# ygjwd12345/UCD

Measured on NVIDIA B200. Metric: ucd_loss_fwd_bwd_pixel_pairs_per_s, higher is better.
Workload: dtype bf16 operands / f32 accumulate (contrastive); f32 (CE, KD, upsample)

## Files before the change

include/ucd_b200.h:

```cpp
#ifndef UCD_B200_H
#define UCD_B200_H

#include <stddef.h>
#include <stdint.h>

#ifdef __cplusplus
extern "C" {
#endif

#define UCD_OK 0
#define UCD_EINVAL (-1)
#define UCD_ECUDA (-2)
#define UCD_ENOSUP (-3)

#define UCD_REDUCTION_NONE 0
#define UCD_REDUCTION_MEAN 1
#define UCD_REDUCTION_SUM 2

#define UCD_FEAT_DIM 256
#define UCD_TILE 128

int ucd_version(void);
const char* ucd_last_error(void);
int ucd_device_ok(void);

int ucd_unce_fwd(const float* x, int64_t* y, float* loss_px, float* lse_all, float* lse_old,
                 float* stats , float* scratch ,
                 int B, int C, int old_cl, int64_t HW, int ignore_index, void* stream);
int ucd_unce_bwd(const float* x, const int64_t* y, const float* lse_all,
                 const float* bkg_gap ,
                 const float* g_px, const float* g_scalar, float g_mul, const float* stats,
                 int mean_over_valid, float* dx, int accumulate, int B, int C, int old_cl, int64_t HW,
                 int ignore_index, void* stream);

int ucd_unkd_fwd(const float* x, const float* t, const float* mask, float alpha, float* out_px,
                 float* stats, float* lse3, float* scratch, int B, int C, int C_old, int64_t HW,
                 void* stream);
int ucd_unkd_bwd(const float* x, const float* t, const float* mask, float alpha, const float* lse3,
                 const float* g_px, const float* g_scalar, float g_mul, float* dx, int accumulate, int B, int C,
                 int C_old, int64_t HW, void* stream);
size_t ucd_reduce_scratch_floats(void);

int ucd_kd_fwd(const float* x, const float* t, const float* mask, float alpha, float* out_px, float* stats,
               float* lse3, float* scratch, int B, int C, int C_old, int64_t HW, int variant, float stats_scale,
               void* stream);
int ucd_kd_bwd(const float* x, const float* t, const float* mask, float alpha, const float* lse3,
               const float* g_px, const float* g_scalar, float g_mul, float* dx, int accumulate, int B, int C,
               int C_old, int64_t HW, int variant, void* stream);
int ucd_unce_unkd_bwd(const float* x, const int64_t* y, const float* lse_all, const float* bkg_gap ,
                      const float* ce_g_px, const float* ce_g_scalar, float ce_g_mul, const float* ce_stats,
                      int mean_over_valid, int old_cl, int ignore_index, const float* t, const float* mask,
                      float alpha, const float* lse3, const float* kd_g_px, const float* kd_g_scalar, float kd_g_mul,
                      int kd_variant, float* dx, int accumulate, int B, int C, int C_old, int64_t HW, void* stream);
int ucd_bkg_mask(const float* t_old, const int64_t* labels, float* mask, int B, int C_old, int64_t HW,
                 int old_cl, void* stream);

int ucd_upsample_bilinear_fwd(const float* in, float* out, int64_t planes, int h, int w, int H, int W,
                              void* stream);
int ucd_upsample_bilinear_bwd(const float* gout, float* gin, int64_t planes, int h, int w, int H, int W,
                              void* stream);
int ucd_unce_unkd_bwd_lowres(const float* x, const int64_t* y, const float* lse_all, const float* bkg_gap,
                             const float* ce_g_px, const float* ce_g_scalar, float ce_g_mul, const float* ce_stats,
                             int mean_over_valid, int old_cl, int ignore_index, const float* t, const float* mask,
                             float alpha, const float* lse3, const float* kd_g_px, const float* kd_g_scalar,
                             float kd_g_mul, int kd_variant, float* d_lr, int B, int C, int C_old, int h, int w, int H,
                             int W, void* stream);

size_t ucd_seg_fused_workspace_floats(int B, int C, int C_old, int h, int w, int H, int W);
int ucd_seg_fused_fwd(const float* lr, const float* lr_old, int64_t* labels, float* g_ce, float* g_kd,
                      float* sums, float* workspace, size_t workspace_floats, int B, int C, int C_old, int h,
                      int w, int H, int W, int old_cl, int ignore_index, float alpha, int need_grad,
                      void* stream);

int64_t ucd_con_max_tiles(int64_t n_px);
int ucd_con_prob_kpad(int C_old);
int ucd_con_num_bins(int max_label, int C_old);
int64_t ucd_con_px_meta_ints(int64_t n_px);
int64_t ucd_con_blk_meta_ints(int64_t n_px, int nb);
int ucd_con_prep_labels(const int64_t* labels, const float* l_po, int B, int C_old, int h, int w,
                        int H, int W, int max_label, int32_t* px_meta, int32_t* blk_meta, int32_t* counts,
                        int32_t* counts_host ,
                        void* stream);
int ucd_con_prep_pack(const float* f_n, const float* f_o, const float* l_po, const int32_t* px_meta,
                      int32_t* blk_meta, const int32_t* counts, int B, int C_old, int h, int w, int max_label,
                      float* anchor_f32, float* contrast_f32, void* la, void* lc,
                      int label_bytes ,
                      void* feat_tiles, void* prob_tiles, int32_t* lab_tiles, int32_t* tile_range,
                      int32_t* row_range , int32_t* row_ref, float* inv_norm,
                      int64_t max_tiles, void* stream);
int ucd_con_prep_bwd(const float* g_anchor, const float* anchor_f32, const float* inv_norm,
                     const int32_t* px_meta, const int32_t* blk_meta, float* df_n, int B, int h, int w,
                     void* stream);
int ucd_con_prep_pack_bf16(const void* f_n, const void* f_o, const float* l_po, const int32_t* px_meta,
                           int32_t* blk_meta, const int32_t* counts, int B, int C_old, int h, int w, int max_label,
                           float* anchor_f32, float* contrast_f32, void* la, void* lc, int label_bytes,
                           void* feat_tiles, void* prob_tiles, int32_t* lab_tiles, int32_t* tile_range,
                           int32_t* row_range, int32_t* row_ref, float* inv_norm, int64_t max_tiles, void* stream);
int ucd_con_prep_bwd_bf16(const float* g_anchor, const float* anchor_f32, const float* inv_norm,
                          const int32_t* px_meta, const int32_t* blk_meta, void* df_n, int B, int h, int w,
                          void* stream);
int ucd_con_tile_ranges(const int32_t* lab_tiles, int64_t n_tiles, const int32_t* n_limit, int32_t* tile_range,
                        void* stream);
int ucd_con_pack_rows(const float* rows, const int32_t* labels, int64_t n, void* feat_tiles,
                      int32_t* lab_tiles, int64_t max_tiles, void* stream);

int ucd_rows_normalize_fwd(const float* f, float* rows, float* inv_norm, int B, int h, int w, void* stream);
int ucd_rows_normalize_bwd(const float* g_rows, const float* rows, const float* inv_norm, float* df, int B, int h,
                           int w, void* stream);

size_t ucd_con_workspace_bytes(int64_t max_row_tiles, int64_t max_col_tiles, int64_t plan_row_tiles,
                               int64_t local_col_tiles );
int ucd_con_fwd(const void* feat_tiles, const void* prob_tiles, const int32_t* lab_tiles,
                const int32_t* chunk_counts, int n_chunks, int64_t chunk_tiles, int64_t chunk_stride_bytes,
                int local_chunk, int part, const void* row_feat_tiles,
                const void* row_prob_tiles, const int32_t* row_lab_tiles, const int32_t* n_rows,
                const int32_t* tile_range, const int32_t* row_range, int64_t self_tile0, const int32_t* min_new, int p_mode, int kpad, const float* dense_p,
                int64_t ldp, float inv_temperature, int need_grad, float* out, float* grad_unit,
                void* workspace, size_t workspace_bytes, int64_t max_row_tiles, int64_t plan_row_tiles,
                void* stream);
size_t ucd_selfcon_workspace_bytes(int64_t tiles );
int ucd_selfcon_fwd(const void* feat_tiles, const int32_t* lab_tiles, const int32_t* tile_range, const int32_t* counts,
                    const int32_t* n_rows, int64_t n, int64_t n_anchor, int mode, float inv_temperature, float kappa,
                    int need_grad, float* out, float* grad_unit, void* workspace, size_t workspace_bytes, void* stream);
int ucd_con_bwd(const float* grad_unit, const float* out, const float* g_scalar, float g_mul,
                const int32_t* n_rows, const int32_t* row_ref, float* d_anchor, int64_t max_rows, void* stream);

#ifdef __cplusplus
}
#endif
#endif
```

ucd_b200/_lib.py:

```python
import ctypes
import os
from ctypes import c_float, c_int, c_int64, c_size_t, c_void_p

_HERE = os.path.dirname(os.path.abspath(__file__))
LIB_PATH = os.path.join(_HERE, "libucd_b200.so")

_lib = None

UCD_ENOSUP = -3

P = c_void_p
_PROTOS = {
    "ucd_version": (c_int, []),
    "ucd_last_error": (ctypes.c_char_p, []),
    "ucd_device_ok": (c_int, []),
    "ucd_reduce_scratch_floats": (c_size_t, []),
    "ucd_unce_fwd": (c_int, [P, P, P, P, P, P, P, c_int, c_int, c_int, c_int64, c_int, P]),
    "ucd_unce_bwd": (c_int, [P, P, P, P, P, P, c_float, P, c_int, P, c_int, c_int, c_int, c_int, c_int64, c_int, P]),
    "ucd_unkd_fwd": (c_int, [P, P, P, c_float, P, P, P, P, c_int, c_int, c_int, c_int64, P]),
    "ucd_unkd_bwd": (c_int, [P, P, P, c_float, P, P, P, c_float, P, c_int, c_int, c_int, c_int, c_int64, P]),
    "ucd_kd_fwd": (c_int, [P, P, P, c_float, P, P, P, P, c_int, c_int, c_int, c_int64, c_int, c_float, P]),
    "ucd_kd_bwd": (c_int, [P, P, P, c_float, P, P, P, c_float, P, c_int, c_int, c_int, c_int, c_int64, c_int, P]),
    "ucd_unce_unkd_bwd": (c_int, [P, P, P, P, P, P, c_float, P, c_int, c_int, c_int, P, P, c_float, P, P, P, c_float, c_int,
                                  P, c_int, c_int, c_int, c_int, c_int64, P]),
    "ucd_unce_unkd_bwd_lowres": (c_int, [P, P, P, P, P, P, c_float, P, c_int, c_int, c_int, P, P, c_float, P, P, P,
                                         c_float, c_int, P, c_int, c_int, c_int, c_int, c_int, c_int, c_int, P]),
    "ucd_bkg_mask": (c_int, [P, P, P, c_int, c_int, c_int64, c_int, P]),
    "ucd_upsample_bilinear_fwd": (c_int, [P, P, c_int64, c_int, c_int, c_int, c_int, P]),
    "ucd_upsample_bilinear_bwd": (c_int, [P, P, c_int64, c_int, c_int, c_int, c_int, P]),
    "ucd_seg_fused_workspace_floats": (c_size_t, [c_int, c_int, c_int, c_int, c_int, c_int, c_int]),
    "ucd_seg_fused_fwd": (c_int, [P, P, P, P, P, P, P, c_size_t, c_int, c_int, c_int, c_int, c_int, c_int, c_int,
                                  c_int, c_int, c_float, c_int, P]),
    "ucd_con_max_tiles": (c_int64, [c_int64]),
    "ucd_con_prob_kpad": (c_int, [c_int]),
    "ucd_con_num_bins": (c_int, [c_int, c_int]),
    "ucd_con_px_meta_ints": (c_int64, [c_int64]),
    "ucd_con_blk_meta_ints": (c_int64, [c_int64, c_int]),
    "ucd_con_prep_labels": (c_int, [P, P, c_int, c_int, c_int, c_int, c_int, c_int, c_int, P, P, P, P, P]),
    "ucd_con_prep_pack": (c_int, [P, P, P, P, P, P, c_int, c_int, c_int, c_int, c_int, P, P, P, P, c_int, P, P, P, P,
                                  P, P, P, c_int64, P]),
    "ucd_con_prep_bwd": (c_int, [P, P, P, P, P, P, c_int, c_int, c_int, P]),
    "ucd_con_prep_pack_bf16": (c_int, [P, P, P, P, P, P, c_int, c_int, c_int, c_int, c_int, P, P, P, P, c_int, P, P, P,
                                       P, P, P, P, c_int64, P]),
    "ucd_con_prep_bwd_bf16": (c_int, [P, P, P, P, P, P, c_int, c_int, c_int, P]),
    "ucd_rows_normalize_fwd": (c_int, [P, P, P, c_int, c_int, c_int, P]),
    "ucd_rows_normalize_bwd": (c_int, [P, P, P, P, c_int, c_int, c_int, P]),
    "ucd_con_tile_ranges": (c_int, [P, c_int64, P, P, P]),
    "ucd_con_pack_rows": (c_int, [P, P, c_int64, P, P, c_int64, P]),
    "ucd_con_workspace_bytes": (c_size_t, [c_int64, c_int64, c_int64, c_int64]),
    "ucd_con_fwd": (c_int, [P, P, P, P, c_int, c_int64, c_int64, c_int, c_int, P, P, P, P, P, P, c_int64, P, c_int, c_int,
                            P, c_int64, c_float, c_int, P, P, P, c_size_t, c_int64, c_int64, P]),
    "ucd_con_bwd": (c_int, [P, P, P, c_float, P, P, P, c_int64, P]),
    "ucd_selfcon_workspace_bytes": (c_size_t, [c_int64]),
    "ucd_selfcon_fwd": (c_int, [P, P, P, P, P, c_int64, c_int64, c_int, c_float, c_float, c_int, P, P, P, c_size_t, P]),
}
EXPORTED = tuple(_PROTOS)
_DEBUG_PROTOS = {
    "ucd_con_debug_trace": (c_int, [P]),
    "ucd_con_debug_splits": (c_int, [c_int64, c_int64]),
    "ucd_selftest_umma": (c_int, [c_int, ctypes.POINTER(c_float)]),
    "ucd_selftest_mma_rate": (c_int, [c_int, c_int, ctypes.POINTER(c_float)]),
    "ucd_selftest_mma_mix": (c_int, [c_int] * 8 + [ctypes.POINTER(c_float)]),
    "ucd_selftest_pipe_rate": (c_int, [c_int, c_int, c_int, ctypes.POINTER(c_float)]),
    "ucd_selftest_read_probe": (c_int, [P, ctypes.c_longlong, c_int, c_int, c_int, c_int, ctypes.POINTER(c_float)]),
}
DEBUG_EXPORTED = tuple(_DEBUG_PROTOS)
DEBUG_LIB_PATH = os.path.join(_HERE, "libucd_b200_debug.so")
_debug = None


def lib():
    global _lib
    if _lib is None:
        if not os.path.exists(LIB_PATH):
            raise RuntimeError(
                "ucd_b200: %s is missing - build it with `python -m ucd_b200.build` "
                "(there is no CPU or PyTorch fallback for this path)" % LIB_PATH)
        h = ctypes.CDLL(LIB_PATH)
        for name, (res, args) in _PROTOS.items():
            fn = getattr(h, name)
            fn.restype = res
            fn.argtypes = args
        _lib = h
    return _lib


def debug_lib(as_product=False):
    global _debug, _lib
    if _debug is None:
        if not os.path.exists(DEBUG_LIB_PATH):
            raise RuntimeError("ucd_b200: %s is missing - build it with `python -m ucd_b200.build --debug`" % DEBUG_LIB_PATH)
        h = ctypes.CDLL(DEBUG_LIB_PATH)
        for name, (res, args) in list(_PROTOS.items()) + list(_DEBUG_PROTOS.items()):
            fn = getattr(h, name)
            fn.restype = res
            fn.argtypes = args
        _debug = h
    if as_product:
        _lib = _debug
    return _debug


class _NvtxProxy:

    def __init__(self, handle):
        self._h = handle

    def __getattr__(self, name):
        fn = getattr(self._h, name)
        if not name.startswith("ucd_") or name in ("ucd_last_error", "ucd_version", "ucd_device_ok"):
            return fn
        import torch

        def wrapped(*args):
            torch.cuda.nvtx.range_push(name)
            try:
                return fn(*args)
            finally:
                torch.cuda.nvtx.range_pop()
        return wrapped


def enable_nvtx(on=True):
    global _lib
    h = lib()
    if on and not isinstance(h, _NvtxProxy):
        _lib = _NvtxProxy(h)
    elif not on and isinstance(h, _NvtxProxy):
        _lib = h._h


def check(rc, what=""):
    if rc != 0:
        msg = lib().ucd_last_error().decode("utf-8", "replace")
        raise RuntimeError("ucd_b200 %s failed (code %d): %s" % (what, rc, msg))


def ptr(t):
    if t is None:
        return None
    return c_void_p(t) if isinstance(t, int) else c_void_p(t.data_ptr())


_raw_stream = None


def cur_stream():
    global _raw_stream
    import torch
    if _raw_stream is None:
        get_raw = getattr(torch._C, "_cuda_getCurrentRawStream", None)
        get_dev = getattr(torch._C, "_cuda_getDevice", None)
        if get_raw is not None and get_dev is not None:
            _raw_stream = lambda: get_raw(get_dev())
        else:
            _raw_stream = lambda: torch.cuda.current_stream().cuda_stream
    return c_void_p(_raw_stream())
```

ucd_b200/csrc/ce_kd.cu:

```cuda
#include "common.cuh"
#include "sweep_adjoint.cuh"

#include <stdlib.h>

namespace ucd {

constexpr int kStreamThreads = 256;
constexpr int kStreamMaxBlocks = kNumSMs * 8;
constexpr int kScratchFloats = 4 * kStreamMaxBlocks + 64;

template <int VEC>
struct Vec;
template <>
struct Vec<4> {
  static __device__ __forceinline__ void load(const float* p, float (&v)[4]) {
    float4 t = ldg_stream4(p);
    v[0] = t.x, v[1] = t.y, v[2] = t.z, v[3] = t.w;
  }
  static __device__ __forceinline__ void load_cached(const float* p, float (&v)[4]) {
    float4 t = *reinterpret_cast<const float4*>(p);
    v[0] = t.x, v[1] = t.y, v[2] = t.z, v[3] = t.w;
  }
  static __device__ __forceinline__ void store(float* p, const float (&v)[4]) {
    *reinterpret_cast<float4*>(p) = make_float4(v[0], v[1], v[2], v[3]);
  }
  static __device__ __forceinline__ void store_stream(float* p, const float (&v)[4]) {
    stg_stream4(p, make_float4(v[0], v[1], v[2], v[3]));
  }
};
template <>
struct Vec<1> {
  static __device__ __forceinline__ void load(const float* p, float (&v)[1]) { v[0] = ldg_stream1(p); }
  static __device__ __forceinline__ void load_cached(const float* p, float (&v)[1]) { v[0] = *p; }
  static __device__ __forceinline__ void store(float* p, const float (&v)[1]) { *p = v[0]; }
  static __device__ __forceinline__ void store_stream(float* p, const float (&v)[1]) { stg_stream1(p, v[0]); }
};

template <int VEC, bool ACC>
__device__ __forceinline__ void store_dx(float* p, float (&o)[VEC]) {
  if (ACC) {
    float old[VEC];
    Vec<VEC>::load(p, old);
#pragma unroll
    for (int i = 0; i < VEC; ++i) o[i] += old[i];
  }
  Vec<VEC>::store_stream(p, o);
}

__global__ void reduce_partials_kernel(const float* __restrict__ part, int nblk, int nk, float* __restrict__ out,
                                       float scale) {
  __shared__ float red[32];
  for (int k = 0; k < nk; ++k) {
    float acc = 0.f;
    for (int i = threadIdx.x; i < nblk; i += blockDim.x) acc += part[(size_t)k * nblk + i];
    float r = block_sum(acc, red);
    if (threadIdx.x == 0) out[k] = r * scale;
  }
}

constexpr float kNegBig = -3.0e38f;
constexpr int kLseChunk = 8;

template <int VEC, bool PICK>
__device__ __forceinline__ void lse_chunks(const float* __restrict__ xp, long long HW, int c0, int c1,
                                           const long long (&lab)[VEC], float (&m)[VEC], float (&s)[VEC],
                                           float (&picked)[VEC]) {
  for (int c = c0; c < c1; c += kLseChunk) {
    float v[kLseChunk][VEC];
#pragma unroll
    for (int k = 0; k < kLseChunk; ++k) {
      if (c + k < c1) {
        Vec<VEC>::load(xp + (long long)(c + k) * HW, v[k]);
      } else {
#pragma unroll
        for (int i = 0; i < VEC; ++i) v[k][i] = kNegBig;
      }
    }
#pragma unroll
    for (int i = 0; i < VEC; ++i) {
      float cm = v[0][i];
#pragma unroll
      for (int k = 1; k < kLseChunk; ++k) cm = fmaxf(cm, v[k][i]);
      const float nm = fmaxf(m[i], cm * kLog2e);
      float acc = s[i] * ex2f(m[i] - nm);
#pragma unroll
      for (int k = 0; k < kLseChunk; ++k) {
        acc += ex2f(fmaf(v[k][i], kLog2e, -nm));
        if (PICK) picked[i] = (lab[i] == c + k) ? v[k][i] : picked[i];
      }
      m[i] = nm;
      s[i] = acc;
    }
  }
}

template <int VEC>
__device__ __forceinline__ void lse_chunk4(const float (&v)[4][VEC], float (&m)[VEC], float (&s)[VEC]) {
#pragma unroll
  for (int i = 0; i < VEC; ++i) {
    const float cm = fmaxf(fmaxf(v[0][i], v[1][i]), fmaxf(v[2][i], v[3][i]));
    const float nm = fmaxf(m[i], cm * kLog2e);
    float acc = s[i] * ex2f(m[i] - nm);
#pragma unroll
    for (int k = 0; k < 4; ++k) acc += ex2f(fmaf(v[k][i], kLog2e, -nm));
    m[i] = nm;
    s[i] = acc;
  }
}

template <int VEC>
__device__ __forceinline__ void lse_planes(const float*& xc, long long HW, int n, float (&m)[VEC], float (&s)[VEC]) {
  int c = 0;
  for (; c + 4 <= n; c += 4) {
    float v[4][VEC];
    Vec<VEC>::load(xc, v[0]);
    Vec<VEC>::load(xc + HW, v[1]);
    Vec<VEC>::load(xc + 2 * HW, v[2]);
    Vec<VEC>::load(xc + 3 * HW, v[3]);
    xc += 4 * HW;
    lse_chunk4<VEC>(v, m, s);
  }
  if (c < n) {
    float v[4][VEC];
#pragma unroll
    for (int k = 0; k < 4; ++k) {
      if (c + k < n) {
        Vec<VEC>::load(xc + k * HW, v[k]);
      } else {
#pragma unroll
        for (int i = 0; i < VEC; ++i) v[k][i] = kNegBig;
      }
    }
    xc += (long long)(n - c) * HW;
    lse_chunk4<VEC>(v, m, s);
  }
}

__device__ __forceinline__ void group_to_bp(long long g, long long gpi, bool small, int vec, long long& b, long long& p) {
  if (small) {
    const unsigned bb = (unsigned)g / (unsigned)gpi;
    b = bb;
    p = (long long)((unsigned)g - bb * (unsigned)gpi) * vec;
  } else {
    b = g / gpi;
    p = (g - b * gpi) * vec;
  }
}

template <int VEC>
__global__ void __launch_bounds__(kStreamThreads, VEC == 4 ? 4 : 2)
unce_fwd_kernel(const float* __restrict__ x, long long* __restrict__ y, float* __restrict__ loss_px,
                float* __restrict__ lse_all_out, float* __restrict__ lse_old_out, float* __restrict__ part,
                int B, int C, int old_cl, long long HW, int ignore_index) {
  const long long gpi = HW / VEC;
  const long long n_groups = gpi * B;
  const bool small = n_groups < (1ll << 31) && gpi < (1ll << 31);
  const int oc = old_cl < C ? (old_cl > 0 ? old_cl : 0) : C;
  float loss_acc = 0.f, valid_acc = 0.f;
  for (long long g = (long long)blockIdx.x * blockDim.x + threadIdx.x; g < n_groups;
       g += (long long)gridDim.x * blockDim.x) {
    long long b, p;
    group_to_bp(g, gpi, small, VEC, b, p);
    const float* xp = x + (b * C) * HW + p;
    long long* yp = y + b * HW + p;
    long long yl[VEC];
    if (VEC == 4) {
      const longlong2 t0 = *reinterpret_cast<const longlong2*>(yp), t1 = *reinterpret_cast<const longlong2*>(yp + 2);
      yl[0] = t0.x, yl[1] = t0.y, yl[2 % VEC] = t1.x, yl[3 % VEC] = t1.y;
    } else {
#pragma unroll
      for (int i = 0; i < VEC; ++i) yl[i] = yp[i];
    }
    int lab[VEC];
    float picked[VEC];
#pragma unroll
    for (int i = 0; i < VEC; ++i) {
      long long t = yl[i];
      if (t < old_cl) {
        if (t != 0) yp[i] = 0;
        t = 0;
      }
      lab[i] = (t < 0 || t > 0x7fffffffLL) ? -1 : (int)t;
      picked[i] = (lab[i] >= 0 && lab[i] < C) ? __ldg(xp + (long long)lab[i] * HW + i) : 0.f;
    }
    float m[VEC], s[VEC], lse_old2[VEC];
#pragma unroll
    for (int i = 0; i < VEC; ++i) m[i] = kNegBig, s[i] = 0.f;
    const float* xc = xp;
    lse_planes<VEC>(xc, HW, oc, m, s);
#pragma unroll
    for (int i = 0; i < VEC; ++i) lse_old2[i] = m[i] + lg2f(s[i]);
    lse_planes<VEC>(xc, HW, C - oc, m, s);
    float out[VEC], la[VEC], lo[VEC];
#pragma unroll
    for (int i = 0; i < VEC; ++i) {
      const float lse2 = m[i] + lg2f(s[i]);
      la[i] = lse2 * kLn2;
      lo[i] = lse_old2[i] * kLn2;
      const bool ign = lab[i] == ignore_index;
      float l = (lab[i] == 0 && old_cl > 0) ? (la[i] - lo[i]) : (la[i] - picked[i]);
      if (ign || lab[i] < 0 || lab[i] >= C) l = 0.f;
      out[i] = l;
      loss_acc += l;
      valid_acc += ign ? 0.f : 1.f;
    }
    Vec<VEC>::store(loss_px + b * HW + p, out);
    Vec<VEC>::store(lse_all_out + b * HW + p, la);
    if (lse_old_out != nullptr) Vec<VEC>::store(lse_old_out + b * HW + p, lo);
  }
  if (part != nullptr) {
    __shared__ float red[32];
    float r0 = block_sum(loss_acc, red);
    float r1 = block_sum(valid_acc, red);
    if (threadIdx.x == 0) {
      part[blockIdx.x] = r0;
      part[gridDim.x + blockIdx.x] = r1;
    }
  }
}

template <int VEC, bool ACC>
__global__ void __launch_bounds__(kStreamThreads)
unce_bwd_kernel(const float* __restrict__ x, const long long* __restrict__ y, const float* __restrict__ lse_all,
                const float* __restrict__ bkg_gap, const float* __restrict__ g_px,
                const float* __restrict__ g_scalar, float g_mul, const float* __restrict__ stats,
                int mean_over_valid, float* __restrict__ dx, int B, int C, int old_cl, long long HW,
                int ignore_index) {
  const long long gpi = HW / VEC;
  const long long n_groups = gpi * B;
  float gs = 0.f;
  if (g_px == nullptr) {
    gs = g_scalar[0] * g_mul;
    if (mean_over_valid) gs = gs / stats[1];
  }
  for (long long g = (long long)blockIdx.x * blockDim.x + threadIdx.x; g < n_groups;
       g += (long long)gridDim.x * blockDim.x) {
    const long long b = g / gpi, p = (g - b * gpi) * VEC;
    const float* xp = x + (b * C) * HW + p;
    float* dp = dx + (b * C) * HW + p;
    const long long* yp = y + b * HW + p;
    float la2[VEC], up[VEC], fold[VEC];
    int lab[VEC];
    {
      float la[VEC], lo[VEC], gp[VEC];
      Vec<VEC>::load_cached(lse_all + b * HW + p, la);
      Vec<VEC>::load_cached(bkg_gap + b * HW + p, lo);
      if (g_px != nullptr) Vec<VEC>::load_cached(g_px + b * HW + p, gp);
#pragma unroll
      for (int i = 0; i < VEC; ++i) {
        long long t = yp[i];
        if (t < old_cl) t = 0;
        const bool dead = (t == ignore_index) || t < 0 || t >= C;
        lab[i] = dead ? -1 : (int)t;
        up[i] = dead ? 0.f : (g_px != nullptr ? gp[i] : gs);
        la2[i] = la[i] * kLog2e;
        fold[i] = ex2f(lo[i] * kLog2e);
      }
    }
#pragma unroll 4
    for (int c = 0; c < C; ++c) {
      float v[VEC], o[VEC];
      Vec<VEC>::load(xp + (long long)c * HW, v);
#pragma unroll
      for (int i = 0; i < VEC; ++i) {
        const float pr = ex2f(fmaf(v[i], kLog2e, -la2[i]));
        float sub;
        if (lab[i] == 0 && old_cl > 0)
          sub = (c < old_cl) ? pr * fold[i] : 0.f;
        else
          sub = (c == lab[i]) ? 1.f : 0.f;
        o[i] = up[i] * (pr - sub);
      }
      store_dx<VEC, ACC>(dp + (long long)c * HW, o);
    }
  }
}

template <int VEC, bool TAIL>
__device__ __forceinline__ void unkd_old_chunk(const float (&v)[4][VEC], const float (&u)[4][VEC], int nv, bool skip0,
                                               float a2, float (&m)[VEC], float (&s)[VEC], float (&mt)[VEC],
                                               float (&st)[VEC], float (&wx)[VEC]) {
#pragma unroll
  for (int i = 0; i < VEC; ++i) {
    float cm = v[0][i], ct = u[0][i] * a2;
#pragma unroll
    for (int k = 1; k < 4; ++k) {
      const bool live = !TAIL || k < nv;
      cm = live ? fmaxf(cm, v[k][i]) : cm;
      ct = live ? fmaxf(ct, u[k][i] * a2) : ct;
    }
    const float nm = fmaxf(m[i], cm * kLog2e), nt = fmaxf(mt[i], ct);
    float acc = s[i] * ex2f(m[i] - nm);
    const float rs = ex2f(mt[i] - nt);
    float tacc = st[i] * rs, wacc = wx[i] * rs;
#pragma unroll
    for (int k = 0; k < 4; ++k) {
      const bool live = !TAIL || k < nv;
      const float ex = ex2f(fmaf(v[k][i], kLog2e, -nm));
      const float et = ex2f(fmaf(u[k][i], a2, -nt));
      acc += live ? ex : 0.f;
      tacc += live ? et : 0.f;
      const float w = (live && !(k == 0 && skip0)) ? et : 0.f;
      wacc = fmaf(w, v[k][i], wacc);
    }
    m[i] = nm, s[i] = acc, mt[i] = nt, st[i] = tacc, wx[i] = wacc;
  }
}

template <int VEC>
__global__ void __launch_bounds__(kStreamThreads, VEC == 4 ? 3 : 2)
unkd_fwd_kernel(const float* __restrict__ x, const float* __restrict__ t, const float* __restrict__ mask,
                float alpha, float* __restrict__ out_px, float* __restrict__ lse3, float* __restrict__ part,
                int B, int C, int Cs, int C_old, int mask_zero, long long HW) {
  const long long gpi = HW / VEC;
  const long long n_groups = gpi * B;
  const bool small = n_groups < (1ll << 31) && gpi < (1ll << 31);
  const long long plane = (long long)B * HW;
  const float a2 = alpha * kLog2e;
  const float inv_cold = 1.f / (float)C_old;
  float acc = 0.f;
  for (long long g = (long long)blockIdx.x * blockDim.x + threadIdx.x; g < n_groups;
       g += (long long)gridDim.x * blockDim.x) {
    long long b, p;
    group_to_bp(g, gpi, small, VEC, b, p);
    const float* xp = x + (b * Cs) * HW + p;
    const float* xc = xp;
    const float* tc = t + (b * C_old) * HW + p;
    float m[VEC], s[VEC], mt[VEC], st[VEC], wx[VEC], x0[VEC], t0[VEC];
#pragma unroll
    for (int i = 0; i < VEC; ++i) m[i] = mt[i] = kNegBig, s[i] = st[i] = wx[i] = 0.f;
    int c = 0;
    for (; c + 4 <= C_old; c += 4) {
      float v[4][VEC], u[4][VEC];
#pragma unroll
      for (int k = 0; k < 4; ++k) {
        Vec<VEC>::load(xc + k * HW, v[k]);
        Vec<VEC>::load(tc + k * HW, u[k]);
      }
      xc += 4 * HW, tc += 4 * HW;
      if (c == 0) {
#pragma unroll
        for (int i = 0; i < VEC; ++i) x0[i] = v[0][i], t0[i] = u[0][i] * a2;
      }
      unkd_old_chunk<VEC, false>(v, u, 4, c == 0, a2, m, s, mt, st, wx);
    }
    if (c < C_old) {
      const int nv = C_old - c;
      float v[4][VEC], u[4][VEC];
#pragma unroll
      for (int k = 0; k < 4; ++k) {
        if (k < nv) {
          Vec<VEC>::load(xc + k * HW, v[k]);
          Vec<VEC>::load(tc + k * HW, u[k]);
        } else {
#pragma unroll
          for (int i = 0; i < VEC; ++i) v[k][i] = 0.f, u[k][i] = 0.f;
        }
      }
      if (c == 0) {
#pragma unroll
        for (int i = 0; i < VEC; ++i) x0[i] = v[0][i], t0[i] = u[0][i] * a2;
      }
      unkd_old_chunk<VEC, true>(v, u, nv, c == 0, a2, m, s, mt, st, wx);
    }
    float mn[VEC], sn[VEC];
#pragma unroll
    for (int i = 0; i < VEC; ++i) mn[i] = kNegBig, sn[i] = 0.f;
    xc = xp + (long long)C_old * HW;
    lse_planes<VEC>(xc, HW, C - C_old, mn, sn);
    float o[VEC], l_all[VEC], l_bkg[VEC], l_t[VEC];
    float mk[VEC];
    if (mask != nullptr) Vec<VEC>::load_cached(mask + b * HW + p, mk);
#pragma unroll
    for (int i = 0; i < VEC; ++i) {
      const float ma = fmaxf(m[i], mn[i]);
      const float lse2 = ma + lg2f(fmaf(s[i], ex2f(m[i] - ma), sn[i] * ex2f(mn[i] - ma)));
      const float x02 = x0[i] * kLog2e;
      const float mb = fmaxf(x02, mn[i]);
      const float lseb2 = mb + lg2f(fmaf(sn[i], ex2f(mn[i] - mb), ex2f(x02 - mb)));
      const float lset2 = mt[i] + lg2f(st[i]);
      l_all[i] = lse2 * kLn2;
      l_bkg[i] = lseb2 * kLn2;
      l_t[i] = lset2 * kLn2;
      const float q0 = ex2f(t0[i] - lset2);
      const float dot = wx[i] / st[i];
      float l = (q0 * (l_bkg[i] - l_all[i]) + dot - (1.f - q0) * l_all[i]) * inv_cold;
      if (mask != nullptr) l *= mask_zero ? (mk[i] == 0.f ? 1.f : 0.f) : mk[i];
      o[i] = -l;
      acc += l;
    }
    if (out_px != nullptr) Vec<VEC>::store(out_px + b * HW + p, o);
    Vec<VEC>::store(lse3 + b * HW + p, l_all);
    Vec<VEC>::store(lse3 + plane + b * HW + p, l_bkg);
    Vec<VEC>::store(lse3 + 2 * plane + b * HW + p, l_t);
  }
  __shared__ float red[32];
  float r = block_sum(acc, red);
  if (threadIdx.x == 0) part[blockIdx.x] = r;
}

template <int VEC, bool ACC>
__global__ void __launch_bounds__(kStreamThreads)
unkd_bwd_kernel(const float* __restrict__ x, const float* __restrict__ t, const float* __restrict__ mask,
                float alpha, const float* __restrict__ lse3, const float* __restrict__ g_px,
                const float* __restrict__ g_scalar, float g_mul, float* __restrict__ dx, int B, int C, int Cs,
                int C_old, int mask_zero, long long HW) {
  const long long gpi = HW / VEC;
  const long long n_groups = gpi * B;
  const long long plane = (long long)B * HW;
  const float a2 = alpha * kLog2e;
  const float inv_cold = 1.f / (float)C_old;
  const float gs = (g_px == nullptr) ? g_scalar[0] * g_mul : 0.f;
  for (long long g = (long long)blockIdx.x * blockDim.x + threadIdx.x; g < n_groups;
       g += (long long)gridDim.x * blockDim.x) {
    const long long b = g / gpi, p = (g - b * gpi) * VEC;
    const float* xp = x + (b * Cs) * HW + p;
    const float* tp = t + (b * C_old) * HW + p;
    float* dp = dx + (b * Cs) * HW + p;
    float la2[VEC], lt2[VEC], up[VEC], fb[VEC];
    {
      float la[VEC], lb[VEC], lt[VEC], gp[VEC], mk[VEC], u0[VEC];
      Vec<VEC>::load_cached(lse3 + b * HW + p, la);
      Vec<VEC>::load_cached(lse3 + plane + b * HW + p, lb);
      Vec<VEC>::load_cached(lse3 + 2 * plane + b * HW + p, lt);
      Vec<VEC>::load_cached(tp, u0);
      if (g_px != nullptr) Vec<VEC>::load_cached(g_px + b * HW + p, gp);
      if (mask != nullptr) Vec<VEC>::load_cached(mask + b * HW + p, mk);
#pragma unroll
      for (int i = 0; i < VEC; ++i) {
        la2[i] = la[i] * kLog2e;
        lt2[i] = lt[i] * kLog2e;
        float u = (g_px != nullptr ? gp[i] : gs) * inv_cold;
        if (mask != nullptr) u *= mask_zero ? (mk[i] == 0.f ? 1.f : 0.f) : mk[i];
        up[i] = u;
        const float q0 = ex2f(fmaf(u0[i], a2, -lt2[i]));
        fb[i] = q0 * ex2f((la[i] - lb[i]) * kLog2e);
      }
    }
    {
      float v[VEC], o[VEC];
      Vec<VEC>::load(xp, v);
#pragma unroll
      for (int i = 0; i < VEC; ++i) {
        const float pr = ex2f(fmaf(v[i], kLog2e, -la2[i]));
        o[i] = up[i] * (pr - pr * fb[i]);
      }
      store_dx<VEC, ACC>(dp, o);
    }
#pragma unroll 4
    for (int c = 1; c < C_old; ++c) {
      float v[VEC], u[VEC], o[VEC];
      Vec<VEC>::load(xp + (long long)c * HW, v);
      Vec<VEC>::load(tp + (long long)c * HW, u);
#pragma unroll
      for (int i = 0; i < VEC; ++i) {
        const float pr = ex2f(fmaf(v[i], kLog2e, -la2[i]));
        const float q = ex2f(fmaf(u[i], a2, -lt2[i]));
        o[i] = up[i] * (pr - q);
      }
      store_dx<VEC, ACC>(dp + (long long)c * HW, o);
    }
#pragma unroll 4
    for (int c = C_old; c < C; ++c) {
      float v[VEC], o[VEC];
      Vec<VEC>::load(xp + (long long)c * HW, v);
#pragma unroll
      for (int i = 0; i < VEC; ++i) {
        const float pr = ex2f(fmaf(v[i], kLog2e, -la2[i]));
        o[i] = up[i] * (pr - pr * fb[i]);
      }
      store_dx<VEC, ACC>(dp + (long long)c * HW, o);
    }
    if (!ACC)
      for (int c = C; c < Cs; ++c) {
        float o[VEC];
#pragma unroll
        for (int i = 0; i < VEC; ++i) o[i] = 0.f;
        Vec<VEC>::store_stream(dp + (long long)c * HW, o);
      }
  }
}

struct PairArgs {
  const long long* y;
  const float *lse_all, *bkg_gap, *ce_g_px, *t, *mask, *lse3, *kd_g_px;
  long long plane;
  float gs_ce, gs_kd, a2, inv_cold;
  int old_cl, ignore_index, C, C_old, mask_zero;
};

__device__ __forceinline__ PairArgs pair_args(const long long* y, const float* lse_all, const float* bkg_gap,
                                              const float* ce_g_px, const float* ce_g_scalar, float ce_g_mul,
                                              const float* ce_stats, int mean_over_valid, int old_cl, int ignore_index,
                                              const float* t, const float* mask, float alpha, const float* lse3,
                                              const float* kd_g_px, const float* kd_g_scalar, float kd_g_mul,
                                              int mask_zero, int B, int C, int C_old, long long HW) {
  PairArgs a;
  a.y = y, a.lse_all = lse_all, a.bkg_gap = bkg_gap, a.ce_g_px = ce_g_px, a.t = t, a.mask = mask, a.lse3 = lse3;
  a.kd_g_px = kd_g_px;
  a.plane = (long long)B * HW;
  a.a2 = alpha * kLog2e;
  a.inv_cold = 1.f / (float)C_old;
  a.gs_ce = 0.f;
  if (ce_g_px == nullptr) {
    a.gs_ce = ce_g_scalar[0] * ce_g_mul;
    if (mean_over_valid) a.gs_ce = a.gs_ce / ce_stats[1];
  }
  a.gs_kd = (kd_g_px == nullptr) ? kd_g_scalar[0] * kd_g_mul : 0.f;
  a.old_cl = old_cl, a.ignore_index = ignore_index, a.C = C, a.C_old = C_old, a.mask_zero = mask_zero;
  return a;
}

template <int VEC>
struct PairCoef {
  float la2[VEC], lt2[VEC], uce[VEC], ukd[VEC], fold[VEC], fb[VEC];
  int lab[VEC];
};

template <int VEC>
__device__ __forceinline__ void pair_coef(const PairArgs& a, long long px, const float* tp, PairCoef<VEC>& q) {
  float la[VEC], lo[VEC], lb[VEC], lt[VEC], gp[VEC], gk[VEC], mk[VEC], u0[VEC];
  Vec<VEC>::load_cached(a.lse_all + px, la);
  Vec<VEC>::load_cached(a.bkg_gap + px, lo);
  Vec<VEC>::load_cached(a.lse3 + a.plane + px, lb);
  Vec<VEC>::load_cached(a.lse3 + 2 * a.plane + px, lt);
  Vec<VEC>::load_cached(tp, u0);
  if (a.ce_g_px != nullptr) Vec<VEC>::load_cached(a.ce_g_px + px, gp);
  if (a.kd_g_px != nullptr) Vec<VEC>::load_cached(a.kd_g_px + px, gk);
  if (a.mask != nullptr) Vec<VEC>::load_cached(a.mask + px, mk);
  const long long* yp = a.y + px;
#pragma unroll
  for (int i = 0; i < VEC; ++i) {
    long long tt = yp[i];
    if (tt < a.old_cl) tt = 0;
    const bool dead = (tt == a.ignore_index) || tt < 0 || tt >= a.C;
    q.lab[i] = dead ? -1 : (int)tt;
    q.uce[i] = dead ? 0.f : (a.ce_g_px != nullptr ? gp[i] : a.gs_ce);
    q.la2[i] = la[i] * kLog2e;
    q.lt2[i] = lt[i] * kLog2e;
    q.fold[i] = ex2f(lo[i] * kLog2e);
    float u = (a.kd_g_px != nullptr ? gk[i] : a.gs_kd) * a.inv_cold;
    if (a.mask != nullptr) u *= a.mask_zero ? (mk[i] == 0.f ? 1.f : 0.f) : mk[i];
    q.ukd[i] = u;
    const float q0 = ex2f(fmaf(u0[i], a.a2, -q.lt2[i]));
    q.fb[i] = q0 * ex2f((la[i] - lb[i]) * kLog2e);
  }
}

template <int VEC>
__device__ __forceinline__ float pair_dx(const PairArgs& a, const PairCoef<VEC>& q, int i, int c, bool old_fg, float v,
                                         float u) {
  const float pr = ex2f(fmaf(v, kLog2e, -q.la2[i]));
  float sub_ce;
  if (q.lab[i] == 0 && a.old_cl > 0)
    sub_ce = (c < a.old_cl) ? pr * q.fold[i] : 0.f;
  else
    sub_ce = (c == q.lab[i]) ? 1.f : 0.f;
  const float sub_kd = old_fg ? ex2f(fmaf(u, a.a2, -q.lt2[i])) : pr * q.fb[i];
  return fmaf(q.uce[i], pr - sub_ce, q.ukd[i] * (pr - sub_kd));
}

template <int VEC, bool ACC>
__global__ void __launch_bounds__(kStreamThreads)
unce_unkd_bwd_kernel(const float* __restrict__ x, const long long* __restrict__ y, const float* __restrict__ lse_all,
                     const float* __restrict__ bkg_gap, const float* __restrict__ ce_g_px,
                     const float* __restrict__ ce_g_scalar, float ce_g_mul, const float* __restrict__ ce_stats,
                     int mean_over_valid, int old_cl, int ignore_index, const float* __restrict__ t,
                     const float* __restrict__ mask, float alpha, const float* __restrict__ lse3,
                     const float* __restrict__ kd_g_px, const float* __restrict__ kd_g_scalar, float kd_g_mul,
                     int mask_zero, float* __restrict__ dx, int B, int C, int C_old, long long HW) {
  const long long gpi = HW / VEC;
  const long long n_groups = gpi * B;
  const PairArgs a = pair_args(y, lse_all, bkg_gap, ce_g_px, ce_g_scalar, ce_g_mul, ce_stats, mean_over_valid, old_cl,
                               ignore_index, t, mask, alpha, lse3, kd_g_px, kd_g_scalar, kd_g_mul, mask_zero, B, C,
                               C_old, HW);
  for (long long g = (long long)blockIdx.x * blockDim.x + threadIdx.x; g < n_groups;
       g += (long long)gridDim.x * blockDim.x) {
    const long long b = g / gpi, p = (g - b * gpi) * VEC;
    const float* xp = x + (b * C) * HW + p;
    const float* tp = t + (b * C_old) * HW + p;
    float* dp = dx + (b * C) * HW + p;
    PairCoef<VEC> q;
    pair_coef<VEC>(a, b * HW + p, tp, q);
#pragma unroll 4
    for (int c = 0; c < C; ++c) {
      float v[VEC], u[VEC], o[VEC];
      Vec<VEC>::load(xp + (long long)c * HW, v);
      const bool old_fg = c >= 1 && c < C_old;
      if (old_fg) Vec<VEC>::load(tp + (long long)c * HW, u);
#pragma unroll
      for (int i = 0; i < VEC; ++i) o[i] = pair_dx<VEC>(a, q, i, c, old_fg, v[i], u[i]);
      store_dx<VEC, ACC>(dp + (long long)c * HW, o);
    }
  }
}

template <int KMAX, int NREG>
__global__ void __maxnreg__(NREG)
unce_unkd_bwd_lowres_kernel(const float* __restrict__ x, const long long* __restrict__ y,
                            const float* __restrict__ lse_all, const float* __restrict__ bkg_gap,
                            const float* __restrict__ ce_g_px, const float* __restrict__ ce_g_scalar, float ce_g_mul,
                            const float* __restrict__ ce_stats, int mean_over_valid, int old_cl, int ignore_index,
                            const float* __restrict__ t, const float* __restrict__ mask, float alpha,
                            const float* __restrict__ lse3, const float* __restrict__ kd_g_px,
                            const float* __restrict__ kd_g_scalar, float kd_g_mul, int mask_zero,
                            float* __restrict__ d_lr, int B, int C, int C_old, int h, int w, int H, int W,
                            float scale_h, float scale_w, int n_ranges, int range_rows, int n_cgroups, int ny_cap) {
  extern __shared__ __align__(16) uint8_t lr_dyn[];
  const int wv = blockDim.x;
  const int tid = threadIdx.x;
  float2* s_p = reinterpret_cast<float2*>(lr_dyn);
  short4* s_j = reinterpret_cast<short4*>(s_p + 2 * KMAX * wv);
  float2* s_h = reinterpret_cast<float2*>(s_j + w);
  int* s_k = reinterpret_cast<int*>(s_h + ny_cap);
  int* s_x0 = s_k + ny_cap;
  int* s_x1 = s_x0 + wv;
  __shared__ int s_lim[2];
  const long long HW = (long long)H * W;
  const PairArgs a = pair_args(y, lse_all, bkg_gap, ce_g_px, ce_g_scalar, ce_g_mul, ce_stats, mean_over_valid, old_cl,
                               ignore_index, t, mask, alpha, lse3, kd_g_px, kd_g_scalar, kd_g_mul, mask_zero, B, C,
                               C_old, HW);
  const int cg = blockIdx.x % n_cgroups;
  const int rest = blockIdx.x / n_cgroups;
  const int rg = rest % n_ranges;
  const long long b = rest / n_ranges;
  const int c0 = (int)((long long)cg * C / n_cgroups), kc = (int)((long long)(cg + 1) * C / n_cgroups) - c0;
  const int y0 = rg * range_rows, ylast = min(h, y0 + range_rows) - 1;
  float wx0[4], wx1[4];
  sweep_x_taps(tid, wv, w, W, scale_w, wx0, wx1, s_x0, s_x1, s_j);
  int i_lo, i_hi;
  const int Ylo = sweep_y_taps(tid, wv, y0, ylast, h, H, scale_h, ny_cap, s_k, s_h, s_lim, i_lo, i_hi);
  const int X = tid * 4;
  const float* xb = x + (b * C + c0) * HW + X;
  const float* tb = t + b * C_old * HW + X;
  float* out = d_lr + (b * C + c0) * (long long)h * w;
  float2 a0[KMAX], a1[KMAX];
#pragma unroll
  for (int j = 0; j < KMAX; ++j) a0[j] = a1[j] = make_float2(0.f, 0.f);
  int cur = -1, flip = 0;
  auto emit = [&](int row, bool shared) {
    float2* sp = s_p + flip * KMAX * wv;
#pragma unroll
    for (int j = 0; j < KMAX; ++j)
      if (j < kc) sp[j * wv + tid] = a0[j];
    __syncthreads();
    for (int o = tid; o < kc * w; o += wv) {
      const int j = o / w, xo = o - j * w;
      const short4 jr = s_j[xo];
      const float2* pj = sp + j * wv;
      float acc = 0.f;
      for (int i = jr.x; i < jr.y; ++i) acc += pj[i].x;
      for (int i = jr.z; i < jr.w; ++i) acc += pj[i].y;
      float* dst = out + ((long long)j * h + row) * w + xo;
      if (shared)
        atomicAdd(dst, acc);
      else
        *dst = acc;
    }
    flip ^= 1;
  };
#pragma unroll 1
  for (int i = i_lo; i < i_hi; ++i) {
    const int k = s_k[i];
    if (k != cur) {
      if (cur >= 0) {
        emit(cur, cur == y0 && y0 > 0);
#pragma unroll
        for (int j = 0; j < KMAX; ++j) a0[j] = a1[j], a1[j] = make_float2(0.f, 0.f);
      }
      cur = k;
    }
    const long long row = (long long)(Ylo + i) * W;
    PairCoef<4> q;
    pair_coef<4>(a, b * HW + row + X, tb + row, q);
    const float2 hw = s_h[i];
#pragma unroll
    for (int j0 = 0; j0 < KMAX; j0 += 4) {
      float v[4][4], u[4][4];
#pragma unroll
      for (int jj = 0; jj < 4; ++jj) {
        const int c = c0 + j0 + jj;
        if (j0 + jj < kc) Vec<4>::load(xb + (long long)(j0 + jj) * HW + row, v[jj]);
        if (j0 + jj < kc && c >= 1 && c < C_old) Vec<4>::load(tb + (long long)c * HW + row, u[jj]);
      }
#pragma unroll
      for (int jj = 0; jj < 4; ++jj) {
        const int j = j0 + jj, c = c0 + j;
        if (j < kc) {
          const bool old_fg = c >= 1 && c < C_old;
          float o[4];
#pragma unroll
          for (int e = 0; e < 4; ++e) o[e] = pair_dx<4>(a, q, e, c, old_fg, v[jj][e], u[jj][e]);
          const float p0 = fmaf(o[3], wx0[3], fmaf(o[2], wx0[2], fmaf(o[1], wx0[1], o[0] * wx0[0])));
          const float p1 = fmaf(o[3], wx1[3], fmaf(o[2], wx1[2], fmaf(o[1], wx1[1], o[0] * wx1[0])));
          a0[j].x = fmaf(hw.x, p0, a0[j].x), a0[j].y = fmaf(hw.x, p1, a0[j].y);
          a1[j].x = fmaf(hw.y, p0, a1[j].x), a1[j].y = fmaf(hw.y, p1, a1[j].y);
        }
      }
    }
  }
  if (cur >= 0) {
    emit(cur, cur == y0 && y0 > 0);
    if (ylast < h - 1) {
#pragma unroll
      for (int j = 0; j < KMAX; ++j) a0[j] = a1[j];
      emit(ylast + 1, true);
    }
  }
}

__global__ void __launch_bounds__(kStreamThreads)
bkg_mask_kernel(const float* __restrict__ t, const long long* __restrict__ y, float* __restrict__ mask, int B,
                int C_old, long long HW, int old_cl) {
  const long long n = (long long)B * HW;
  for (long long g = (long long)blockIdx.x * blockDim.x + threadIdx.x; g < n; g += (long long)gridDim.x * blockDim.x) {
    const long long b = g / HW, p = g - b * HW;
    const float* tp = t + (b * C_old) * HW + p;
    const float t0 = ldg_stream1(tp);
    const bool t0_nan = t0 != t0;
    bool bkg = true;
    for (int c = 1; c < C_old; ++c) {
      const float v = ldg_stream1(tp + (long long)c * HW);
      if (!t0_nan && (v > t0 || v != v)) bkg = false;
    }
    mask[g] = (bkg || y[g] > old_cl) ? 1.f : 0.f;
  }
}

static int stream_grid(long long n_groups) {
  long long blocks = (n_groups + kStreamThreads - 1) / kStreamThreads;
  if (blocks > kStreamMaxBlocks) blocks = kStreamMaxBlocks;
  if (blocks < 1) blocks = 1;
  return (int)blocks;
}

static bool can_vec4(long long HW, std::initializer_list<const void*> ptrs) {
  if (HW % 4 != 0) return false;
  for (const void* p : ptrs)
    if (p != nullptr && !aligned16(p)) return false;
  return true;
}

}

using namespace ucd;

extern "C" size_t ucd_reduce_scratch_floats(void) { return (size_t)kScratchFloats; }

extern "C" int ucd_unce_fwd(const float* x, int64_t* y, float* loss_px, float* lse_all, float* lse_old,
                            float* stats, float* scratch, int B, int C, int old_cl, int64_t HW,
                            int ignore_index, void* stream) {
  UCD_CHECK_ARG(x && y && loss_px && lse_all, "ucd_unce_fwd: null pointer");
  UCD_CHECK_ARG(B > 0 && C > 0 && HW > 0, "ucd_unce_fwd: bad shape B=%d C=%d HW=%lld", B, C, (long long)HW);
  UCD_CHECK_ARG(old_cl >= 0 && old_cl <= C, "ucd_unce_fwd: old_cl=%d outside [0,%d]", old_cl, C);
  UCD_CHECK_ARG(stats == nullptr || scratch != nullptr, "ucd_unce_fwd: stats requested without scratch");
  cudaStream_t st = (cudaStream_t)stream;
  float* part = stats ? scratch : nullptr;
  const bool v4 = can_vec4(HW, {x, loss_px, lse_all, lse_old}) && aligned16(y);
  const int grid = stream_grid((long long)B * HW / (v4 ? 4 : 1));
  if (v4)
    unce_fwd_kernel<4><<<grid, kStreamThreads, 0, st>>>(x, (long long*)y, loss_px, lse_all, lse_old, part, B, C,
                                                        old_cl, HW, ignore_index);
  else
    unce_fwd_kernel<1><<<grid, kStreamThreads, 0, st>>>(x, (long long*)y, loss_px, lse_all, lse_old, part, B, C,
                                                        old_cl, HW, ignore_index);
  UCD_CHECK_LAUNCH("unce_fwd_kernel");
  if (stats) {
    reduce_partials_kernel<<<1, 256, 0, st>>>(part, grid, 2, stats, 1.f);
    UCD_CHECK_LAUNCH("reduce_partials_kernel");
  }
  return UCD_OK;
}

extern "C" int ucd_unce_bwd(const float* x, const int64_t* y, const float* lse_all, const float* bkg_gap,
                            const float* g_px, const float* g_scalar, float g_mul, const float* stats,
                            int mean_over_valid, float* dx, int accumulate, int B, int C, int old_cl, int64_t HW,
                            int ignore_index, void* stream) {
  UCD_CHECK_ARG(x && y && lse_all && bkg_gap && dx, "ucd_unce_bwd: null pointer");
  UCD_CHECK_ARG(g_px || g_scalar, "ucd_unce_bwd: need g_px or g_scalar");
  UCD_CHECK_ARG(!mean_over_valid || stats, "ucd_unce_bwd: mean_over_valid needs stats");
  UCD_CHECK_ARG(B > 0 && C > 0 && HW > 0, "ucd_unce_bwd: bad shape");
  cudaStream_t st = (cudaStream_t)stream;
  const bool v4 = can_vec4(HW, {x, lse_all, bkg_gap, g_px, dx}) && aligned16(y);
  const int grid = stream_grid((long long)B * HW / (v4 ? 4 : 1));
  auto kern = v4 ? (accumulate ? unce_bwd_kernel<4, true> : unce_bwd_kernel<4, false>)
                 : (accumulate ? unce_bwd_kernel<1, true> : unce_bwd_kernel<1, false>);
  kern<<<grid, kStreamThreads, 0, st>>>(x, (const long long*)y, lse_all, bkg_gap, g_px, g_scalar, g_mul, stats,
                                        mean_over_valid, dx, B, C, old_cl, HW, ignore_index);
  UCD_CHECK_LAUNCH("unce_bwd_kernel");
  return UCD_OK;
}

static int kd_fwd_impl(const float* x, const float* t, const float* mask, float alpha, float* out_px, float* stats,
                       float* lse3, float* scratch, int B, int C, int C_old, int64_t HW, int variant, float stats_scale,
                       void* stream) {
  UCD_CHECK_ARG(x && t && stats && lse3 && scratch, "ucd_kd_fwd: null pointer");
  UCD_CHECK_ARG(B > 0 && HW > 0 && C_old >= 1 && C >= C_old, "ucd_kd_fwd: bad shape C=%d C_old=%d", C, C_old);
  UCD_CHECK_ARG(variant >= 0 && variant <= 2, "ucd_kd_fwd: bad variant %d", variant);
  cudaStream_t st = (cudaStream_t)stream;
  const int Cu = variant == 1 ? C_old : C, mz = variant == 2 ? 1 : 0;
  const bool v4 = can_vec4(HW, {x, t, mask, out_px, lse3}) && ((long long)B * HW) % 4 == 0;
  const int grid = stream_grid((long long)B * HW / (v4 ? 4 : 1));
  if (v4)
    unkd_fwd_kernel<4><<<grid, kStreamThreads, 0, st>>>(x, t, mask, alpha, out_px, lse3, scratch, B, Cu, C, C_old, mz, HW);
  else
    unkd_fwd_kernel<1><<<grid, kStreamThreads, 0, st>>>(x, t, mask, alpha, out_px, lse3, scratch, B, Cu, C, C_old, mz, HW);
  UCD_CHECK_LAUNCH("unkd_fwd_kernel");
  reduce_partials_kernel<<<1, 256, 0, st>>>(scratch, grid, 1, stats, stats_scale);
  UCD_CHECK_LAUNCH("reduce_partials_kernel");
  return UCD_OK;
}

static int kd_bwd_impl(const float* x, const float* t, const float* mask, float alpha, const float* lse3,
                       const float* g_px, const float* g_scalar, float g_mul, float* dx, int accumulate, int B, int C,
                       int C_old, int64_t HW, int variant, void* stream) {
  UCD_CHECK_ARG(x && t && lse3 && dx, "ucd_kd_bwd: null pointer");
  UCD_CHECK_ARG(g_px || g_scalar, "ucd_kd_bwd: need g_px or g_scalar");
  UCD_CHECK_ARG(B > 0 && HW > 0 && C_old >= 1 && C >= C_old, "ucd_kd_bwd: bad shape");
  UCD_CHECK_ARG(variant >= 0 && variant <= 2, "ucd_kd_bwd: bad variant %d", variant);
  cudaStream_t st = (cudaStream_t)stream;
  const int Cu = variant == 1 ? C_old : C, mz = variant == 2 ? 1 : 0;
  const bool v4 = can_vec4(HW, {x, t, mask, g_px, lse3, dx}) && ((long long)B * HW) % 4 == 0;
  const int grid = stream_grid((long long)B * HW / (v4 ? 4 : 1));
  auto kern = v4 ? (accumulate ? unkd_bwd_kernel<4, true> : unkd_bwd_kernel<4, false>)
                 : (accumulate ? unkd_bwd_kernel<1, true> : unkd_bwd_kernel<1, false>);
  kern<<<grid, kStreamThreads, 0, st>>>(x, t, mask, alpha, lse3, g_px, g_scalar, g_mul, dx, B, Cu, C, C_old, mz, HW);
  UCD_CHECK_LAUNCH("unkd_bwd_kernel");
  return UCD_OK;
}

extern "C" int ucd_unkd_fwd(const float* x, const float* t, const float* mask, float alpha, float* out_px,
                            float* stats, float* lse3, float* scratch, int B, int C, int C_old, int64_t HW,
                            void* stream) {
  return kd_fwd_impl(x, t, mask, alpha, out_px, stats, lse3, scratch, B, C, C_old, HW, 0, 1.f, stream);
}

extern "C" int ucd_unkd_bwd(const float* x, const float* t, const float* mask, float alpha, const float* lse3,
                            const float* g_px, const float* g_scalar, float g_mul, float* dx, int accumulate, int B,
                            int C, int C_old, int64_t HW, void* stream) {
  return kd_bwd_impl(x, t, mask, alpha, lse3, g_px, g_scalar, g_mul, dx, accumulate, B, C, C_old, HW, 0, stream);
}

extern "C" int ucd_kd_fwd(const float* x, const float* t, const float* mask, float alpha, float* out_px,
                          float* stats, float* lse3, float* scratch, int B, int C, int C_old, int64_t HW,
                          int variant, float stats_scale, void* stream) {
  return kd_fwd_impl(x, t, mask, alpha, out_px, stats, lse3, scratch, B, C, C_old, HW, variant, stats_scale, stream);
}

extern "C" int ucd_kd_bwd(const float* x, const float* t, const float* mask, float alpha, const float* lse3,
                          const float* g_px, const float* g_scalar, float g_mul, float* dx, int accumulate, int B,
                          int C, int C_old, int64_t HW, int variant, void* stream) {
  return kd_bwd_impl(x, t, mask, alpha, lse3, g_px, g_scalar, g_mul, dx, accumulate, B, C, C_old, HW, variant, stream);
}

extern "C" int ucd_bkg_mask(const float* t_old, const int64_t* labels, float* mask, int B, int C_old, int64_t HW,
                            int old_cl, void* stream) {
  UCD_CHECK_ARG(t_old && labels && mask, "ucd_bkg_mask: null pointer");
  UCD_CHECK_ARG(B > 0 && C_old >= 1 && HW > 0, "ucd_bkg_mask: bad shape");
  bkg_mask_kernel<<<stream_grid((long long)B * HW), kStreamThreads, 0, (cudaStream_t)stream>>>(
      t_old, (const long long*)labels, mask, B, C_old, HW, old_cl);
  UCD_CHECK_LAUNCH("bkg_mask_kernel");
  return UCD_OK;
}

extern "C" int ucd_unce_unkd_bwd(const float* x, const int64_t* y, const float* lse_all, const float* bkg_gap,
                                 const float* ce_g_px, const float* ce_g_scalar, float ce_g_mul, const float* ce_stats,
                                 int mean_over_valid, int old_cl, int ignore_index, const float* t, const float* mask,
                                 float alpha, const float* lse3, const float* kd_g_px, const float* kd_g_scalar,
                                 float kd_g_mul, int kd_variant, float* dx, int accumulate, int B, int C, int C_old,
                                 int64_t HW, void* stream) {
  UCD_CHECK_ARG(x && y && lse_all && bkg_gap && t && lse3 && dx, "ucd_unce_unkd_bwd: null pointer");
  UCD_CHECK_ARG((ce_g_px || ce_g_scalar) && (kd_g_px || kd_g_scalar), "ucd_unce_unkd_bwd: need g_px or g_scalar for both terms");
  UCD_CHECK_ARG(!mean_over_valid || ce_stats, "ucd_unce_unkd_bwd: mean_over_valid needs stats");
  UCD_CHECK_ARG(B > 0 && HW > 0 && C_old >= 1 && C >= C_old, "ucd_unce_unkd_bwd: bad shape");
  UCD_CHECK_ARG(kd_variant == 0 || kd_variant == 2, "ucd_unce_unkd_bwd: KD variant must be 0 (unbiased) or 2 (masked)");
  cudaStream_t st = (cudaStream_t)stream;
  const bool v4 = can_vec4(HW, {x, lse_all, bkg_gap, ce_g_px, t, mask, lse3, kd_g_px, dx}) && aligned16(y) &&
                  ((long long)B * HW) % 4 == 0;
  const int grid = stream_grid((long long)B * HW / (v4 ? 4 : 1));
  auto kern = v4 ? (accumulate ? unce_unkd_bwd_kernel<4, true> : unce_unkd_bwd_kernel<4, false>)
                 : (accumulate ? unce_unkd_bwd_kernel<1, true> : unce_unkd_bwd_kernel<1, false>);
  kern<<<grid, kStreamThreads, 0, st>>>(x, (const long long*)y, lse_all, bkg_gap, ce_g_px, ce_g_scalar, ce_g_mul,
                                        ce_stats, mean_over_valid, old_cl, ignore_index, t, mask, alpha, lse3, kd_g_px,
                                        kd_g_scalar, kd_g_mul, kd_variant == 2 ? 1 : 0, dx, B, C, C_old, HW);
  UCD_CHECK_LAUNCH("unce_unkd_bwd_kernel");
  return UCD_OK;
}

extern "C" int ucd_unce_unkd_bwd_lowres(const float* x, const int64_t* y, const float* lse_all, const float* bkg_gap,
                                        const float* ce_g_px, const float* ce_g_scalar, float ce_g_mul,
                                        const float* ce_stats, int mean_over_valid, int old_cl, int ignore_index,
                                        const float* t, const float* mask, float alpha, const float* lse3,
                                        const float* kd_g_px, const float* kd_g_scalar, float kd_g_mul, int kd_variant,
                                        float* d_lr, int B, int C, int C_old, int h, int w, int H, int W,
                                        void* stream) {
  UCD_CHECK_ARG(x && y && lse_all && bkg_gap && t && lse3 && d_lr, "ucd_unce_unkd_bwd_lowres: null pointer");
  UCD_CHECK_ARG((ce_g_px || ce_g_scalar) && (kd_g_px || kd_g_scalar),
                "ucd_unce_unkd_bwd_lowres: need g_px or g_scalar for both terms");
  UCD_CHECK_ARG(!mean_over_valid || ce_stats, "ucd_unce_unkd_bwd_lowres: mean_over_valid needs stats");
  UCD_CHECK_ARG(B > 0 && C_old >= 1 && C >= C_old && h > 0 && w > 0 && H > 0 && W > 0,
                "ucd_unce_unkd_bwd_lowres: bad shape");
  UCD_CHECK_ARG(kd_variant == 0 || kd_variant == 2,
                "ucd_unce_unkd_bwd_lowres: KD variant must be 0 (unbiased) or 2 (masked)");
  const int up = H / h;
  const bool ok = H % h == 0 && W % w == 0 && (W / w) % 8 == 0 && W / 4 <= 256 && (W / 4) % 32 == 0 && w <= W / 4 &&
                  can_vec4((long long)H * W, {x, lse_all, bkg_gap, ce_g_px, t, mask, lse3, kd_g_px}) && aligned16(y) &&
                  up <= 64;
  if (!ok) {
    set_error("ucd_unce_unkd_bwd_lowres: %dx%d -> %dx%d is not a sweep-form shape", h, w, H, W);
    return UCD_ENOSUP;
  }
  cudaStream_t st = (cudaStream_t)stream;
  const int wv = W / 4;
  struct Variant {
    int k, nreg;
    void (*fn)(const float*, const long long*, const float*, const float*, const float*, const float*, float,
               const float*, int, int, int, const float*, const float*, float, const float*, const float*,
               const float*, float, int, float*, int, int, int, int, int, int, int, float, float, int, int, int, int);
  };
  static const Variant variants[] = {{8, 128, unce_unkd_bwd_lowres_kernel<8, 128>},
                                     {4, 128, unce_unkd_bwd_lowres_kernel<4, 128>},
#ifdef UCD_DEBUG_KNOBS
                                     {4, 96, unce_unkd_bwd_lowres_kernel<4, 96>},
                                     {8, 112, unce_unkd_bwd_lowres_kernel<8, 112>},
#endif
  };
  int vi = 0;
#ifdef UCD_DEBUG_KNOBS
  if (const char* e = getenv("UCD_LRB_VARIANT")) vi = (atoi(e) >= 0 && atoi(e) < 4) ? atoi(e) : 0;
#endif
  const Variant& var = variants[vi];
  const int min_groups = (C + var.k - 1) / var.k;
  int groups = min_groups, rows = h;
  const long long want = 2ll * kNumSMs * (65536 / var.nreg / 32 * 32);
  auto threads = [&](int r, int g) { return (long long)B * ((h + r - 1) / r) * g * wv; };
  while (rows > 1 && threads(rows, groups) < want) rows = (rows + 1) / 2;
  while (groups < C && threads(rows, groups) < want) ++groups;
  auto dyn_bytes = [&](int r) {
    return (size_t)2 * var.k * wv * 8 + (size_t)w * 8 + (size_t)((r + 2) * up + 8) * 12 + (size_t)2 * wv * 4;
  };
#ifdef UCD_DEBUG_KNOBS
  if (const char* e = getenv("UCD_LRB_ROWS")) rows = atoi(e) > 0 ? min(atoi(e), h) : rows;
  if (const char* e = getenv("UCD_LRB_GROUPS")) groups = atoi(e) >= min_groups ? min(atoi(e), C) : groups;
#endif
  while (rows > 1 && dyn_bytes(rows) > 200 * 1024) rows = (rows + 1) / 2;
  const int n_ranges = (h + rows - 1) / rows;
  const long long nb = (long long)B * n_ranges * groups;
  if (nb >= (1ll << 31) || dyn_bytes(rows) > 200 * 1024) {
    set_error("ucd_unce_unkd_bwd_lowres: B=%d h=%d H=%d needs more blocks or shared memory than one launch has", B, h, H);
    return UCD_ENOSUP;
  }
  const int ny_cap = (rows + 2) * up + 8;
  const size_t dyn = dyn_bytes(rows);
  auto kern = var.fn;
  cudaError_t e;
  if (dyn > 48 * 1024) {
    e = cudaFuncSetAttribute(kern, cudaFuncAttributeMaxDynamicSharedMemorySize, (int)dyn);
    if (e != cudaSuccess) return cuda_fail(e, "cudaFuncSetAttribute(unce_unkd_bwd_lowres)");
  }
  e = cudaMemsetAsync(d_lr, 0, (size_t)B * C * h * w * sizeof(float), st);
  if (e != cudaSuccess) return cuda_fail(e, "cudaMemsetAsync(unce_unkd_bwd_lowres)");
  kern<<<(unsigned)nb, wv, dyn, st>>>(x, (const long long*)y, lse_all, bkg_gap, ce_g_px, ce_g_scalar, ce_g_mul,
                                      ce_stats, mean_over_valid, old_cl, ignore_index, t, mask, alpha, lse3, kd_g_px,
                                      kd_g_scalar, kd_g_mul, kd_variant == 2 ? 1 : 0, d_lr, B, C, C_old, h, w, H, W,
                                      (float)h / (float)H, (float)w / (float)W, n_ranges, rows, groups, ny_cap);
  UCD_CHECK_LAUNCH("unce_unkd_bwd_lowres_kernel");
  return UCD_OK;
}
```

ucd_b200/csrc/common.cuh:

```cuda
#pragma once
#include <cuda_runtime.h>
#include <cuda_bf16.h>
#include <stdint.h>
#include <stdio.h>
#include <stdarg.h>

#include "../../include/ucd_b200.h"

namespace ucd {

void set_error(const char* fmt, ...);
int cuda_fail(cudaError_t e, const char* what);

#define UCD_CHECK_ARG(cond, ...)            \
  do {                                      \
    if (!(cond)) {                          \
      ::ucd::set_error(__VA_ARGS__);        \
      return UCD_EINVAL;                    \
    }                                       \
  } while (0)

#define UCD_CHECK_LAUNCH(what)                                   \
  do {                                                           \
    cudaError_t e__ = cudaGetLastError();                        \
    if (e__ != cudaSuccess) return ::ucd::cuda_fail(e__, what);  \
  } while (0)

inline bool aligned16(const void* p) { return (reinterpret_cast<uintptr_t>(p) & 15u) == 0; }

constexpr int kNumSMs = 148;
constexpr float kLog2e = 1.4426950408889634f;
constexpr float kLn2 = 0.6931471805599453f;

__device__ __forceinline__ float ex2f(float x) {
  float y;
  asm("ex2.approx.ftz.f32 %0, %1;" : "=f"(y) : "f"(x));
  return y;
}
__device__ __forceinline__ float lg2f(float x) {
  float y;
  asm("lg2.approx.ftz.f32 %0, %1;" : "=f"(y) : "f"(x));
  return y;
}
__device__ __forceinline__ float rcpf(float x) {
  float y;
  asm("rcp.approx.ftz.f32 %0, %1;" : "=f"(y) : "f"(x));
  return y;
}

__device__ __forceinline__ void lse_push(float& m, float& s, float v) {
  float d = v - m;
  float e = ex2f(-fabsf(d));
  s = (d > 0.f) ? fmaf(s, e, 1.f) : (s + e);
  m = fmaxf(m, v);
}

__device__ __forceinline__ float warp_sum(float v) {
#pragma unroll
  for (int o = 16; o > 0; o >>= 1) v += __shfl_xor_sync(0xffffffffu, v, o);
  return v;
}
__device__ __forceinline__ float warp_max(float v) {
#pragma unroll
  for (int o = 16; o > 0; o >>= 1) v = fmaxf(v, __shfl_xor_sync(0xffffffffu, v, o));
  return v;
}

__device__ __forceinline__ float block_sum(float v, float* smem32) {
  const int lane = threadIdx.x & 31, wid = threadIdx.x >> 5;
  v = warp_sum(v);
  __syncthreads();
  if (lane == 0) smem32[wid] = v;
  __syncthreads();
  const int nw = (blockDim.x + 31) >> 5;
  float r = 0.f;
  if (wid == 0) {
    r = (lane < nw) ? smem32[lane] : 0.f;
    r = warp_sum(r);
  }
  return r;
}

__device__ __forceinline__ float4 ldg_stream4(const float* p) {
  float4 v;
  asm volatile("ld.global.nc.L1::no_allocate.v4.f32 {%0,%1,%2,%3}, [%4];"
               : "=f"(v.x), "=f"(v.y), "=f"(v.z), "=f"(v.w)
               : "l"(p));
  return v;
}
__device__ __forceinline__ float ldg_stream1(const float* p) {
  float v;
  asm volatile("ld.global.nc.L1::no_allocate.f32 %0, [%1];" : "=f"(v) : "l"(p));
  return v;
}
__device__ __forceinline__ void stg_stream4(float* p, float4 v) {
  asm volatile("st.global.cs.v4.f32 [%0], {%1,%2,%3,%4};" ::"l"(p), "f"(v.x), "f"(v.y), "f"(v.z), "f"(v.w)
               : "memory");
}
__device__ __forceinline__ void stg_stream1(float* p, float v) {
  asm volatile("st.global.cs.f32 [%0], %1;" ::"l"(p), "f"(v) : "memory");
}

__device__ __forceinline__ void cp_async16(void* smem_dst, const void* gsrc) {
  const uint32_t d = (uint32_t)__cvta_generic_to_shared(smem_dst);
  asm volatile("cp.async.cg.shared.global [%0], [%1], 16;" ::"r"(d), "l"(gsrc) : "memory");
}
__device__ __forceinline__ void cp_async_commit() { asm volatile("cp.async.commit_group;" ::: "memory"); }
template <int N>
__device__ __forceinline__ void cp_async_wait() {
  asm volatile("cp.async.wait_group %0;" ::"n"(N) : "memory");
}

struct Tap {
  int i0, i1;
  float w0, w1;
};
__device__ __forceinline__ Tap bilinear_tap(int dst, float scale, int in_size, int out_size) {
  Tap t;
  if (in_size == out_size) {
    t.i0 = t.i1 = dst;
    t.w0 = 1.f;
    t.w1 = 0.f;
    return t;
  }
  float src = __fmaf_rn(scale, __fadd_rn((float)dst, 0.5f), -0.5f);
  src = src < 0.f ? 0.f : src;
  int i0 = (int)floorf(src);
  i0 = i0 < in_size - 1 ? i0 : in_size - 1;
  t.i0 = i0;
  t.i1 = i0 + (i0 < in_size - 1 ? 1 : 0);
  float l1 = __fsub_rn(src, (float)i0);
  l1 = fminf(fmaxf(l1, 0.f), 1.f);
  t.w1 = l1;
  t.w0 = __fsub_rn(1.f, l1);
  return t;
}

__device__ __forceinline__ float bilinear_blend(bool small_out, float v00, float v01, float v10, float v11,
                                                float h0, float h1, float w0, float w1) {
  if (small_out) {
    float acc = __fmul_rn(__fmul_rn(h0, w1), v01);
    acc = __fmaf_rn(__fmul_rn(h0, w0), v00, acc);
    acc = __fmaf_rn(__fmul_rn(h1, w0), v10, acc);
    return __fmaf_rn(__fmul_rn(h1, w1), v11, acc);
  }
  const float t0 = __fmaf_rn(v00, w0, __fmul_rn(v01, w1));
  const float t1 = __fmaf_rn(v10, w0, __fmul_rn(v11, w1));
  return __fmaf_rn(t0, h0, __fmul_rn(t1, h1));
}

}
```

ucd_b200/csrc/upsample.cu:

```cuda
#include "common.cuh"
#include "sweep_adjoint.cuh"

#include <stdlib.h>

namespace ucd {

constexpr int kUpThreads = 256;

template <int VEC>
__global__ void __launch_bounds__(kUpThreads)
upsample_fwd_kernel(const float* __restrict__ in, float* __restrict__ out, long long planes, int h, int w, int H,
                    int W, float scale_h, float scale_w, int planes_per_block) {
  const int wv = (W + VEC - 1) / VEC;
  const long long idx = (long long)blockIdx.x * blockDim.x + threadIdx.x;
  if (idx >= (long long)H * wv) return;
  const int Y = (int)(idx / wv);
  const int X = (int)(idx - (long long)Y * wv) * VEC;
  const Tap ty = bilinear_tap(Y, scale_h, h, H);
  int x0[VEC], x1[VEC];
  float wx0[VEC], wx1[VEC];
  const bool small_out = H + W <= 128;
  bool uniform = true;
#pragma unroll
  for (int i = 0; i < VEC; ++i) {
    const Tap tx = bilinear_tap(X + i, scale_w, w, W);
    x0[i] = tx.i0, x1[i] = tx.i1, wx0[i] = tx.w0, wx1[i] = tx.w1;
    uniform = uniform && tx.i0 == x0[0] && tx.i1 == x1[0];
  }
  const long long p0 = (long long)blockIdx.y * planes_per_block;
  const long long p1 = (p0 + planes_per_block < planes) ? p0 + planes_per_block : planes;
  const size_t in_plane = (size_t)h * w, out_plane = (size_t)H * W;
  float* dst = out + p0 * out_plane + (size_t)Y * W + X;
  if (uniform) {
    const float* s00 = in + p0 * in_plane + ty.i0 * w + x0[0];
    const int d01 = x1[0] - x0[0], d10 = (ty.i1 - ty.i0) * w;
    constexpr int UP = 4;
    long long p = p0;
    for (; p + UP <= p1; p += UP) {
      float v[UP][4];
#pragma unroll
      for (int u = 0; u < UP; ++u) {
        const float* s = s00 + u * in_plane;
        v[u][0] = __ldg(s), v[u][1] = __ldg(s + d01), v[u][2] = __ldg(s + d10), v[u][3] = __ldg(s + d10 + d01);
      }
#pragma unroll
      for (int u = 0; u < UP; ++u) {
        float r[VEC];
#pragma unroll
        for (int i = 0; i < VEC; ++i)
          r[i] = bilinear_blend(small_out, v[u][0], v[u][1], v[u][2], v[u][3], ty.w0, ty.w1, wx0[i], wx1[i]);
        if (VEC == 4)
          stg_stream4(dst + u * out_plane, make_float4(r[0], r[1], r[2], r[3]));
        else
          stg_stream1(dst + u * out_plane, r[0]);
      }
      s00 += UP * in_plane;
      dst += UP * out_plane;
    }
    for (; p < p1; ++p) {
      const float a = __ldg(s00), b = __ldg(s00 + d01), c = __ldg(s00 + d10), d = __ldg(s00 + d10 + d01);
      float r[VEC];
#pragma unroll
      for (int i = 0; i < VEC; ++i) r[i] = bilinear_blend(small_out, a, b, c, d, ty.w0, ty.w1, wx0[i], wx1[i]);
      if (VEC == 4)
        stg_stream4(dst, make_float4(r[0], r[1], r[2], r[3]));
      else
        stg_stream1(dst, r[0]);
      s00 += in_plane;
      dst += out_plane;
    }
    return;
  }
  for (long long p = p0; p < p1; ++p) {
    const float* src = in + p * in_plane;
    float r[VEC];
#pragma unroll
    for (int i = 0; i < VEC; ++i)
      r[i] = bilinear_blend(small_out, __ldg(src + ty.i0 * w + x0[i]), __ldg(src + ty.i0 * w + x1[i]),
                            __ldg(src + ty.i1 * w + x0[i]), __ldg(src + ty.i1 * w + x1[i]), ty.w0, ty.w1, wx0[i],
                            wx1[i]);
    if (VEC == 4)
      stg_stream4(dst, make_float4(r[0], r[1], r[2], r[3]));
    else
      stg_stream1(dst, r[0]);
    dst += out_plane;
  }
}

constexpr int kUpMaxIvRows = 96;
template <int VEC>
__global__ void __launch_bounds__(kUpThreads)
upsample_fwd_interval_kernel(const float* __restrict__ in, float* __restrict__ out, int h, int w, int H, int W,
                             float scale_h, float scale_w, int tw, int n_col_tiles) {
  __shared__ float s_h0[kUpMaxIvRows], s_h1[kUpMaxIvRows];
  __shared__ int s_lo[3], s_hi[3];
  const int wv = (W + VEC - 1) / VEC;
  const int rp = kUpThreads / tw;
  const int per_plane = h * n_col_tiles;
  const long long plane = blockIdx.x / per_plane;
  const int rem = (int)(blockIdx.x - plane * per_plane);
  const int k = rem / n_col_tiles, col_tile = rem - k * n_col_tiles;
  const float inv = (float)H / (float)h;
  int lo = (int)floorf(((float)k - 0.5f) * inv) - 2, hi = (int)ceilf(((float)k + 1.5f) * inv) + 2;
  lo = max(lo, 0), hi = min(hi, H - 1);
  if (threadIdx.x < kUpMaxIvRows) {
    const int Y = lo + (int)threadIdx.x;
    bool match = false;
    if (Y <= hi) {
      const Tap ty = bilinear_tap(Y, scale_h, h, H);
      match = ty.i0 == k;
      s_h0[threadIdx.x] = ty.w0, s_h1[threadIdx.x] = ty.w1;
    }
    const unsigned bal = __ballot_sync(0xffffffffu, match);
    if ((threadIdx.x & 31) == 0) {
      const int wq = threadIdx.x >> 5;
      s_lo[wq] = bal ? wq * 32 + __ffs(bal) - 1 : 1 << 30;
      s_hi[wq] = bal ? wq * 32 + 31 - __clz(bal) : -1;
    }
  }
  __syncthreads();
  const int ia = min(s_lo[0], min(s_lo[1], s_lo[2])), ib = max(s_hi[0], max(s_hi[1], s_hi[2]));
  const int nrow = ib - ia + 1;
  if (nrow <= 0) return;
  const int Ya = lo + ia;
  const int xg = col_tile * tw + (int)threadIdx.x % tw, rphase = (int)threadIdx.x / tw;
  if (xg >= wv || rphase >= rp) return;
  const int X = xg * VEC;
  const int k1 = min(k + 1, h - 1);
  const float* r0 = in + (size_t)plane * h * w + (size_t)k * w;
  const float* r1 = in + (size_t)plane * h * w + (size_t)k1 * w;
  float t0[VEC], t1[VEC];
#pragma unroll
  for (int i = 0; i < VEC; ++i) {
    const Tap tx = bilinear_tap(min(X + i, W - 1), scale_w, w, W);
    t0[i] = __fmaf_rn(__ldg(r0 + tx.i0), tx.w0, __fmul_rn(__ldg(r0 + tx.i1), tx.w1));
    t1[i] = __fmaf_rn(__ldg(r1 + tx.i0), tx.w0, __fmul_rn(__ldg(r1 + tx.i1), tx.w1));
  }
  float* dst = out + (size_t)plane * H * W + (size_t)(Ya + rphase) * W + X;
  const size_t step = (size_t)rp * W;
#pragma unroll 4
  for (int r = rphase; r < nrow; r += rp) {
    const float h0 = s_h0[ia + r], h1 = s_h1[ia + r];
    float o[VEC];
#pragma unroll
    for (int i = 0; i < VEC; ++i) o[i] = __fmaf_rn(t0[i], h0, __fmul_rn(t1[i], h1));
    if (VEC == 4)
      stg_stream4(dst, make_float4(o[0], o[1], o[2], o[3]));
    else
      stg_stream1(dst, o[0]);
    dst += step;
  }
}

template <int RY, int VEC>
__global__ void __launch_bounds__(kUpThreads)
upsample_bwd_kernel(const float* __restrict__ gout, float* __restrict__ gin, int h, int w, int H, int W,
                    float scale_h, float scale_w, float inv_scale_h, float inv_scale_w, int ny_cap) {
  extern __shared__ __align__(16) float up_smem[];
  float* colsum = up_smem;
  float* wrow = up_smem + (size_t)RY * W;
  const long long plane = blockIdx.y;
  const int ybase = blockIdx.x * RY;
  const int ylast = min(ybase + RY, h) - 1;
  const float* g = gout + (size_t)plane * H * W;
  int Ylo = (int)floorf(((float)ybase - 0.5f) * inv_scale_h - 0.5f) - 2;
  int Yhi = (int)ceilf(((float)ylast + 1.5f) * inv_scale_h - 0.5f) + 2;
  Ylo = max(Ylo, 0);
  Yhi = min(Yhi, H - 1);
  if (h == H) {
    Ylo = ybase;
    Yhi = ylast;
  }
  Yhi = min(Yhi, Ylo + ny_cap - 1);
  const int ny = Yhi - Ylo + 1;
  for (int i = threadIdx.x; i < ny; i += kUpThreads) {
    const Tap ty = bilinear_tap(Ylo + i, scale_h, h, H);
#pragma unroll
    for (int r = 0; r < RY; ++r) {
      float wgt = 0.f;
      if (ty.i0 - ybase == r) wgt += ty.w0;
      if (ty.i1 - ybase == r) wgt += ty.w1;
      wrow[i * RY + r] = wgt;
    }
  }
  for (int i = threadIdx.x; i < RY * W; i += kUpThreads) colsum[i] = 0.f;
  __syncthreads();
  const int ngroups = (W + VEC - 1) / VEC;
  const int nsplit = max(1, min(kUpThreads / ngroups, 8));
  const int team = threadIdx.x / ngroups;
  const bool working = team < nsplit || ngroups >= kUpThreads;
  for (int g0 = 0; g0 < ngroups; g0 += kUpThreads) {
    const int xg = g0 + (ngroups >= kUpThreads ? threadIdx.x : threadIdx.x - team * ngroups);
    float acc[RY][VEC];
#pragma unroll
    for (int r = 0; r < RY; ++r)
#pragma unroll
      for (int k = 0; k < VEC; ++k) acc[r][k] = 0.f;
    if (working && xg < ngroups) {
      const int ystep = ngroups >= kUpThreads ? 1 : nsplit;
      const float* gp = g + (size_t)Ylo * W + (size_t)xg * VEC;
#pragma unroll 4
      for (int i = (ngroups >= kUpThreads ? 0 : team); i < ny; i += ystep) {
        float v[VEC];
        if (VEC == 4) {
          const float4 t = ldg_stream4(gp + (size_t)i * W);
          v[0] = t.x, v[1] = t.y, v[2] = t.z, v[3] = t.w;
        } else {
          v[0] = ldg_stream1(gp + (size_t)i * W);
        }
        float wr[RY];
        if (RY == 4) {
          const float4 t = *reinterpret_cast<const float4*>(wrow + i * RY);
          wr[0] = t.x, wr[1] = t.y, wr[2] = t.z, wr[3] = t.w;
        } else {
#pragma unroll
          for (int r = 0; r < RY; ++r) wr[r] = wrow[i * RY + r];
        }
#pragma unroll
        for (int r = 0; r < RY; ++r)
#pragma unroll
          for (int k = 0; k < VEC; ++k) acc[r][k] = fmaf(wr[r], v[k], acc[r][k]);
      }
    }
    for (int s = 0; s < (ngroups >= kUpThreads ? 1 : nsplit); ++s) {
      if (working && xg < ngroups && (ngroups >= kUpThreads || team == s)) {
#pragma unroll
        for (int r = 0; r < RY; ++r)
#pragma unroll
          for (int k = 0; k < VEC; ++k) colsum[r * W + xg * VEC + k] += acc[r][k];
      }
      __syncthreads();
    }
  }
  const int n_out = RY * w;
  for (int o = threadIdx.x; o < n_out; o += kUpThreads) {
    const int r = o / w, x = o - r * w;
    if (ybase + r >= h) continue;
    int Xlo = (int)floorf(((float)x - 0.5f) * inv_scale_w - 0.5f) - 2;
    int Xhi = (int)ceilf(((float)x + 1.5f) * inv_scale_w - 0.5f) + 2;
    Xlo = max(Xlo, 0);
    Xhi = min(Xhi, W - 1);
    if (w == W) Xlo = Xhi = x;
    float acc = 0.f;
    for (int X = Xlo; X <= Xhi; ++X) {
      const Tap tx = bilinear_tap(X, scale_w, w, W);
      float wgt = 0.f;
      if (tx.i0 == x) wgt += tx.w0;
      if (tx.i1 == x) wgt += tx.w1;
      acc = fmaf(wgt, colsum[r * W + X], acc);
    }
    gin[((size_t)plane * h + ybase + r) * w + x] = acc;
  }
}

template <int UN>
__global__ void __launch_bounds__(256, 4)
upsample_bwd_sweep_kernel(const float* __restrict__ gout, float* __restrict__ gin, int h, int w, int H, int W,
                          float scale_h, float scale_w, long long total_rows, int cap_rows, int ny_cap) {
  extern __shared__ __align__(16) uint8_t up_dyn[];
  const int wv = blockDim.x;
  const int tid = threadIdx.x;
  float4* ring = reinterpret_cast<float4*>(up_dyn);
  float2* s_p = reinterpret_cast<float2*>(ring + (size_t)UN * wv);
  short4* s_j = reinterpret_cast<short4*>(s_p + 2 * wv);
  float2* s_h = reinterpret_cast<float2*>(s_j + w);
  int* s_k = reinterpret_cast<int*>(s_h + ny_cap);
  int* s_x0 = s_k + ny_cap;
  int* s_x1 = s_x0 + wv;
  __shared__ int s_lim[2];
  const int X = tid * 4;
  float wx0[4], wx1[4];
  sweep_x_taps(tid, wv, w, W, scale_w, wx0, wx1, s_x0, s_x1, s_j);
  const uint32_t ring_s = (uint32_t)__cvta_generic_to_shared(ring + tid);
  const uint32_t slot_b = (uint32_t)wv * 16u;
  int flip = 0;
  const long long r_begin = total_rows * (long long)blockIdx.x / (long long)gridDim.x;
  const long long r_end = total_rows * ((long long)blockIdx.x + 1) / (long long)gridDim.x;
  for (long long r = r_begin; r < r_end;) {
    const long long plane = r / h;
    const int y0 = (int)(r - plane * h);
    const int ylast = (int)min((long long)min(h, y0 + cap_rows), y0 + (r_end - r)) - 1;
    r += ylast - y0 + 1;
    int i_lo, i_hi;
    const int Ylo = sweep_y_taps(tid, wv, y0, ylast, h, H, scale_h, ny_cap, s_k, s_h, s_lim, i_lo, i_hi);
    const float* gp = gout + (size_t)plane * H * W + (size_t)(Ylo + i_lo) * W + X;
    float* out = gin + (size_t)plane * h * w;
    float a0p0 = 0.f, a0p1 = 0.f, a1p0 = 0.f, a1p1 = 0.f, c0 = 0.f, c1 = 0.f;
    int cur = -1;
    auto emit = [&](int row, float v0, float v1, bool shared) {
      s_p[flip * wv + tid] = make_float2(v0, v1);
      __syncthreads();
      if (tid < w) {
        const short4 jr = s_j[tid];
        const float2* sp = s_p + flip * wv;
        float acc = 0.f;
        for (int j = jr.x; j < jr.y; ++j) acc += sp[j].x;
        for (int j = jr.z; j < jr.w; ++j) acc += sp[j].y;
        if (shared)
          atomicAdd(out + (size_t)row * w + tid, acc);
        else
          out[(size_t)row * w + tid] = acc;
      }
      flip ^= 1;
    };
    auto flush = [&]() {
      emit(cur, a0p0 + c0, a0p1 + c1, cur == y0 && y0 > 0);
      c0 = a1p0, c1 = a1p1;
      a0p0 = a0p1 = a1p0 = a1p1 = 0.f;
    };
    int nfetch = i_hi - i_lo;
    uint32_t fslot = 0, cslot = 0;
    auto fetch = [&]() {
      if (nfetch > 0) {
        asm volatile("cp.async.cg.shared.global [%0], [%1], 16;" ::"r"(ring_s + fslot), "l"(gp) : "memory");
        gp += W;
        --nfetch;
      }
      cp_async_commit();
      fslot = (fslot + slot_b == slot_b * UN) ? 0u : fslot + slot_b;
    };
#pragma unroll
    for (int j = 0; j < UN - 1; ++j) fetch();
#pragma unroll 1
    for (int i = i_lo; i < i_hi; ++i) {
      fetch();
      cp_async_wait<UN - 1>();
      const int k = s_k[i];
      if (k != cur) {
        if (cur >= 0) flush();
        cur = k;
      }
      float4 x;
      asm volatile("ld.shared.v4.f32 {%0,%1,%2,%3}, [%4];" : "=f"(x.x), "=f"(x.y), "=f"(x.z), "=f"(x.w) : "r"(ring_s + cslot));
      cslot = (cslot + slot_b == slot_b * UN) ? 0u : cslot + slot_b;
      const float2 hw = s_h[i];
      const float p0 = fmaf(x.w, wx0[3], fmaf(x.z, wx0[2], fmaf(x.y, wx0[1], x.x * wx0[0])));
      const float p1 = fmaf(x.w, wx1[3], fmaf(x.z, wx1[2], fmaf(x.y, wx1[1], x.x * wx1[0])));
      a0p0 = fmaf(hw.x, p0, a0p0), a0p1 = fmaf(hw.x, p1, a0p1);
      a1p0 = fmaf(hw.y, p0, a1p0), a1p1 = fmaf(hw.y, p1, a1p1);
    }
    cp_async_wait<0>();
    if (cur >= 0) {
      flush();
      if (ylast < h - 1) emit(ylast + 1, c0, c1, true);
    }
  }
}

}

using namespace ucd;

extern "C" int ucd_upsample_bilinear_fwd(const float* in, float* out, int64_t planes, int h, int w, int H, int W,
                                         void* stream) {
  UCD_CHECK_ARG(in && out, "ucd_upsample_bilinear_fwd: null pointer");
  UCD_CHECK_ARG(planes > 0 && h > 0 && w > 0 && H > 0 && W > 0, "ucd_upsample_bilinear_fwd: bad shape");
  UCD_CHECK_ARG((long long)h * w < (1ll << 30), "ucd_upsample_bilinear_fwd: source plane too large");
  cudaStream_t st = (cudaStream_t)stream;
  const float sh = (float)h / (float)H, sw = (float)w / (float)W;
  const bool v4 = (W % 4 == 0) && aligned16(out);
  const int wv = v4 ? W / 4 : W;
  if (H + W > 128 && H >= h && W >= w && (double)H / h <= 40.0  && planes * (long long)h < (1ll << 30) / 64) {
    const int tw = wv < kUpThreads ? wv : kUpThreads;
    const int nct = (wv + tw - 1) / tw;
    const unsigned nblk = (unsigned)(planes * h * nct);
    if (v4)
      upsample_fwd_interval_kernel<4><<<nblk, kUpThreads, 0, st>>>(in, out, h, w, H, W, sh, sw, tw, nct);
    else
      upsample_fwd_interval_kernel<1><<<nblk, kUpThreads, 0, st>>>(in, out, h, w, H, W, sh, sw, tw, nct);
    UCD_CHECK_LAUNCH("upsample_fwd_interval_kernel");
    return UCD_OK;
  }
  const long long work = (long long)H * wv;
  const int gx = (int)((work + kUpThreads - 1) / kUpThreads);
  long long want_y = (32ll * kNumSMs + gx - 1) / gx;
  if (want_y < 1) want_y = 1;
  if (want_y > (planes + 15) / 16) want_y = (planes + 15) / 16;
#ifdef UCD_DEBUG_KNOBS
  if (const char* e = getenv("UCD_UP_GY")) want_y = atoi(e) > 0 ? atoi(e) : want_y;
#endif
  if (want_y > planes) want_y = planes;
  const int ppb = (int)((planes + want_y - 1) / want_y);
  const int gy = (int)((planes + ppb - 1) / ppb);
  UCD_CHECK_ARG(gy <= 65535, "ucd_upsample_bilinear_fwd: too many planes");
  dim3 grid(gx, gy);
  if (v4)
    upsample_fwd_kernel<4><<<grid, kUpThreads, 0, st>>>(in, out, planes, h, w, H, W, sh, sw, ppb);
  else
    upsample_fwd_kernel<1><<<grid, kUpThreads, 0, st>>>(in, out, planes, h, w, H, W, sh, sw, ppb);
  UCD_CHECK_LAUNCH("upsample_fwd_kernel");
  return UCD_OK;
}

extern "C" int ucd_upsample_bilinear_bwd(const float* gout, float* gin, int64_t planes, int h, int w, int H, int W,
                                         void* stream) {
  UCD_CHECK_ARG(gout && gin, "ucd_upsample_bilinear_bwd: null pointer");
  UCD_CHECK_ARG(planes > 0 && h > 0 && w > 0 && H > 0 && W > 0, "ucd_upsample_bilinear_bwd: bad shape");
  cudaStream_t st = (cudaStream_t)stream;
  constexpr int RY = 4;
  const int ny_cap = (h == H) ? RY : (int)((double)(RY + 2) * H / h) + 8;
  const size_t smem = ((size_t)RY * W + (size_t)ny_cap * RY) * sizeof(float);
  UCD_CHECK_ARG(smem <= 200 * 1024, "ucd_upsample_bilinear_bwd: W=%d / scale too large for one block", W);
  const float sh = (float)h / (float)H, sw = (float)w / (float)W;
  const bool v4 = (W % 4 == 0) && aligned16(gout);
  const int up = H / (h > 0 ? h : 1);
  constexpr int kUpSweepTaps = 640;
  const int cap_rows = up > 0 ? (kUpSweepTaps - 8) / up - 2 : 0;
  if (v4 && H % h == 0 && W % w == 0 && (W / w) % 8 == 0 && W / 4 <= 256 && (W / 4) % 32 == 0 && w <= W / 4 &&
      cap_rows >= 1) {
    int un = 8, bps = (W / 4 <= 128 ? 4 : 2);
#ifdef UCD_DEBUG_KNOBS
    if (const char* e = getenv("UCD_UPB_UN")) un = atoi(e);
    if (const char* e = getenv("UCD_UPB_BPS")) bps = atoi(e);
#endif
    const long long total_rows = planes * h;
    long long nb = (long long)kNumSMs * bps;
    while (nb > kNumSMs && total_rows / nb < 4) nb -= kNumSMs;
    if (nb > total_rows) nb = total_rows;
    long long seg = (total_rows + nb - 1) / nb + 1;
    if (seg > cap_rows) seg = cap_rows;
    const int ny_cap = (int)(seg + 2) * up + 8;
    const int wv4 = W / 4;
    const size_t dyn = (size_t)un * wv4 * 16 + (size_t)2 * wv4 * 8 + (size_t)ny_cap * 12 + (size_t)2 * wv4 * 4 + (size_t)w * 8;
    cudaError_t e = cudaMemsetAsync(gin, 0, (size_t)planes * h * w * sizeof(float), st);
    if (e != cudaSuccess) return cuda_fail(e, "cudaMemsetAsync(upsample_bwd)");
    auto kern = upsample_bwd_sweep_kernel<8>;
#ifdef UCD_DEBUG_KNOBS
    if (un == 4) kern = upsample_bwd_sweep_kernel<4>;
    if (un == 12) kern = upsample_bwd_sweep_kernel<12>;
    if (un == 16) kern = upsample_bwd_sweep_kernel<16>;
#endif
    if (dyn > 48 * 1024) {
      e = cudaFuncSetAttribute(kern, cudaFuncAttributeMaxDynamicSharedMemorySize, (int)dyn);
      if (e != cudaSuccess) return cuda_fail(e, "cudaFuncSetAttribute(upsample_bwd_sweep)");
    }
    kern<<<(unsigned)nb, wv4, dyn, st>>>(gout, gin, h, w, H, W, sh, sw, total_rows, cap_rows, ny_cap);
    UCD_CHECK_LAUNCH("upsample_bwd_sweep_kernel");
    return UCD_OK;
  }
  auto kern = v4 ? upsample_bwd_kernel<RY, 4> : upsample_bwd_kernel<RY, 1>;
  if (smem > 48 * 1024) {
    cudaError_t e = cudaFuncSetAttribute(kern, cudaFuncAttributeMaxDynamicSharedMemorySize, (int)smem);
    if (e != cudaSuccess) return cuda_fail(e, "cudaFuncSetAttribute(upsample_bwd)");
  }
  const int gyb = (h + RY - 1) / RY;
  for (int64_t p0 = 0; p0 < planes; p0 += 65535) {
    const int np = (int)((planes - p0 < 65535) ? planes - p0 : 65535);
    dim3 grid(gyb, np);
    kern<<<grid, kUpThreads, smem, st>>>(gout + (size_t)p0 * H * W, gin + (size_t)p0 * h * w, h, w, H, W, sh, sw,
                                         (float)H / (float)h, (float)W / (float)w, ny_cap);
    UCD_CHECK_LAUNCH("upsample_bwd_kernel");
  }
  return UCD_OK;
}
```

ucd_b200/losses.py:

```python
from __future__ import annotations

import weakref

import torch
import torch.nn as nn

from . import _lib
from ._lib import check, cur_stream, ptr

FEAT_DIM = 256
TILE = 128


def _need_cuda(*tensors):
    cur = None
    for t in tensors:
        if t is None:
            continue
        if not t.is_cuda:
            raise RuntimeError("ucd_b200: expected CUDA tensors (there is no CPU fallback for this path)")
        if cur is None:
            cur = torch.cuda.current_device()
        if t.device.index != cur:
            raise RuntimeError("ucd_b200: tensor on cuda:%d but the current device is cuda:%d - wrap the call in "
                               "`with torch.cuda.device(tensor.device):`" % (t.device.index, cur))


def _f32c(t):
    if t.dtype != torch.float32:
        t = t.float()
    return t.contiguous()


def _scalar_grad(g):
    if g.dim() == 0:
        return g.reshape(1)
    if all(s == 0 for s in g.stride()):
        return g.as_strided((1,), (1,))
    return None


class _UpsampleFn(torch.autograd.Function):
    @staticmethod
    def forward(ctx, x, out_h, out_w):
        _need_cuda(x)
        ctx.set_materialize_grads(False)
        x = _f32c(x)
        lead, (h, w) = x.shape[:-2], x.shape[-2:]
        planes = 1
        for d in lead:
            planes *= d
        out = torch.empty(*lead, out_h, out_w, device=x.device, dtype=torch.float32)
        if planes > 0:
            check(_lib.lib().ucd_upsample_bilinear_fwd(ptr(x), ptr(out), planes, h, w, out_h, out_w, cur_stream()),
                  "upsample_bilinear_fwd")
        ctx.shape = (lead, h, w, out_h, out_w, planes)
        return out

    @staticmethod
    def backward(ctx, g):
        if g is None:
            return None, None, None
        lead, h, w, out_h, out_w, planes = ctx.shape
        g = _f32c(g)
        gin = torch.empty(*lead, h, w, device=g.device, dtype=torch.float32)
        if planes > 0:
            check(_lib.lib().ucd_upsample_bilinear_bwd(ptr(g), ptr(gin), planes, h, w, out_h, out_w, cur_stream()),
                  "upsample_bilinear_bwd")
        return gin, None, None


def interpolate_bilinear(x, size):
    out = _UpsampleFn.apply(x, int(size[0]), int(size[1]))
    if out.requires_grad:
        out._ucd_upsample = (x, x._version, out._version)
    return out


class _Route:

    __slots__ = ("lr_shape", "out_ref", "out_hw", "probe_node")
    _probes = {}

    def __init__(self, src, out, probe_node):
        self.lr_shape, self.out_hw, self.probe_node = tuple(src.shape), tuple(out.shape[2:]), probe_node
        self.out_ref = weakref.ref(out)

    @staticmethod
    def of(outputs):
        rec = getattr(outputs, "_ucd_upsample", None)
        if rec is None:
            return None
        src, src_version, out_version = rec
        if (src._version != src_version or outputs._version != out_version or not src.requires_grad
                or src.dim() != 4 or outputs.dim() != 4):
            return None
        probe = _Route._probes.get(outputs.device)
        if probe is None:
            probe = _Route._probes[outputs.device] = torch.empty((), device=outputs.device, requires_grad=True)
        return _Route(src, outputs, torch.autograd.graph.get_gradient_edge(probe).node), src, probe

    def route_now(self):
        out = self.out_ref()
        if out is None or out.retains_grad or out._backward_hooks:
            return False
        try:
            return bool(torch._C._will_engine_execute_node(self.probe_node))
        except Exception:
            return False


class _GradChain:

    __slots__ = ("token", "calls", "pending", "closed")
    MAX_MEMBERS = 4

    def __init__(self):
        self.token, self.calls, self.pending, self.closed = None, 0, [], False

    @staticmethod
    def of(t):
        if not (torch.is_grad_enabled() and t.requires_grad and t.dtype == torch.float32 and t.is_contiguous()):
            return None
        chain = getattr(t, "_ucd_grad_chain", None)
        if chain is None or chain.closed or chain.calls >= _GradChain.MAX_MEMBERS:
            chain = t._ucd_grad_chain = _GradChain()
        return chain

    def submit(self, term, seq, is_head, route=None):
        self.closed = True
        if seq == self.calls:
            self.pending = []
        if not is_head:
            if term is not None:
                self.pending.append(term)
            return None, None, None
        terms, self.pending = self.pending + ([term] if term is not None else []), []
        self.token = None
        if not terms:
            return None, None, None
        d_lr = _launch_lowres(terms, route) if route is not None else None
        if d_lr is not None:
            return None, None, d_lr
        return _launch_terms(terms), None, None


def _pair(terms):
    ce = [t for t in terms if t["kind"] == "ce"]
    kd = [t for t in terms if t["kind"] == "kd" and t["variant"] in (0, 2)]
    if ce and kd and ce[0]["C"] == kd[0]["C"] and ce[0]["HW"] == kd[0]["HW"]:
        return ce[0], kd[0]
    return None


def _launch_lowres(terms, route):
    pair = _pair(terms)
    if pair is None or len(terms) != 2 or not route.route_now():
        return None
    c, k = pair
    B, C, h, w = route.lr_shape
    H, W = route.out_hw
    d_lr = torch.empty(B, C, h, w, device=c["x"].device, dtype=torch.float32)
    rc = _lib.lib().ucd_unce_unkd_bwd_lowres(
        ptr(c["x"]), ptr(c["targets"]), ptr(c["lse"][0]), ptr(c["lse"][1]), ptr(c["g_px"]), ptr(c["g_sc"]), 1.0,
        ptr(c["stats"]), c["mean_over_valid"], c["old_cl"], c["ignore_index"], ptr(k["t"]), ptr(k["m"]), k["alpha"],
        ptr(k["lse3"]), ptr(k["g_px"]), ptr(k["g_sc"]), k["g_mul"], k["variant"], ptr(d_lr), B, C, k["C_old"], h, w,
        H, W, cur_stream())
    if rc == _lib.UCD_ENOSUP:
        return None
    check(rc, "unce_unkd_bwd_lowres")
    return d_lr


def _launch_terms(terms):
    dx = torch.empty_like(terms[0]["x"])
    pair = _pair(terms)
    acc = False
    if pair is not None:
        c, k = pair
        check(_lib.lib().ucd_unce_unkd_bwd(
            ptr(c["x"]), ptr(c["targets"]), ptr(c["lse"][0]), ptr(c["lse"][1]), ptr(c["g_px"]), ptr(c["g_sc"]), 1.0,
            ptr(c["stats"]), c["mean_over_valid"], c["old_cl"], c["ignore_index"], ptr(k["t"]), ptr(k["m"]), k["alpha"],
            ptr(k["lse3"]), ptr(k["g_px"]), ptr(k["g_sc"]), k["g_mul"], k["variant"], ptr(dx), 0, c["B"], c["C"],
            k["C_old"], c["HW"], cur_stream()), "unce_unkd_bwd")
        terms = [t for t in terms if t is not c and t is not k]
        acc = True
    for t in terms:
        _launch_term(t, dx, acc)
        acc = True
    return dx


def _launch_term(t, dx, acc):
    if t["kind"] == "ce":
        check(_lib.lib().ucd_unce_bwd(ptr(t["x"]), ptr(t["targets"]), ptr(t["lse"][0]), ptr(t["lse"][1]), ptr(t["g_px"]),
                                      ptr(t["g_sc"]), 1.0, ptr(t["stats"]), t["mean_over_valid"], ptr(dx),
                                      1 if acc else 0, t["B"], t["C"], t["old_cl"], t["HW"], t["ignore_index"],
                                      cur_stream()), "unce_bwd")
    else:
        check(_lib.lib().ucd_kd_bwd(ptr(t["x"]), ptr(t["t"]), ptr(t["m"]), t["alpha"], ptr(t["lse3"]), ptr(t["g_px"]),
                                    ptr(t["g_sc"]), t["g_mul"], ptr(dx), 1 if acc else 0, t["B"], t["C"], t["C_old"],
                                    t["HW"], t["variant"], cur_stream()), "kd_bwd")


class _UnceFn(torch.autograd.Function):
    @staticmethod
    def forward(ctx, inputs, targets, old_cl, ignore_index, reduction, chain=None, link=None, route=None, src=None,
                probe=None):
        ctx.chain, ctx.is_head, ctx.seq = chain, link is None, (chain.calls if chain is not None else 0)
        ctx.route = route
        ctx.set_materialize_grads(False)
        B, C = inputs.shape[0], inputs.shape[1]
        HW = inputs.numel() // max(B * C, 1)
        x = _f32c(inputs)
        dev = x.device
        loss_px = torch.empty(targets.shape, device=dev, dtype=torch.float32)
        lse = torch.empty(targets.shape, device=dev, dtype=torch.float32)
        want_stats = reduction != "none"
        stats = torch.empty(2, device=dev, dtype=torch.float32) if want_stats else None
        scratch = (torch.empty(_lib.lib().ucd_reduce_scratch_floats(), device=dev, dtype=torch.float32)
                   if want_stats else None)
        check(_lib.lib().ucd_unce_fwd(ptr(x), ptr(targets), ptr(loss_px), ptr(lse), None, ptr(stats),
                                      ptr(scratch), B, C, old_cl, HW, ignore_index, cur_stream()), "unce_fwd")
        ctx.save_for_backward(x, targets, lse, stats, loss_px)
        ctx.cfg = (B, C, HW, old_cl, ignore_index, reduction)
        out = loss_px if reduction == "none" else (stats[0].clone() if reduction == "sum" else stats[0] / stats[1])
        if chain is None:
            return out
        return out, torch.empty((), device=dev, dtype=torch.float32)

    @staticmethod
    def backward(ctx, g, g_token=None):
        x, targets, lse, stats, loss_px = ctx.saved_tensors
        B, C, HW, old_cl, ignore_index, reduction = ctx.cfg
        if g is None:
            if ctx.chain is None:
                return (None,) * 10
            d_in, d_link, d_src = ctx.chain.submit(None, ctx.seq, ctx.is_head, ctx.route)
            return d_in, None, None, None, None, None, d_link, None, d_src, None
        g_px, g_sc = None, None
        if reduction == "none":
            g_sc = _scalar_grad(g)
            if g_sc is None:
                g_px = _f32c(g)
        else:
            g_sc = g.reshape(1)
        if g_sc is not None:
            g_sc = _f32c(g_sc)
        term = dict(kind="ce", x=x, targets=targets, lse=(lse, loss_px), stats=stats, g_px=g_px, g_sc=g_sc,
                    mean_over_valid=1 if reduction == "mean" else 0, B=B, C=C, HW=HW, old_cl=old_cl,
                    ignore_index=ignore_index)
        if ctx.chain is None:
            dx = torch.empty_like(x)
            _launch_term(term, dx, False)
            return (dx,) + (None,) * 9
        d_in, d_link, d_src = ctx.chain.submit(term, ctx.seq, ctx.is_head, ctx.route)
        return d_in, None, None, None, None, None, d_link, None, d_src, None


def _chained(fn, inputs, args):
    chain = _GradChain.of(inputs)
    if chain is None:
        return fn.apply(inputs, *args)
    route = None
    if chain.token is None:
        route = _Route.of(inputs)
    chain.calls += 1
    if route is None:
        out, token = fn.apply(inputs, *args, chain, chain.token)
    else:
        out, token = fn.apply(inputs, *args, chain, chain.token, *route)
    chain.token = token
    return out


class UnbiasedCrossEntropy(nn.Module):

    def __init__(self, old_cl=None, reduction='mean', ignore_index=255):
        super().__init__()
        self.reduction = reduction
        self.ignore_index = ignore_index
        self.old_cl = old_cl

    def forward(self, inputs, targets):
        _need_cuda(inputs, targets)
        if self.reduction not in ("none", "mean", "sum"):
            raise ValueError("reduction must be 'none', 'mean' or 'sum'")
        if targets.dtype != torch.int64:
            raise TypeError("UnbiasedCrossEntropy: targets must be int64 (train.py:98 casts labels to long)")
        if inputs.dim() < 2 or targets.shape != inputs.shape[:1] + inputs.shape[2:]:
            raise ValueError("UnbiasedCrossEntropy: inputs [B,C,...] and targets [B,...] shapes disagree")
        old_cl = inputs.shape[1] if self.old_cl is None else int(self.old_cl)
        tgt = targets if targets.is_contiguous() else targets.contiguous()
        out = _chained(_UnceFn, inputs, (tgt, old_cl, int(self.ignore_index), self.reduction))
        if tgt is not targets:
            targets.copy_(tgt)
        return out


class _UnkdFn(torch.autograd.Function):
    @staticmethod
    def forward(ctx, inputs, targets, mask, alpha, reduction, variant=0, chain=None, link=None, route=None, src=None,
                probe=None):
        ctx.chain, ctx.is_head, ctx.seq = chain, link is None, (chain.calls if chain is not None else 0)
        ctx.route = route
        ctx.set_materialize_grads(False)
        B, C, C_old = inputs.shape[0], inputs.shape[1], targets.shape[1]
        HW = inputs.numel() // max(B * C, 1)
        x, t = _f32c(inputs), _f32c(targets)
        m = None if mask is None else _f32c(mask)
        dev = x.device
        px_shape = (B,) + tuple(inputs.shape[2:])
        out_px = torch.empty(px_shape, device=dev, dtype=torch.float32) if reduction == "none" else None
        stats = torch.empty(1, device=dev, dtype=torch.float32)
        lse3 = torch.empty((3,) + px_shape, device=dev, dtype=torch.float32)
        scratch = torch.empty(_lib.lib().ucd_reduce_scratch_floats(), device=dev, dtype=torch.float32)
        scale = -1.0 / float(B * HW) if reduction == "mean" else -1.0
        check(_lib.lib().ucd_kd_fwd(ptr(x), ptr(t), ptr(m), float(alpha), ptr(out_px), ptr(stats), ptr(lse3),
                                    ptr(scratch), B, C, C_old, HW, variant, scale, cur_stream()), "kd_fwd")
        ctx.save_for_backward(x, t, m, lse3)
        ctx.cfg = (B, C, C_old, HW, float(alpha), reduction, variant)
        out = out_px if reduction == "none" else stats[0]
        if chain is None:
            return out
        return out, torch.empty((), device=dev, dtype=torch.float32)

    @staticmethod
    def backward(ctx, g, g_token=None):
        x, t, m, lse3 = ctx.saved_tensors
        B, C, C_old, HW, alpha, reduction, variant = ctx.cfg
        if g is None:
            if ctx.chain is None:
                return (None,) * 11
            d_in, d_link, d_src = ctx.chain.submit(None, ctx.seq, ctx.is_head, ctx.route)
            return d_in, None, None, None, None, None, None, d_link, None, d_src, None
        g_px, g_sc, g_mul = None, None, 1.0
        if reduction == "none":
            g_sc = _scalar_grad(g)
            if g_sc is None:
                g_px = _f32c(g)
        else:
            g_sc = g.reshape(1)
            if reduction == "mean":
                g_mul = 1.0 / float(B * HW)
        if g_sc is not None:
            g_sc = _f32c(g_sc)
        term = dict(kind="kd", x=x, t=t, m=m, lse3=lse3, g_px=g_px, g_sc=g_sc, g_mul=g_mul, alpha=alpha, B=B, C=C,
                    C_old=C_old, HW=HW, variant=variant)
        if ctx.chain is None:
            dx = torch.empty_like(x)
            _launch_term(term, dx, False)
            return (dx,) + (None,) * 10
        d_in, d_link, d_src = ctx.chain.submit(term, ctx.seq, ctx.is_head, ctx.route)
        return d_in, None, None, None, None, None, None, d_link, None, d_src, None


class UnbiasedKnowledgeDistillationLoss(nn.Module):

    def __init__(self, reduction='mean', alpha=1.):
        super().__init__()
        self.reduction = reduction
        self.alpha = alpha

    def forward(self, inputs, targets, mask=None):
        _need_cuda(inputs, targets, mask)
        if inputs.shape[1] < targets.shape[1] or inputs.shape[2:] != targets.shape[2:]:
            raise ValueError("UnbiasedKnowledgeDistillationLoss: inputs [B,C,...] / targets [B,C_old,...] disagree")
        if mask is not None and tuple(mask.shape) != (inputs.shape[0],) + tuple(inputs.shape[2:]):
            raise ValueError("UnbiasedKnowledgeDistillationLoss: mask must be [B,...]")
        red = self.reduction if self.reduction in ("mean", "sum") else "none"
        return _chained(_UnkdFn, inputs, (targets.detach(), mask, self.alpha, red, 0))


def _kd_forward(name, variant, self, inputs, targets, mask):
    _need_cuda(inputs, targets, mask)
    if inputs.shape[1] < targets.shape[1] or inputs.shape[2:] != targets.shape[2:]:
        raise ValueError("%s: inputs [B,C,...] / targets [B,C_old,...] disagree" % name)
    if mask is not None and tuple(mask.shape) != (inputs.shape[0],) + tuple(inputs.shape[2:]):
        raise ValueError("%s: mask must be [B,...]" % name)
    red = self.reduction if self.reduction in ("mean", "sum") else "none"
    return _chained(_UnkdFn, inputs, (targets.detach(), mask, self.alpha, red, variant))


class KnowledgeDistillationLoss(nn.Module):

    def __init__(self, reduction='mean', alpha=1.):
        super().__init__()
        self.reduction = reduction
        self.alpha = alpha

    def forward(self, inputs, targets, mask=None):
        return _kd_forward("KnowledgeDistillationLoss", 1, self, inputs, targets, mask)


class MaskKnowledgeDistillationLoss(nn.Module):

    def __init__(self, reduction='mean', alpha=1.):
        super().__init__()
        self.reduction = reduction
        self.alpha = alpha

    def forward(self, inputs, targets, mask=None):
        return _kd_forward("MaskKnowledgeDistillationLoss", 2, self, inputs, targets, mask)


class MaskCrossEntropy(nn.Module):

    def __init__(self, old_cl=None, reduction='mean', ignore_index=255):
        super().__init__()
        self.reduction = reduction
        self.ignore_index = ignore_index
        self.old_cl = old_cl

    def forward(self, inputs, targets, outputs_old=None):
        _need_cuda(inputs, targets, outputs_old)
        if targets.dtype != torch.int64:
            raise TypeError("MaskCrossEntropy: targets must be int64")
        if inputs.dim() < 2 or targets.shape != inputs.shape[:1] + inputs.shape[2:]:
            raise ValueError("MaskCrossEntropy: inputs [B,C,...] and targets [B,...] shapes disagree")
        if outputs_old is not None and self.old_cl is None:
            raise TypeError("MaskCrossEntropy: old_cl=None cannot be compared with the labels (loss.py:210)")
        old_cl = 0 if self.old_cl is None else int(self.old_cl)
        ign = int(self.ignore_index)
        if old_cl > 1:
            tgt = torch.where((targets >= 1) & (targets < old_cl), torch.full_like(targets, ign), targets).contiguous()
        else:
            tgt = targets.clone()
        loss = _UnceFn.apply(inputs, tgt, old_cl, ign, "none")
        if outputs_old is not None:
            t = _f32c(outputs_old.detach())
            B, C_old = t.shape[0], t.shape[1]
            mask = torch.empty(targets.shape, device=t.device, dtype=torch.float32)
            lab = targets if targets.is_contiguous() else targets.contiguous()
            check(_lib.lib().ucd_bkg_mask(ptr(t), ptr(lab), ptr(mask), B, C_old, t[0, 0].numel(), old_cl,
                                          cur_stream()), "bkg_mask")
            loss = loss * mask
        if self.reduction == 'mean':
            return -torch.mean(loss)
        if self.reduction == 'sum':
            return -torch.sum(loss)
        return loss


def payload_layout(max_tiles, kpad):
    al = lambda n: (n + 255) & ~255
    off = {"counts": 0}
    o = 256
    for name, nbytes in (("range", max_tiles * 8), ("lab", max_tiles * TILE * 4), ("prob", max_tiles * kpad * TILE * 2),
                         ("feat", max_tiles * FEAT_DIM * TILE * 2)):
        off[name] = o
        o += al(nbytes)
    off["nbytes"] = o
    return off


def payload_views(buf, max_tiles, kpad):
    lay = payload_layout(max_tiles, kpad)
    assert buf.dtype == torch.uint8 and buf.shape[-1] == lay["nbytes"]

    def sec(name, nbytes, dtype, shape):
        v = buf[..., lay[name]:lay[name] + nbytes].view(dtype)
        return v.unflatten(-1, shape)
    T = max_tiles
    return dict(counts=sec("counts", 16, torch.int32, (4,)), range=sec("range", T * 8, torch.int32, (T, 2)),
                lab=sec("lab", T * TILE * 4, torch.int32, (T, TILE)),
                prob=sec("prob", T * kpad * TILE * 2, torch.bfloat16, (T, kpad // 8, TILE, 8)),
                feat=sec("feat", T * FEAT_DIM * TILE * 2, torch.bfloat16, (T, FEAT_DIM // 8, TILE, 8)))


class ContrastPack:

    def __init__(self):
        self.n_px = 0
        self.shape = None
        self.c_old = 0
        self.kpad = 0
        self.max_tiles = 0
        self.payload = None
        self.addr = None
        self._views = None
        self.n_a = self.n_o = self.min_new = None
        self.px_meta = self.blk_meta = None
        self.label_n = self.mix = self.flags = None
        self.anchor_f32 = self.contrast_f32 = None
        self.la = self.lc = None
        self.row_range = None
        self.row_ref = self.inv_norm = None
        self.max_label = 20
        self.l_po = None
        self.bf16_feats = False

    @property
    def n_c(self):
        return self.n_a + self.n_o

    def _view(self, name):
        if self._views is None:
            self._views = payload_views(self.payload, self.max_tiles, self.kpad)
        return self._views[name]

    counts = property(lambda self: self._view("counts"))
    tile_range = property(lambda self: self._view("range"))
    lab_tiles = property(lambda self: self._view("lab"))
    prob_tiles = property(lambda self: self._view("prob"))
    feat_tiles = property(lambda self: self._view("feat"))


_PINNED = {}


def _pinned_counts(dev):
    key = (dev.type, dev.index)
    buf = _PINNED.get(key)
    if buf is None:
        buf = _PINNED[key] = torch.empty(4, dtype=torch.int32).pin_memory()
    return buf


def _multi_rank():
    import torch.distributed as dist
    return dist.is_available() and dist.is_initialized() and dist.get_world_size() > 1


def _build_pack(f_n, f_o, l_po, labels, max_label, sync=True, require_new_class=True):
    _need_cuda(f_n, f_o, l_po, labels)
    if f_n.dim() != 4 or f_n.shape[1] != FEAT_DIM or f_o.shape != f_n.shape:
        raise ValueError("pre_contrastive_pixel: f_n / f_o must be [B,%d,h,w]" % FEAT_DIM)
    B, _, h, w = f_n.shape
    if l_po.dim() != 4 or l_po.shape[0] != B or tuple(l_po.shape[2:]) != (h, w):
        raise ValueError("pre_contrastive_pixel: l_po must be [B,C_old,h,w]")
    if labels.dim() != 3 or labels.shape[0] != B:
        raise ValueError("pre_contrastive_pixel: l_n must be [B,H,W]")
    L = _lib.lib()
    dev = f_n.device
    labels = labels.to(torch.int64).contiguous()
    bf16_feats = f_n.dtype == torch.bfloat16 and f_o.dtype == torch.bfloat16
    if bf16_feats:
        f_n, f_o = f_n.contiguous(), f_o.contiguous()
    else:
        f_n, f_o = _f32c(f_n), _f32c(f_o)
    l_po = _f32c(l_po)
    H, W = labels.shape[-2:]
    pk = ContrastPack()
    pk.bf16_feats = bf16_feats
    pk.shape, pk.n_px, pk.c_old = (B, h, w), B * h * w, l_po.shape[1]
    pk.kpad = L.ucd_con_prob_kpad(pk.c_old)
    pk.max_tiles = L.ucd_con_max_tiles(pk.n_px)
    n_px = pk.n_px
    i32 = dict(device=dev, dtype=torch.int32)
    pk.max_label = int(max_label)
    nb = L.ucd_con_num_bins(pk.max_label, pk.c_old)
    pk.px_meta = torch.empty(7, n_px, **i32)
    pk.label_n, pk.mix, pk.flags = pk.px_meta[0], pk.px_meta[1], pk.px_meta[2]
    pk.blk_meta = torch.empty(L.ucd_con_blk_meta_ints(n_px, nb), **i32)
    lay = payload_layout(pk.max_tiles, pk.kpad)
    pk.payload = torch.empty(lay["nbytes"], device=dev, dtype=torch.uint8)
    base = pk.payload.data_ptr()
    ad = pk.addr = {k: base + lay[k] for k in ("counts", "range", "lab", "prob", "feat")}
    st = cur_stream()
    counts_host = _pinned_counts(dev)
    check(L.ucd_con_prep_labels(ptr(labels), ptr(l_po), B, pk.c_old, h, w, H, W, pk.max_label, ptr(pk.px_meta),
                                ptr(pk.blk_meta), ad["counts"], counts_host.data_ptr(), st), "con_prep_labels")
    copied = None
    if sync:
        copied = torch.cuda.Event()
        copied.record()
    pk.anchor_f32 = torch.empty(n_px, FEAT_DIM, device=dev, dtype=torch.float32)
    pk.contrast_f32 = torch.empty(2 * n_px, FEAT_DIM, device=dev, dtype=torch.float32)
    ldt = _label_dtype(max(pk.max_label, pk.c_old - 1))
    pk.la = torch.empty(n_px, device=dev, dtype=ldt)
    pk.lc = torch.empty(2 * n_px, device=dev, dtype=ldt)
    pk.row_range = torch.empty((n_px + TILE - 1) // TILE, 2, **i32)
    pk.row_ref = torch.empty(n_px, **i32)
    pk.inv_norm = torch.empty(n_px, device=dev, dtype=torch.float32)
    pack_fn = L.ucd_con_prep_pack_bf16 if bf16_feats else L.ucd_con_prep_pack
    check(pack_fn(ptr(f_n), ptr(f_o), ptr(l_po), ptr(pk.px_meta), ptr(pk.blk_meta), ad["counts"], B,
                  pk.c_old, h, w, pk.max_label, ptr(pk.anchor_f32), ptr(pk.contrast_f32), ptr(pk.la),
                  ptr(pk.lc), pk.la.element_size(), ad["feat"], ad["prob"], ad["lab"],
                  ad["range"], ptr(pk.row_range), ptr(pk.row_ref), ptr(pk.inv_norm),
                  pk.max_tiles, st),
          "con_prep_pack")
    pk.l_po = l_po
    if not sync:
        return pk
    copied.synchronize()
    pk.n_a, pk.n_o, pk.min_new, _ = (int(v) for v in counts_host.tolist())
    if require_new_class and pk.n_a > 0 and pk.min_new > max(int(max_label), 0):
        raise RuntimeError("pre_contrastive_pixel: no new-class pixel in the batch "
                           "(the reference raises here too, utils/loss.py:355)")
    return pk


class _AnchorFn(torch.autograd.Function):

    @staticmethod
    def forward(ctx, f_n, pack):
        ctx.pack = pack
        ctx.in_dtype = f_n.dtype
        return pack.anchor_f32[:pack.n_a]

    @staticmethod
    def backward(ctx, g):
        pk = ctx.pack
        B, h, w = pk.shape
        g = _f32c(g)
        if pk.n_a == 0:
            return torch.zeros(B, FEAT_DIM, h, w, device=g.device, dtype=ctx.in_dtype), None
        direct_bf16 = pk.bf16_feats and ctx.in_dtype == torch.bfloat16
        df = torch.empty(B, FEAT_DIM, h, w, device=g.device, dtype=torch.bfloat16 if direct_bf16 else torch.float32)
        bwd_fn = _lib.lib().ucd_con_prep_bwd_bf16 if direct_bf16 else _lib.lib().ucd_con_prep_bwd
        check(bwd_fn(ptr(g), ptr(pk.anchor_f32), ptr(pk.inv_norm), ptr(pk.px_meta),
                     ptr(pk.blk_meta), ptr(df), B, h, w, cur_stream()), "con_prep_bwd")
        return df.to(ctx.in_dtype), None


class JointProb:

    def __init__(self, pack):
        self.pack = pack

    @property
    def shape(self):
        return (self.pack.n_a, self.pack.n_c)

    def dense(self):
        pk = self.pack
        B, h, w = pk.shape
        p = torch.softmax(pk.l_po.permute(0, 2, 3, 1).reshape(pk.n_px, pk.c_old), dim=1)
        anchor = (pk.flags & 1).bool()
        pseudo = (pk.flags & 2).bool()
        pa = p[anchor]
        pc = torch.cat([pa, p[pseudo]])
        P = pa @ pc.T
        la, lc = pk.la[:pk.n_a].to(torch.int32), pk.lc[:pk.n_c].to(torch.int32)
        P[(la >= pk.min_new)[:, None] & (lc >= pk.min_new)[None, :]] = 1.0
        return P

    def detach(self):
        return self


def _label_dtype(max_label):
    return torch.int8 if max_label <= 127 else torch.int32


class _RowsFn(torch.autograd.Function):

    @staticmethod
    def forward(ctx, f):
        x = _f32c(f)
        B, D, h, w = x.shape
        rows = torch.empty(B * h * w, D, device=x.device, dtype=torch.float32)
        inv = torch.empty(B * h * w, device=x.device, dtype=torch.float32)
        check(_lib.lib().ucd_rows_normalize_fwd(ptr(x), ptr(rows), ptr(inv), B, h, w, cur_stream()), "rows_normalize_fwd")
        ctx.save_for_backward(rows, inv)
        ctx.shape, ctx.in_dtype = (B, D, h, w), f.dtype
        return rows

    @staticmethod
    def backward(ctx, g):
        rows, inv = ctx.saved_tensors
        B, D, h, w = ctx.shape
        df = torch.empty(B, D, h, w, device=g.device, dtype=torch.float32)
        check(_lib.lib().ucd_rows_normalize_bwd(ptr(_f32c(g)), ptr(rows), ptr(inv), ptr(df), B, h, w, cur_stream()),
              "rows_normalize_bwd")
        return df.to(ctx.in_dtype)


def _pixel_to_pixel(f_n, l_n, f_o, max_label):
    _need_cuda(f_n, l_n, f_o)
    if f_n.dim() != 4 or f_n.shape[1] != FEAT_DIM or (f_o is not None and f_o.shape != f_n.shape):
        raise ValueError("pre_contrastive_pixel: f_n / f_o must be [B,%d,h,w]" % FEAT_DIM)
    B, _, h, w = f_n.shape
    if l_n.dim() != 3 or l_n.shape[0] != B:
        raise ValueError("pre_contrastive_pixel: l_n must be [B,H,W]")
    L = _lib.lib()
    dev = f_n.device
    labels = l_n.to(torch.int64).contiguous()
    H, W = labels.shape[-2:]
    n_px = B * h * w
    i32 = dict(device=dev, dtype=torch.int32)
    px_meta = torch.empty(7, n_px, **i32)
    blk_meta = torch.empty(L.ucd_con_blk_meta_ints(n_px, L.ucd_con_num_bins(int(max_label), 1)), **i32)
    counts = torch.empty(4, **i32)
    dummy = torch.zeros(B, 1, h, w, device=dev, dtype=torch.float32)
    check(L.ucd_con_prep_labels(ptr(labels), ptr(dummy), B, 1, h, w, H, W, int(max_label), ptr(px_meta), ptr(blk_meta),
                                ptr(counts), None, cur_stream()), "con_prep_labels")
    lab = px_meta[0].to(_label_dtype(int(max_label)))
    out = _RowsFn.apply(f_n)
    if f_o is not None:
        out = torch.cat((out, _RowsFn.apply(f_o.detach())), dim=0)
        lab = torch.cat((lab, lab))
    return out.unsqueeze(1), lab


def pre_contrastive_pixel(f_n, l_n, l_po=None, f_o=None, max_label=20, require_new_class=None):
    if l_po is None:
        return _pixel_to_pixel(f_n, l_n, f_o, max_label)
    if f_o is None:
        raise UnboundLocalError("pre_contrastive_pixel: l_po without f_o is undefined in the reference too "
                                "(utils/loss.py:399 returns an unassigned `Output`)")
    if require_new_class is None:
        require_new_class = not _multi_rank()
    pack = _build_pack(f_n.detach(), f_o.detach(), l_po.detach(), l_n, max_label, require_new_class=require_new_class)
    anchor = _AnchorFn.apply(f_n, pack)
    anchor._ucd_pack = pack
    out = (anchor, pack.contrast_f32[:pack.n_c], pack.la[:pack.n_a], pack.lc[:pack.n_c], JointProb(pack))
    return out


pre_contractive_pixel = pre_contrastive_pixel


def _local_cols(pack):
    ad = pack.addr
    return dict(feat=ad["feat"], prob=ad["prob"], lab=ad["lab"], range=ad["range"],
                counts=ad["counts"], n_chunks=1, chunk_tiles=pack.max_tiles, kpad=pack.kpad, min_new=ad["counts"] + 8,
                payload=pack.payload)


def gather_contrast_columns(payload, max_tiles, kpad, group, async_op=False):
    import torch.distributed as dist
    world, rank = dist.get_world_size(group), dist.get_rank(group)
    payload = payload.contiguous()
    buf = torch.empty(world, payload.numel(), device=payload.device, dtype=torch.uint8)
    work = dist.all_gather_into_tensor(buf.view(-1), payload, group=group, async_op=async_op)
    out = payload_views(buf, max_tiles, kpad)
    out.update(buf=buf, n_chunks=world, chunk_tiles=max_tiles, chunk_stride=payload.numel(),
               self_tile0=rank * max_tiles, rank=rank, work=work if async_op else None)
    return out


class _ConFn(torch.autograd.Function):
    @staticmethod
    def forward(ctx, anchor, cols, rows, inv_tau, p_mode, dense_p, group, ddp_scale):
        L = _lib.lib()
        dev = anchor.device
        max_row_tiles = rows["max_tiles"]
        plan_tiles = rows.get("plan_tiles", 0)
        out = torch.empty(3, device=dev, dtype=torch.float32)
        need_grad = bool(ctx.needs_input_grad[0])
        grad_unit = (torch.empty(max_row_tiles * TILE, FEAT_DIM, device=dev, dtype=torch.float32)
                     if need_grad else None)

        def run(c, part, n_chunks, stride, local_chunk, self_tile0, ws, ws_bytes):
            check(L.ucd_con_fwd(ptr(c["feat"]), ptr(c["prob"]), ptr(c["lab"]), ptr(c["counts"]), n_chunks,
                                c["chunk_tiles"], stride, local_chunk, part, ptr(rows["feat"]), ptr(rows["prob"]),
                                ptr(rows["lab"]), ptr(rows["n_rows"]), ptr(c["range"]), ptr(rows["range"]),
                                self_tile0, ptr(c["min_new"]), p_mode, c["kpad"], ptr(dense_p),
                                0 if dense_p is None else dense_p.shape[1], inv_tau, 1 if need_grad else 0, ptr(out),
                                ptr(grad_unit), ptr(ws), ws_bytes, max_row_tiles, plan_tiles, cur_stream()),
                  "con_fwd")

        if group is None:
            ws_bytes = L.ucd_con_workspace_bytes(max_row_tiles, cols["n_chunks"] * cols["chunk_tiles"], plan_tiles, 0)
            ws = torch.empty(ws_bytes, device=dev, dtype=torch.uint8)
            run(cols, 0, cols["n_chunks"], 0, -1, rows["self_tile0"], ws, ws_bytes)
        else:
            g = gather_contrast_columns(cols["payload"], cols["chunk_tiles"], cols["kpad"], group, async_op=True)
            world, rank, T = g["n_chunks"], g["rank"], cols["chunk_tiles"]
            ws_bytes = L.ucd_con_workspace_bytes(max_row_tiles, world * T, plan_tiles, T)
            ws = torch.empty(ws_bytes, device=dev, dtype=torch.uint8)
            run(cols, 1, world, g["chunk_stride"], rank, g["self_tile0"], ws, ws_bytes)
            g["work"].wait()
            gc = dict(feat=g["feat"][0], prob=g["prob"][0], lab=g["lab"][0], range=g["range"][0],
                      counts=g["counts"][0], min_new=g["counts"][0, 2:3], chunk_tiles=T, kpad=cols["kpad"])
            run(gc, 2, world, g["chunk_stride"], rank, g["self_tile0"], ws, ws_bytes)
            ctx.gathered = g["buf"]
        world = 1
        if group is not None:
            import torch.distributed as dist
            dist.all_reduce(out[:2], group=group)
            world = dist.get_world_size(group)
        n_rows = rows["n_rows"]
        if isinstance(n_rows, int):
            ctx.n_rows_addr, ctx.keep = n_rows, rows.get("keep")
            ctx.save_for_backward(grad_unit, out, None, rows.get("row_ref"))
        else:
            ctx.n_rows_addr = None
            ctx.save_for_backward(grad_unit, out, n_rows, rows.get("row_ref"))
        ctx.static_pack = rows.get("static_pack")
        ctx.n_a = anchor.shape[0] if ctx.static_pack is None else ctx.static_pack.n_px
        ctx.in_dtype = anchor.dtype
        ctx.world = world if ddp_scale else 1
        if group is not None:
            return out[0] / out[1]
        return out[2]

    @staticmethod
    def backward(ctx, g):
        grad_unit, out, n_rows, row_ref = ctx.saved_tensors
        if ctx.n_rows_addr is not None:
            n_rows = ctx.n_rows_addr
        d_anchor = torch.empty(ctx.n_a, FEAT_DIM, device=g.device, dtype=torch.float32)
        if ctx.n_a == 0:
            return d_anchor.to(ctx.in_dtype), None, None, None, None, None, None, None
        check(_lib.lib().ucd_con_bwd(ptr(grad_unit), ptr(out), ptr(_f32c(g.reshape(1))), float(ctx.world),
                                     ptr(n_rows), ptr(row_ref), ptr(d_anchor), ctx.n_a, cur_stream()), "con_bwd")
        pk = ctx.static_pack
        if pk is not None:
            B, h, w = pk.shape
            direct_bf16 = pk.bf16_feats and ctx.in_dtype == torch.bfloat16
            df = torch.empty(B, FEAT_DIM, h, w, device=g.device,
                             dtype=torch.bfloat16 if direct_bf16 else torch.float32)
            bwd_fn = _lib.lib().ucd_con_prep_bwd_bf16 if direct_bf16 else _lib.lib().ucd_con_prep_bwd
            check(bwd_fn(ptr(d_anchor), ptr(pk.anchor_f32), ptr(pk.inv_norm), ptr(pk.px_meta),
                         ptr(pk.blk_meta), ptr(df), B, h, w, cur_stream()), "con_prep_bwd")
            d_anchor = df.to(ctx.in_dtype)
        return d_anchor, None, None, None, None, None, None, None


class PixelConLossV2(nn.Module):

    def __init__(self, sample_method='none', temperature=0.07, *, gather_negatives=False, process_group=None,
                 ddp_grad_scale=True):
        super(PixelConLossV2, self).__init__()
        self.temperature = temperature
        self.sample_method = sample_method
        self.gather_negatives = gather_negatives
        self.process_group = process_group
        self.ddp_grad_scale = ddp_grad_scale
        self.max_dense_bytes = 2 << 30
        print(temperature)

    def _group(self):
        if not self.gather_negatives:
            return None
        import torch.distributed as dist
        if not (dist.is_available() and dist.is_initialized()):
            return None
        g = self.process_group if self.process_group is not None else dist.group.WORLD
        return g if dist.get_world_size(g) > 1 else None

    def forward(self, anchor_features, contrast_feature, anchor_labels, contrast_labels, P=None):
        _need_cuda(anchor_features, contrast_feature)
        inv_tau = 1.0 / float(self.temperature)
        L = _lib.lib()
        dev = anchor_features.device
        pack = P.pack if isinstance(P, JointProb) else None
        own = pack is not None and (getattr(anchor_features, "_ucd_pack", None) is pack or (
            anchor_features.dtype == torch.float32 and tuple(anchor_features.shape) == (pack.n_a, FEAT_DIM)
            and (pack.n_a == 0 or anchor_features.data_ptr() == pack.anchor_f32.data_ptr())))
        if pack is not None and not own:
            import warnings
            n_bytes = 4.0 * pack.n_a * pack.n_c
            msg = ("PixelConLossV2: anchor_features is not the tensor pre_contrastive_pixel returned (cast / clone / "
                   "slice?): falling back to a dense %d x %d joint-probability matrix (%.2f GB).  Pass the tuple "
                   "through unchanged, or use PixelContrastiveDistillation." % (pack.n_a, pack.n_c, n_bytes / 1e9))
            if n_bytes > self.max_dense_bytes:
                raise RuntimeError(msg + "  Refusing: above max_dense_bytes=%d." % self.max_dense_bytes)
            warnings.warn(msg, RuntimeWarning, stacklevel=2)
            P, pack = P.dense(), None
        if pack is not None:
            group = self._group()
            ad = pack.addr
            rows = dict(feat=ad["feat"], prob=ad["prob"], lab=ad["lab"], n_rows=ad["counts"], keep=pack.payload,
                        range=pack.row_range, row_ref=pack.row_ref, max_tiles=max(1, (pack.n_a + TILE - 1) // TILE),
                        self_tile0=0)
            cols = _local_cols(pack)
            if pack.n_a == 0 and group is None:
                return anchor_features.sum() * 0.0
            return _ConFn.apply(anchor_features, cols, rows, inv_tau, 1, None, group, self.ddp_grad_scale)

        if anchor_features.dim() != 2 or anchor_features.shape[1] != FEAT_DIM or contrast_feature.shape[1] != FEAT_DIM:
            raise ValueError("PixelConLossV2: features must be [N,%d]" % FEAT_DIM)
        n_a, n_c = anchor_features.shape[0], contrast_feature.shape[0]
        if n_a == 0 or n_c == 0:
            return anchor_features.sum() * 0.0
        if contrast_feature.requires_grad and torch.is_grad_enabled():
            raise RuntimeError("PixelConLossV2: contrast_feature requires grad, but this implementation only "
                               "differentiates w.r.t. anchor_features (the UCD prep detaches the contrast side, "
                               "utils/loss.py:366); pass contrast_feature.detach() if that is what you mean")
        a32, c32 = _f32c(anchor_features.detach()), _f32c(contrast_feature.detach())
        la = anchor_labels.reshape(-1).to(device=dev, dtype=torch.int32).contiguous()
        lc = contrast_labels.reshape(-1).to(device=dev, dtype=torch.int32).contiguous()
        if la.numel() != n_a or lc.numel() != n_c:
            raise ValueError("PixelConLossV2: label / feature counts disagree")
        rt, ct = (n_a + TILE - 1) // TILE, (n_c + TILE - 1) // TILE
        bf = dict(device=dev, dtype=torch.bfloat16)
        rfeat = torch.empty(rt, FEAT_DIM // 8, TILE, 8, **bf)
        cfeat = torch.empty(ct, FEAT_DIM // 8, TILE, 8, **bf)
        rlab = torch.empty(rt, TILE, device=dev, dtype=torch.int32)
        clab = torch.empty(ct, TILE, device=dev, dtype=torch.int32)
        st = cur_stream()
        check(L.ucd_con_pack_rows(ptr(a32), ptr(la), n_a, ptr(rfeat), ptr(rlab), rt, st), "con_pack_rows")
        check(L.ucd_con_pack_rows(ptr(c32), ptr(lc), n_c, ptr(cfeat), ptr(clab), ct, st), "con_pack_rows")
        rrange = torch.empty(rt, 2, device=dev, dtype=torch.int32)
        crange = torch.empty(ct, 2, device=dev, dtype=torch.int32)
        check(L.ucd_con_tile_ranges(ptr(rlab), rt, None, ptr(rrange), st), "con_tile_ranges")
        check(L.ucd_con_tile_ranges(ptr(clab), ct, None, ptr(crange), st), "con_tile_ranges")
        counts = torch.tensor([[n_c, 0]], device=dev, dtype=torch.int32)
        n_rows = torch.tensor([n_a], device=dev, dtype=torch.int32)
        dense_p, p_mode = None, 0
        if P is not None:
            if tuple(P.shape) != (n_a, n_c):
                raise ValueError("PixelConLossV2: P must be [N_a, N_c]")
            dense_p, p_mode = _f32c(P.detach()), 2
        cols = dict(feat=cfeat, prob=None, lab=clab, range=crange, counts=counts, n_chunks=1, chunk_tiles=ct, kpad=16,
                    min_new=None)
        rows = dict(feat=rfeat, prob=None, lab=rlab, range=rrange, n_rows=n_rows, max_tiles=rt, self_tile0=0)
        return _ConFn.apply(anchor_features, cols, rows, inv_tau, p_mode, dense_p, None, False)


class _SelfConFn(torch.autograd.Function):
    @staticmethod
    def forward(ctx, rows, labels, mode, n_anchor, inv_tau, kappa):
        L = _lib.lib()
        dev = rows.device
        n, D = rows.shape
        x = _f32c(rows.detach())
        if D < FEAT_DIM:
            x = torch.nn.functional.pad(x, (0, FEAT_DIM - D))
        lab = labels.to(device=dev, dtype=torch.int32).contiguous()
        tiles = (n + TILE - 1) // TILE
        feat = torch.empty(tiles, FEAT_DIM // 8, TILE, 8, device=dev, dtype=torch.bfloat16)
        ltile = torch.empty(tiles, TILE, device=dev, dtype=torch.int32)
        rng = torch.empty(tiles, 2, device=dev, dtype=torch.int32)
        st = cur_stream()
        check(L.ucd_con_pack_rows(ptr(x), ptr(lab), n, ptr(feat), ptr(ltile), tiles, st), "con_pack_rows")
        check(L.ucd_con_tile_ranges(ptr(ltile), tiles, None, ptr(rng), st), "con_tile_ranges")
        meta = torch.tensor([n, 0, n], device=dev, dtype=torch.int32)
        need_grad = bool(ctx.needs_input_grad[0])
        out = torch.empty(3, device=dev, dtype=torch.float32)
        grad_unit = torch.empty(n, FEAT_DIM, device=dev, dtype=torch.float32) if need_grad else None
        ws_bytes = L.ucd_selfcon_workspace_bytes(tiles)
        ws = torch.empty(ws_bytes, device=dev, dtype=torch.uint8)
        check(L.ucd_selfcon_fwd(ptr(feat), ptr(ltile), ptr(rng), ptr(meta), meta.data_ptr() + 8, n, n_anchor, mode,
                                inv_tau, kappa, 1 if need_grad else 0, ptr(out), ptr(grad_unit), ptr(ws), ws_bytes, st),
              "selfcon_fwd")
        ctx.save_for_backward(grad_unit, out, meta)
        ctx.shape, ctx.in_dtype = (n, D), rows.dtype
        return out[2]

    @staticmethod
    def backward(ctx, g):
        grad_unit, out, meta = ctx.saved_tensors
        n, D = ctx.shape
        d = torch.empty(n, FEAT_DIM, device=g.device, dtype=torch.float32)
        check(_lib.lib().ucd_con_bwd(ptr(grad_unit), ptr(out), ptr(_f32c(g.reshape(1))), 1.0, meta.data_ptr() + 8, None,
                                     ptr(d), n, cur_stream()), "con_bwd")
        return d[:, :D].to(ctx.in_dtype), None, None, None, None, None


def _selfcon_rows(features, what):
    if features.dim() < 3:
        raise ValueError('`features` needs to be [bsz, n_views, ...],'
                         'at least 3 dimensions are required')
    _need_cuda(features)
    feats = features.reshape(features.shape[0], features.shape[1], -1)
    if feats.shape[2] > FEAT_DIM:
        raise NotImplementedError("%s: feature width %d > %d is not supported by the sweep kernels"
                                  % (what, feats.shape[2], FEAT_DIM))
    return feats, feats.transpose(0, 1).reshape(-1, feats.shape[2])


class PixelConLoss(nn.Module):

    def __init__(self, sample_method='none', temperature=1):
        super().__init__()
        self.temperature = temperature
        self.sample_method = sample_method

    def forward(self, features, labels=None):
        feats, rows = _selfcon_rows(features, "PixelConLoss")
        if labels is None:
            raise AttributeError("PixelConLoss: labels are required (the reference calls labels.view, loss_new.py:376)")
        lab = labels.reshape(-1)
        if lab.numel() != feats.shape[0] or feats.shape[1] != 1:
            raise ValueError("PixelConLoss: expected features [n, 1, D] and n labels")
        lab = lab.to(rows.device)
        lab = lab - lab.min()
        return _SelfConFn.apply(rows, lab, 0, rows.shape[0], 1.0 / float(self.temperature), 1.0)


class SupConLoss(nn.Module):

    def __init__(self, temperature=0.07, contrast_mode='all', base_temperature=0.07):
        super().__init__()
        self.temperature = temperature
        self.contrast_mode = contrast_mode
        self.base_temperature = base_temperature

    def forward(self, features, labels=None, mask=None):
        feats, rows = _selfcon_rows(features, "SupConLoss")
        bsz, n_views = feats.shape[0], feats.shape[1]
        if labels is not None and mask is not None:
            raise ValueError('Cannot define both `labels` and `mask`')
        if mask is not None:
            raise NotImplementedError("SupConLoss: an explicit `mask` is not supported; pass labels (or nothing: SimCLR)")
        if labels is None:
            lab = torch.arange(bsz, device=rows.device)
        else:
            lab = labels.contiguous().view(-1).to(rows.device)
            if lab.shape[0] != bsz:
                raise ValueError('Num of labels does not match num of features')
            lab = lab - lab.min()
        if self.contrast_mode == 'one':
            n_anchor = bsz
        elif self.contrast_mode == 'all':
            n_anchor = bsz * n_views
        else:
            raise ValueError('Unknown mode: {}'.format(self.contrast_mode))
        return _SelfConFn.apply(rows, lab.repeat(n_views), 1, n_anchor, 1.0 / float(self.temperature),
                                float(self.temperature) / float(self.base_temperature))


class PixelContrastiveDistillation(nn.Module):

    def __init__(self, temperature=0.07, max_label=20, *, gather_negatives=False, process_group=None,
                 ddp_grad_scale=True, expected_anchor_fraction=1.0):
        super().__init__()
        self.temperature = temperature
        self.max_label = int(max_label)
        self.gather_negatives = gather_negatives
        self.process_group = process_group
        self.ddp_grad_scale = ddp_grad_scale
        self.expected_anchor_fraction = float(expected_anchor_fraction)

    def _group(self):
        if not self.gather_negatives:
            return None
        import torch.distributed as dist
        if not (dist.is_available() and dist.is_initialized()):
            return None
        group = self.process_group if self.process_group is not None else dist.group.WORLD
        return group if dist.get_world_size(group) > 1 else None

    def forward(self, f_n, l_n, l_po, f_o):
        pack = _build_pack(f_n.detach(), f_o.detach(), l_po.detach(), l_n, self.max_label, sync=False)
        cap_tiles = (pack.n_px + TILE - 1) // TILE
        plan_tiles = max(1, min(cap_tiles, int(cap_tiles * self.expected_anchor_fraction + 0.999)))
        ad = pack.addr
        rows = dict(feat=ad["feat"], prob=ad["prob"], lab=ad["lab"], n_rows=ad["counts"], keep=pack.payload,
                    range=pack.row_range, row_ref=pack.row_ref, max_tiles=cap_tiles, self_tile0=0,
                    plan_tiles=plan_tiles, static_pack=pack)
        group = self._group()
        cols = _local_cols(pack)
        return _ConFn.apply(f_n, cols, rows, 1.0 / float(self.temperature), 1, None, group, self.ddp_grad_scale)


class _SegFusedFn(torch.autograd.Function):
    @staticmethod
    def forward(ctx, lr, lr_old, labels, old_cl, ignore_index, alpha):
        _need_cuda(lr, lr_old, labels)
        x, t = _f32c(lr), _f32c(lr_old)
        B, C, h, w = x.shape
        C_old = t.shape[1]
        H, W = labels.shape[-2:]
        dev = x.device
        need_grad = bool(ctx.needs_input_grad[0])
        sums = torch.empty(3, device=dev, dtype=torch.float32)
        g = torch.empty(2, B, C, h, w, device=dev, dtype=torch.float32) if need_grad else None
        n_ws = int(_lib.lib().ucd_seg_fused_workspace_floats(B, C, C_old, h, w, H, W))
        if n_ws == 0:
            raise ValueError("FusedUnbiasedLosses: shapes not supported (%s)" % ((B, C, C_old, h, w, H, W),))
        ws = torch.empty(n_ws, device=dev, dtype=torch.float32)
        check(_lib.lib().ucd_seg_fused_fwd(ptr(x), ptr(t), ptr(labels), ptr(g[0]) if need_grad else None,
                                           ptr(g[1]) if need_grad else None, ptr(sums), ptr(ws), n_ws, B, C, C_old,
                                           h, w, H, W, old_cl, ignore_index, float(alpha), 1 if need_grad else 0,
                                           cur_stream()), "seg_fused_fwd")
        ctx.save_for_backward(g)
        ctx.n_px = float(B * H * W)
        ctx.in_dtype = lr.dtype
        return sums[0] / ctx.n_px, sums[2] / ctx.n_px, sums[1]

    @staticmethod
    def backward(ctx, g_ce, g_kd, _g_cnt):
        (g,) = ctx.saved_tensors
        d = g[0] * (g_ce / ctx.n_px) + g[1] * (g_kd / ctx.n_px)
        return d.to(ctx.in_dtype), None, None, None, None, None


class FusedUnbiasedLosses(nn.Module):

    def __init__(self, old_cl, ignore_index=255, alpha=1., ce_reduction='mean'):
        super().__init__()
        self.old_cl, self.ignore_index, self.alpha, self.ce_reduction = int(old_cl), int(ignore_index), alpha, ce_reduction

    def forward(self, logits_lr, logits_old_lr, labels):
        if labels.dtype != torch.int64 or labels.dim() != 3:
            raise TypeError("FusedUnbiasedLosses: labels must be int64 [B,H,W]")
        if logits_lr.dim() != 4 or logits_old_lr.dim() != 4 or logits_lr.shape[0] != labels.shape[0] \
                or logits_lr.shape[2:] != logits_old_lr.shape[2:] or logits_old_lr.shape[1] > logits_lr.shape[1]:
            raise ValueError("FusedUnbiasedLosses: logits [B,C,h,w] / old logits [B,C_old,h,w] / labels [B,H,W] disagree")
        tgt = labels if labels.is_contiguous() else labels.contiguous()
        ce, kd, cnt = _SegFusedFn.apply(logits_lr, logits_old_lr.detach(), tgt, self.old_cl, self.ignore_index, self.alpha)
        if tgt is not labels:
            labels.copy_(tgt)
        if self.ce_reduction == 'valid':
            ce = ce * (float(labels.numel()) / cnt)
        return ce, kd
```

Before: 577,900.

## Compute CE and KD forward directly from low-res logits via fused bilinear upsample

Adds low-resolution forward kernels for the unbiased CE and KD losses. They rebuild upsampled logits on the fly from the pre-upsample source, using shared-memory row interpolation tiles, instead of reading the full-resolution upsampled tensors from HBM. Device walkers are refactored around a plane-source abstraction so the HBM and low-res paths share the same logsumexp code. The Python side detects tensors produced by the package's upsample, checks they are unmodified, and routes to the new path with a fallback. This cuts forward memory traffic but adds shared-memory syncs and recomputed interpolation.

```diff
diff --git a/include/ucd_b200.h b/include/ucd_b200.h
--- a/include/ucd_b200.h
+++ b/include/ucd_b200.h
@@ -27,6 +27,9 @@
 int ucd_unce_fwd(const float* x, int64_t* y, float* loss_px, float* lse_all, float* lse_old,
                  float* stats , float* scratch ,
                  int B, int C, int old_cl, int64_t HW, int ignore_index, void* stream);
+int ucd_unce_fwd_lowres(const float* lr, int64_t* y, float* loss_px, float* lse_all, float* lse_old,
+                        float* stats , float* scratch, int B, int C, int old_cl, int h, int w, int H, int W,
+                        int ignore_index, void* stream);
 int ucd_unce_bwd(const float* x, const int64_t* y, const float* lse_all,
                  const float* bkg_gap ,
                  const float* g_px, const float* g_scalar, float g_mul, const float* stats,
@@ -44,6 +47,9 @@
 int ucd_kd_fwd(const float* x, const float* t, const float* mask, float alpha, float* out_px, float* stats,
                float* lse3, float* scratch, int B, int C, int C_old, int64_t HW, int variant, float stats_scale,
                void* stream);
+int ucd_kd_fwd_lowres(const float* lr, const float* lo, const float* mask, float alpha, float* out_px, float* stats,
+                      float* lse3, float* scratch, int B, int C, int C_old, int h, int w, int H, int W, int variant,
+                      float stats_scale, void* stream);
 int ucd_kd_bwd(const float* x, const float* t, const float* mask, float alpha, const float* lse3,
                const float* g_px, const float* g_scalar, float g_mul, float* dx, int accumulate, int B, int C,
                int C_old, int64_t HW, int variant, void* stream);
diff --git a/ucd_b200/_lib.py b/ucd_b200/_lib.py
--- a/ucd_b200/_lib.py
+++ b/ucd_b200/_lib.py
@@ -16,10 +16,13 @@
     "ucd_device_ok": (c_int, []),
     "ucd_reduce_scratch_floats": (c_size_t, []),
     "ucd_unce_fwd": (c_int, [P, P, P, P, P, P, P, c_int, c_int, c_int, c_int64, c_int, P]),
+    "ucd_unce_fwd_lowres": (c_int, [P, P, P, P, P, P, P, c_int, c_int, c_int, c_int, c_int, c_int, c_int, c_int, P]),
     "ucd_unce_bwd": (c_int, [P, P, P, P, P, P, c_float, P, c_int, P, c_int, c_int, c_int, c_int, c_int64, c_int, P]),
     "ucd_unkd_fwd": (c_int, [P, P, P, c_float, P, P, P, P, c_int, c_int, c_int, c_int64, P]),
     "ucd_unkd_bwd": (c_int, [P, P, P, c_float, P, P, P, c_float, P, c_int, c_int, c_int, c_int, c_int64, P]),
     "ucd_kd_fwd": (c_int, [P, P, P, c_float, P, P, P, P, c_int, c_int, c_int, c_int64, c_int, c_float, P]),
+    "ucd_kd_fwd_lowres": (c_int, [P, P, P, c_float, P, P, P, P, c_int, c_int, c_int, c_int, c_int, c_int, c_int, c_int,
+                                  c_float, P]),
     "ucd_kd_bwd": (c_int, [P, P, P, c_float, P, P, P, c_float, P, c_int, c_int, c_int, c_int, c_int64, c_int, P]),
     "ucd_unce_unkd_bwd": (c_int, [P, P, P, P, P, P, c_float, P, c_int, c_int, c_int, P, P, c_float, P, P, P, c_float, c_int,
                                   P, c_int, c_int, c_int, c_int, c_int64, P]),
diff --git a/ucd_b200/csrc/ce_kd.cu b/ucd_b200/csrc/ce_kd.cu
--- a/ucd_b200/csrc/ce_kd.cu
+++ b/ucd_b200/csrc/ce_kd.cu
@@ -109,31 +109,72 @@
 }
 
 template <int VEC>
-__device__ __forceinline__ void lse_planes(const float*& xc, long long HW, int n, float (&m)[VEC], float (&s)[VEC]) {
+struct HbmPlanes {
+  const float* p;
+  long long HW;
+  __device__ __forceinline__ void next(float (&v)[4][VEC]) {
+    Vec<VEC>::load(p, v[0]);
+    Vec<VEC>::load(p + HW, v[1]);
+    Vec<VEC>::load(p + 2 * HW, v[2]);
+    Vec<VEC>::load(p + 3 * HW, v[3]);
+    p += 4 * HW;
+  }
+  __device__ __forceinline__ void tail(int n, float fill, float (&v)[4][VEC]) {
+#pragma unroll
+    for (int k = 0; k < 4; ++k) {
+      if (k < n) {
+        Vec<VEC>::load(p + k * HW, v[k]);
+      } else {
+#pragma unroll
+        for (int i = 0; i < VEC; ++i) v[k][i] = fill;
+      }
+    }
+    p += (long long)n * HW;
+  }
+};
+
+template <int VEC, class P>
+__device__ __forceinline__ void lse_planes(P& src, int n, float (&m)[VEC], float (&s)[VEC]) {
   int c = 0;
   for (; c + 4 <= n; c += 4) {
     float v[4][VEC];
-    Vec<VEC>::load(xc, v[0]);
-    Vec<VEC>::load(xc + HW, v[1]);
-    Vec<VEC>::load(xc + 2 * HW, v[2]);
-    Vec<VEC>::load(xc + 3 * HW, v[3]);
-    xc += 4 * HW;
+    src.next(v);
     lse_chunk4<VEC>(v, m, s);
   }
   if (c < n) {
     float v[4][VEC];
-#pragma unroll
-    for (int k = 0; k < 4; ++k) {
-      if (c + k < n) {
-        Vec<VEC>::load(xc + k * HW, v[k]);
-      } else {
-#pragma unroll
-        for (int i = 0; i < VEC; ++i) v[k][i] = kNegBig;
-      }
-    }
-    xc += (long long)(n - c) * HW;
+    src.tail(n - c, kNegBig, v);
     lse_chunk4<VEC>(v, m, s);
   }
+}
+
+template <int VEC, class P>
+__device__ __forceinline__ void unce_walk(P& src, int C, int oc, float (&m)[VEC], float (&s)[VEC],
+                                          float (&lse_old2)[VEC]) {
+#pragma unroll
+  for (int i = 0; i < VEC; ++i) m[i] = kNegBig, s[i] = 0.f;
+  lse_planes<VEC>(src, oc, m, s);
+#pragma unroll
+  for (int i = 0; i < VEC; ++i) lse_old2[i] = m[i] + lg2f(s[i]);
+  lse_planes<VEC>(src, C - oc, m, s);
+}
+
+__device__ __forceinline__ int unce_label(long long* yp, long long t, int old_cl, bool write) {
+  if (t < old_cl) {
+    if (t != 0 && write) *yp = 0;
+    t = 0;
+  }
+  return (t < 0 || t > 0x7fffffffLL) ? -1 : (int)t;
+}
+
+__device__ __forceinline__ float unce_px(float m, float s, float lse_old2, int lab, float picked, int C, int old_cl,
+                                         int ignore_index, float& la, float& lo) {
+  const float lse2 = m + lg2f(s);
+  la = lse2 * kLn2;
+  lo = lse_old2 * kLn2;
+  float l = (lab == 0 && old_cl > 0) ? (la - lo) : (la - picked);
+  if (lab == ignore_index || lab < 0 || lab >= C) l = 0.f;
+  return l;
 }
 
 __device__ __forceinline__ void group_to_bp(long long g, long long gpi, bool small, int vec, long long& b, long long& p) {
@@ -175,34 +216,18 @@
     float picked[VEC];
 #pragma unroll
     for (int i = 0; i < VEC; ++i) {
-      long long t = yl[i];
-      if (t < old_cl) {
-        if (t != 0) yp[i] = 0;
-        t = 0;
-      }
-      lab[i] = (t < 0 || t > 0x7fffffffLL) ? -1 : (int)t;
+      lab[i] = unce_label(yp + i, yl[i], old_cl, true);
       picked[i] = (lab[i] >= 0 && lab[i] < C) ? __ldg(xp + (long long)lab[i] * HW + i) : 0.f;
     }
     float m[VEC], s[VEC], lse_old2[VEC];
-#pragma unroll
-    for (int i = 0; i < VEC; ++i) m[i] = kNegBig, s[i] = 0.f;
-    const float* xc = xp;
-    lse_planes<VEC>(xc, HW, oc, m, s);
-#pragma unroll
-    for (int i = 0; i < VEC; ++i) lse_old2[i] = m[i] + lg2f(s[i]);
-    lse_planes<VEC>(xc, HW, C - oc, m, s);
+    HbmPlanes<VEC> src{xp, HW};
+    unce_walk<VEC>(src, C, oc, m, s, lse_old2);
     float out[VEC], la[VEC], lo[VEC];
 #pragma unroll
     for (int i = 0; i < VEC; ++i) {
-      const float lse2 = m[i] + lg2f(s[i]);
-      la[i] = lse2 * kLn2;
-      lo[i] = lse_old2[i] * kLn2;
-      const bool ign = lab[i] == ignore_index;
-      float l = (lab[i] == 0 && old_cl > 0) ? (la[i] - lo[i]) : (la[i] - picked[i]);
-      if (ign || lab[i] < 0 || lab[i] >= C) l = 0.f;
-      out[i] = l;
-      loss_acc += l;
-      valid_acc += ign ? 0.f : 1.f;
+      out[i] = unce_px(m[i], s[i], lse_old2[i], lab[i], picked[i], C, old_cl, ignore_index, la[i], lo[i]);
+      loss_acc += out[i];
+      valid_acc += lab[i] == ignore_index ? 0.f : 1.f;
     }
     Vec<VEC>::store(loss_px + b * HW + p, out);
     Vec<VEC>::store(lse_all_out + b * HW + p, la);
@@ -305,6 +330,59 @@
     }
     m[i] = nm, s[i] = acc, mt[i] = nt, st[i] = tacc, wx[i] = wacc;
   }
+}
+
+template <int VEC>
+struct UnkdStats {
+  float m[VEC], s[VEC], mt[VEC], st[VEC], wx[VEC], x0[VEC], t0[VEC], mn[VEC], sn[VEC];
+};
+
+template <int VEC, class P>
+__device__ __forceinline__ void unkd_walk(P& xs, P& ts, int C, int C_old, float a2, UnkdStats<VEC>& r) {
+#pragma unroll
+  for (int i = 0; i < VEC; ++i) r.m[i] = r.mt[i] = kNegBig, r.s[i] = r.st[i] = r.wx[i] = 0.f;
+  int c = 0;
+  for (; c + 4 <= C_old; c += 4) {
+    float v[4][VEC], u[4][VEC];
+    xs.next(v);
+    ts.next(u);
+    if (c == 0) {
+#pragma unroll
+      for (int i = 0; i < VEC; ++i) r.x0[i] = v[0][i], r.t0[i] = u[0][i] * a2;
+    }
+    unkd_old_chunk<VEC, false>(v, u, 4, c == 0, a2, r.m, r.s, r.mt, r.st, r.wx);
+  }
+  if (c < C_old) {
+    const int nv = C_old - c;
+    float v[4][VEC], u[4][VEC];
+    xs.tail(nv, 0.f, v);
+    ts.tail(nv, 0.f, u);
+    if (c == 0) {
+#pragma unroll
+      for (int i = 0; i < VEC; ++i) r.x0[i] = v[0][i], r.t0[i] = u[0][i] * a2;
+    }
+    unkd_old_chunk<VEC, true>(v, u, nv, c == 0, a2, r.m, r.s, r.mt, r.st, r.wx);
+  }
+#pragma unroll
+  for (int i = 0; i < VEC; ++i) r.mn[i] = kNegBig, r.sn[i] = 0.f;
+  lse_planes<VEC>(xs, C - C_old, r.mn, r.sn);
+}
+
+template <int VEC>
+__device__ __forceinline__ float unkd_px(const UnkdStats<VEC>& r, int i, float inv_cold, float& l_all, float& l_bkg,
+                                         float& l_t) {
+  const float ma = fmaxf(r.m[i], r.mn[i]);
+  const float lse2 = ma + lg2f(fmaf(r.s[i], ex2f(r.m[i] - ma), r.sn[i] * ex2f(r.mn[i] - ma)));
+  const float x02 = r.x0[i] * kLog2e;
+  const float mb = fmaxf(x02, r.mn[i]);
+  const float lseb2 = mb + lg2f(fmaf(r.sn[i], ex2f(r.mn[i] - mb), ex2f(x02 - mb)));
+  const float lset2 = r.mt[i] + lg2f(r.st[i]);
+  l_all = lse2 * kLn2;
+  l_bkg = lseb2 * kLn2;
+  l_t = lset2 * kLn2;
+  const float q0 = ex2f(r.t0[i] - lset2);
+  const float dot = r.wx[i] / r.st[i];
+  return (q0 * (l_bkg - l_all) + dot - (1.f - q0) * l_all) * inv_cold;
 }
 
 template <int VEC>
@@ -323,68 +401,15 @@
        g += (long long)gridDim.x * blockDim.x) {
     long long b, p;
     group_to_bp(g, gpi, small, VEC, b, p);
-    const float* xp = x + (b * Cs) * HW + p;
-    const float* xc = xp;
-    const float* tc = t + (b * C_old) * HW + p;
-    float m[VEC], s[VEC], mt[VEC], st[VEC], wx[VEC], x0[VEC], t0[VEC];
-#pragma unroll
-    for (int i = 0; i < VEC; ++i) m[i] = mt[i] = kNegBig, s[i] = st[i] = wx[i] = 0.f;
-    int c = 0;
-    for (; c + 4 <= C_old; c += 4) {
-      float v[4][VEC], u[4][VEC];
-#pragma unroll
-      for (int k = 0; k < 4; ++k) {
-        Vec<VEC>::load(xc + k * HW, v[k]);
-        Vec<VEC>::load(tc + k * HW, u[k]);
-      }
-      xc += 4 * HW, tc += 4 * HW;
-      if (c == 0) {
-#pragma unroll
-        for (int i = 0; i < VEC; ++i) x0[i] = v[0][i], t0[i] = u[0][i] * a2;
-      }
-      unkd_old_chunk<VEC, false>(v, u, 4, c == 0, a2, m, s, mt, st, wx);
-    }
-    if (c < C_old) {
-      const int nv = C_old - c;
-      float v[4][VEC], u[4][VEC];
-#pragma unroll
-      for (int k = 0; k < 4; ++k) {
-        if (k < nv) {
-          Vec<VEC>::load(xc + k * HW, v[k]);
-          Vec<VEC>::load(tc + k * HW, u[k]);
-        } else {
-#pragma unroll
-          for (int i = 0; i < VEC; ++i) v[k][i] = 0.f, u[k][i] = 0.f;
-        }
-      }
-      if (c == 0) {
-#pragma unroll
-        for (int i = 0; i < VEC; ++i) x0[i] = v[0][i], t0[i] = u[0][i] * a2;
-      }
-      unkd_old_chunk<VEC, true>(v, u, nv, c == 0, a2, m, s, mt, st, wx);
-    }
-    float mn[VEC], sn[VEC];
-#pragma unroll
-    for (int i = 0; i < VEC; ++i) mn[i] = kNegBig, sn[i] = 0.f;
-    xc = xp + (long long)C_old * HW;
-    lse_planes<VEC>(xc, HW, C - C_old, mn, sn);
+    HbmPlanes<VEC> xs{x + (b * Cs) * HW + p, HW}, ts{t + (b * C_old) * HW + p, HW};
+    UnkdStats<VEC> r;
+    unkd_walk<VEC>(xs, ts, C, C_old, a2, r);
     float o[VEC], l_all[VEC], l_bkg[VEC], l_t[VEC];
     float mk[VEC];
     if (mask != nullptr) Vec<VEC>::load_cached(mask + b * HW + p, mk);
 #pragma unroll
     for (int i = 0; i < VEC; ++i) {
-      const float ma = fmaxf(m[i], mn[i]);
-      const float lse2 = ma + lg2f(fmaf(s[i], ex2f(m[i] - ma), sn[i] * ex2f(mn[i] - ma)));
-      const float x02 = x0[i] * kLog2e;
-      const float mb = fmaxf(x02, mn[i]);
-      const float lseb2 = mb + lg2f(fmaf(sn[i], ex2f(mn[i] - mb), ex2f(x02 - mb)));
-      const float lset2 = mt[i] + lg2f(st[i]);
-      l_all[i] = lse2 * kLn2;
-      l_bkg[i] = lseb2 * kLn2;
-      l_t[i] = lset2 * kLn2;
-      const float q0 = ex2f(t0[i] - lset2);
-      const float dot = wx[i] / st[i];
-      float l = (q0 * (l_bkg[i] - l_all[i]) + dot - (1.f - q0) * l_all[i]) * inv_cold;
+      float l = unkd_px<VEC>(r, i, inv_cold, l_all[i], l_bkg[i], l_t[i]);
       if (mask != nullptr) l *= mask_zero ? (mk[i] == 0.f ? 1.f : 0.f) : mk[i];
       o[i] = -l;
       acc += l;
@@ -393,6 +418,251 @@
     Vec<VEC>::store(lse3 + b * HW + p, l_all);
     Vec<VEC>::store(lse3 + plane + b * HW + p, l_bkg);
     Vec<VEC>::store(lse3 + 2 * plane + b * HW + p, l_t);
+  }
+  __shared__ float red[32];
+  float r = block_sum(acc, red);
+  if (threadIdx.x == 0) part[blockIdx.x] = r;
+}
+
+constexpr int kLrWin = 32;
+constexpr int kLrMaxTW = 128;
+
+struct LrGeom {
+  const int *cx0, *cx1;
+  const float *cw0, *cw1;
+  int k, k1, w, hw, TW;
+};
+
+struct LrPlanes {
+  const float* src;
+  float* T;
+  const LrGeom* g;
+  int c, lo, hi, cend;
+  int tx4;
+  float h0, h1;
+  __device__ __forceinline__ void ensure(int n) {
+    if (c + n <= hi) return;
+    __syncthreads();
+    const int nc = min(kLrWin, cend - c), TW = g->TW, sh = __ffs(TW) - 1;
+    const int col = threadIdx.x & (TW - 1), js = blockDim.x >> sh;
+    const int a = g->cx0[col], b = g->cx1[col];
+    const float w0 = g->cw0[col], w1 = g->cw1[col];
+    const int d1 = (g->k1 - g->k) * g->w;
+    const float* p = src + (long long)c * g->hw + g->k * g->w;
+#pragma unroll 4
+    for (int j = threadIdx.x >> sh; j < nc; j += js) {
+      const float* r0 = p + (long long)j * g->hw;
+      const float v00 = __ldg(r0 + a), v01 = __ldg(r0 + b), v10 = __ldg(r0 + d1 + a), v11 = __ldg(r0 + d1 + b);
+      T[(2 * j) * TW + col] = __fmaf_rn(v00, w0, __fmul_rn(v01, w1));
+      T[(2 * j + 1) * TW + col] = __fmaf_rn(v10, w0, __fmul_rn(v11, w1));
+    }
+    __syncthreads();
+    lo = c, hi = c + nc;
+  }
+  __device__ __forceinline__ float get1(int ch, int i) const {
+    const float* p = T + (2 * (ch - lo)) * g->TW + tx4 + i;
+    return __fmaf_rn(p[0], h0, __fmul_rn(p[g->TW], h1));
+  }
+  __device__ __forceinline__ void get(int ch, float (&v)[4]) const {
+    const float* p = T + (2 * (ch - lo)) * g->TW + tx4;
+    const float4 t0 = *reinterpret_cast<const float4*>(p), t1 = *reinterpret_cast<const float4*>(p + g->TW);
+    v[0] = __fmaf_rn(t0.x, h0, __fmul_rn(t1.x, h1));
+    v[1] = __fmaf_rn(t0.y, h0, __fmul_rn(t1.y, h1));
+    v[2] = __fmaf_rn(t0.z, h0, __fmul_rn(t1.z, h1));
+    v[3] = __fmaf_rn(t0.w, h0, __fmul_rn(t1.w, h1));
+  }
+  __device__ __forceinline__ void next(float (&v)[4][4]) {
+    ensure(4);
+#pragma unroll
+    for (int k = 0; k < 4; ++k) get(c + k, v[k]);
+    c += 4;
+  }
+  __device__ __forceinline__ void tail(int n, float fill, float (&v)[4][4]) {
+    ensure(n);
+#pragma unroll
+    for (int k = 0; k < 4; ++k) {
+      if (k < n) {
+        get(c + k, v[k]);
+      } else {
+#pragma unroll
+        for (int i = 0; i < 4; ++i) v[k][i] = fill;
+      }
+    }
+    c += n;
+  }
+};
+
+struct LrBlock {
+  float s_h0[kIvMaxRows], s_h1[kIvMaxRows];
+  int s_lo[3], s_hi[3];
+  int cx0[kLrMaxTW], cx1[kLrMaxTW];
+  float cw0[kLrMaxTW], cw1[kLrMaxTW];
+};
+
+__device__ __forceinline__ int lr_item(LrBlock& sb, LrGeom& g, long long item, int n_tiles, int h, int w, int H, int W,
+                                       float scale_h, float scale_w, long long& b, int& Ya, int& ia, int& col0) {
+  const int tile = (int)(item % n_tiles);
+  const long long rest = item / n_tiles;
+  const int k = (int)(rest % h);
+  b = rest / h;
+  col0 = tile * g.TW;
+  __syncthreads();
+  for (int i = threadIdx.x; i < g.TW; i += blockDim.x) {
+    const Tap tx = bilinear_tap(min(col0 + i, W - 1), scale_w, w, W);
+    sb.cx0[i] = tx.i0, sb.cx1[i] = tx.i1, sb.cw0[i] = tx.w0, sb.cw1[i] = tx.w1;
+  }
+  g.k = k, g.k1 = min(k + 1, h - 1);
+  return interval_rows(k, h, H, scale_h, sb.s_h0, sb.s_h1, sb.s_lo, sb.s_hi, Ya, ia);
+}
+
+__device__ __forceinline__ float lr_point(const float* src, const LrGeom& g, int ch, float h0, float h1, const Tap& tx) {
+  const float* pl = src + (long long)ch * g.hw;
+  const float* r0 = pl + g.k * g.w;
+  const float* r1 = pl + g.k1 * g.w;
+  return bilinear_blend(false, __ldg(r0 + tx.i0), __ldg(r0 + tx.i1), __ldg(r1 + tx.i0), __ldg(r1 + tx.i1), h0, h1,
+                        tx.w0, tx.w1);
+}
+
+__global__ void __launch_bounds__(kStreamThreads, 3)
+unce_fwd_lowres_kernel(const float* __restrict__ lr, long long* __restrict__ y, float* __restrict__ loss_px,
+                       float* __restrict__ lse_all_out, float* __restrict__ lse_old_out, float* __restrict__ part,
+                       int B, int C, int old_cl, int ignore_index, int h, int w, int H, int W, float scale_h,
+                       float scale_w, int tw4, int n_tiles, int v4) {
+  extern __shared__ __align__(16) float lr_T[];
+  __shared__ LrBlock sb;
+  const int tx = threadIdx.x % tw4, rphase = threadIdx.x / tw4, rp = blockDim.x / tw4;
+  const long long HW = (long long)H * W;
+  const int oc = old_cl < C ? (old_cl > 0 ? old_cl : 0) : C;
+  LrGeom g{sb.cx0, sb.cx1, sb.cw0, sb.cw1, 0, 0, w, h * w, 4 * tw4};
+  float loss_acc = 0.f, valid_acc = 0.f;
+  const long long n_items = (long long)B * h * n_tiles;
+  for (long long item = blockIdx.x; item < n_items; item += gridDim.x) {
+    long long b;
+    int Ya, ia, col0;
+    const int nrow = lr_item(sb, g, item, n_tiles, h, w, H, W, scale_h, scale_w, b, Ya, ia, col0);
+    const float* src = lr + b * C * (long long)h * w;
+    const int X = col0 + 4 * tx;
+    for (int r0 = 0; r0 < nrow; r0 += rp) {
+      const int r = min(r0 + rphase, nrow - 1);
+      const bool live_row = r0 + rphase < nrow;
+      const float h0 = sb.s_h0[ia + r], h1 = sb.s_h1[ia + r];
+      const long long px = b * HW + (long long)(Ya + r) * W;
+      long long* yp = y + px;
+      long long yl[4];
+#pragma unroll
+      for (int i = 0; i < 4; ++i) yl[i] = yp[min(X + i, W - 1)];
+      LrPlanes xs{src, lr_T, &g, 0, 0, -1, C, 4 * tx, h0, h1};
+      xs.ensure(1);
+      int lab[4];
+      bool live[4];
+      float picked[4];
+#pragma unroll
+      for (int i = 0; i < 4; ++i) {
+        const int Xi = min(X + i, W - 1);
+        live[i] = live_row && X + i < W;
+        lab[i] = unce_label(yp + Xi, yl[i], old_cl, live[i]);
+        if (lab[i] >= 0 && lab[i] < xs.hi)
+          picked[i] = xs.get1(lab[i], i);
+        else
+          picked[i] = (lab[i] >= 0 && lab[i] < C) ? lr_point(src, g, lab[i], h0, h1, bilinear_tap(Xi, scale_w, w, W))
+                                                  : 0.f;
+      }
+      float m[4], s[4], lse_old2[4];
+      unce_walk<4>(xs, C, oc, m, s, lse_old2);
+      float out[4], la[4], lo[4];
+#pragma unroll
+      for (int i = 0; i < 4; ++i) {
+        out[i] = unce_px(m[i], s[i], lse_old2[i], lab[i], picked[i], C, old_cl, ignore_index, la[i], lo[i]);
+        if (live[i]) {
+          loss_acc += out[i];
+          valid_acc += lab[i] == ignore_index ? 0.f : 1.f;
+        }
+      }
+      if (v4 && live[3]) {
+        Vec<4>::store(loss_px + px + X, out);
+        Vec<4>::store(lse_all_out + px + X, la);
+        if (lse_old_out != nullptr) Vec<4>::store(lse_old_out + px + X, lo);
+      } else {
+#pragma unroll
+        for (int i = 0; i < 4; ++i)
+          if (live[i]) {
+            loss_px[px + X + i] = out[i];
+            lse_all_out[px + X + i] = la[i];
+            if (lse_old_out != nullptr) lse_old_out[px + X + i] = lo[i];
+          }
+      }
+    }
+  }
+  if (part != nullptr) {
+    __shared__ float red[32];
+    float r0 = block_sum(loss_acc, red);
+    float r1 = block_sum(valid_acc, red);
+    if (threadIdx.x == 0) {
+      part[blockIdx.x] = r0;
+      part[gridDim.x + blockIdx.x] = r1;
+    }
+  }
+}
+
+__global__ void __launch_bounds__(kStreamThreads, 3)
+unkd_fwd_lowres_kernel(const float* __restrict__ lr, const float* __restrict__ lo, const float* __restrict__ mask,
+                       float alpha, float* __restrict__ out_px, float* __restrict__ lse3, float* __restrict__ part,
+                       int B, int C, int Cs, int C_old, int mask_zero, int h, int w, int H, int W, float scale_h,
+                       float scale_w, int tw4, int n_tiles, int v4) {
+  extern __shared__ __align__(16) float lr_T[];
+  __shared__ LrBlock sb;
+  const int tx = threadIdx.x % tw4, rphase = threadIdx.x / tw4, rp = blockDim.x / tw4;
+  const long long HW = (long long)H * W, plane = (long long)B * HW;
+  const float a2 = alpha * kLog2e;
+  const float inv_cold = 1.f / (float)C_old;
+  LrGeom g{sb.cx0, sb.cx1, sb.cw0, sb.cw1, 0, 0, w, h * w, 4 * tw4};
+  float* T_t = lr_T + 2 * min(C, kLrWin) * g.TW;
+  float acc = 0.f;
+  const long long n_items = (long long)B * h * n_tiles;
+  for (long long item = blockIdx.x; item < n_items; item += gridDim.x) {
+    long long b;
+    int Ya, ia, col0;
+    const int nrow = lr_item(sb, g, item, n_tiles, h, w, H, W, scale_h, scale_w, b, Ya, ia, col0);
+    const long long lhw = (long long)h * w;
+    const int X = col0 + 4 * tx;
+    for (int r0 = 0; r0 < nrow; r0 += rp) {
+      const int r = min(r0 + rphase, nrow - 1);
+      const bool live_row = r0 + rphase < nrow;
+      const float h0 = sb.s_h0[ia + r], h1 = sb.s_h1[ia + r];
+      const long long px = b * HW + (long long)(Ya + r) * W;
+      LrPlanes xs{lr + b * Cs * lhw, lr_T, &g, 0, 0, -1, C, 4 * tx, h0, h1};
+      LrPlanes ts{lo + b * C_old * lhw, T_t, &g, 0, 0, -1, C_old, 4 * tx, h0, h1};
+      UnkdStats<4> st;
+      unkd_walk<4>(xs, ts, C, C_old, a2, st);
+      float o[4], l_all[4], l_bkg[4], l_t[4];
+      bool live[4];
+#pragma unroll
+      for (int i = 0; i < 4; ++i) {
+        live[i] = live_row && X + i < W;
+        float l = unkd_px<4>(st, i, inv_cold, l_all[i], l_bkg[i], l_t[i]);
+        if (mask != nullptr) {
+          const float mk = mask[px + min(X + i, W - 1)];
+          l *= mask_zero ? (mk == 0.f ? 1.f : 0.f) : mk;
+        }
+        o[i] = -l;
+        if (live[i]) acc += l;
+      }
+      if (v4 && live[3]) {
+        if (out_px != nullptr) Vec<4>::store(out_px + px + X, o);
+        Vec<4>::store(lse3 + px + X, l_all);
+        Vec<4>::store(lse3 + plane + px + X, l_bkg);
+        Vec<4>::store(lse3 + 2 * plane + px + X, l_t);
+      } else {
+#pragma unroll
+        for (int i = 0; i < 4; ++i)
+          if (live[i]) {
+            if (out_px != nullptr) out_px[px + X + i] = o[i];
+            lse3[px + X + i] = l_all[i];
+            lse3[plane + px + X + i] = l_bkg[i];
+            lse3[2 * plane + px + X + i] = l_t[i];
+          }
+      }
+    }
   }
   __shared__ float red[32];
   float r = block_sum(acc, red);
@@ -741,6 +1011,42 @@
   return true;
 }
 
+struct LrLaunch {
+  int tw4, n_tiles, grid;
+  size_t dyn;
+};
+static bool lowres_shape(const char* who, const void* kern, int B, int win_channels, int h, int w, int H, int W,
+                         LrLaunch& L, int& rc) {
+  if (!(H + W > 128 && H > h && W > w && (double)H / h <= 40.0)) {
+    set_error("%s: %dx%d -> %dx%d is not a shape the low-res path takes", who, h, w, H, W);
+    rc = UCD_ENOSUP;
+    return false;
+  }
+  int rp = 8;
+  while (rp < 32 && rp * h < H) rp *= 2;
+  L.tw4 = kStreamThreads / rp;
+  const int TW = 4 * L.tw4;
+  L.n_tiles = (W + TW - 1) / TW;
+  L.dyn = (size_t)2 * win_channels * TW * sizeof(float);
+  const long long n_items = (long long)B * h * L.n_tiles;
+  cudaError_t e = cudaFuncSetAttribute(kern, cudaFuncAttributeMaxDynamicSharedMemorySize, (int)L.dyn);
+  if (e != cudaSuccess) {
+    rc = cuda_fail(e, who);
+    return false;
+  }
+  int per_sm = 0;
+  e = cudaOccupancyMaxActiveBlocksPerMultiprocessor(&per_sm, kern, kStreamThreads, L.dyn);
+  if (e != cudaSuccess) {
+    rc = cuda_fail(e, who);
+    return false;
+  }
+  long long grid = (long long)(per_sm > 0 ? per_sm : 1) * kNumSMs;
+  if (grid > kStreamMaxBlocks) grid = kStreamMaxBlocks;
+  if (grid > n_items) grid = n_items;
+  L.grid = (int)grid;
+  return true;
+}
+
 }
 
 using namespace ucd;
@@ -772,6 +1078,32 @@
   return UCD_OK;
 }
 
+extern "C" int ucd_unce_fwd_lowres(const float* lr, int64_t* y, float* loss_px, float* lse_all, float* lse_old,
+                                   float* stats, float* scratch, int B, int C, int old_cl, int h, int w, int H, int W,
+                                   int ignore_index, void* stream) {
+  UCD_CHECK_ARG(lr && y && loss_px && lse_all, "ucd_unce_fwd_lowres: null pointer");
+  UCD_CHECK_ARG(B > 0 && C > 0 && h > 0 && w > 0 && H > 0 && W > 0, "ucd_unce_fwd_lowres: bad shape");
+  UCD_CHECK_ARG(old_cl >= 0 && old_cl <= C, "ucd_unce_fwd_lowres: old_cl=%d outside [0,%d]", old_cl, C);
+  UCD_CHECK_ARG(stats == nullptr || scratch != nullptr, "ucd_unce_fwd_lowres: stats requested without scratch");
+  LrLaunch L;
+  int rc = UCD_OK;
+  if (!lowres_shape("ucd_unce_fwd_lowres", (const void*)unce_fwd_lowres_kernel, B, min(C, kLrWin), h, w, H, W, L, rc))
+    return rc;
+  cudaStream_t st = (cudaStream_t)stream;
+  float* part = stats ? scratch : nullptr;
+  const int v4 = W % 4 == 0 && aligned16(y) && aligned16(loss_px) && aligned16(lse_all) &&
+                 (lse_old == nullptr || aligned16(lse_old));
+  unce_fwd_lowres_kernel<<<L.grid, kStreamThreads, L.dyn, st>>>(lr, (long long*)y, loss_px, lse_all, lse_old, part, B,
+                                                                 C, old_cl, ignore_index, h, w, H, W, (float)h / (float)H,
+                                                                 (float)w / (float)W, L.tw4, L.n_tiles, v4);
+  UCD_CHECK_LAUNCH("unce_fwd_lowres_kernel");
+  if (stats) {
+    reduce_partials_kernel<<<1, 256, 0, st>>>(part, L.grid, 2, stats, 1.f);
+    UCD_CHECK_LAUNCH("reduce_partials_kernel");
+  }
+  return UCD_OK;
+}
+
 extern "C" int ucd_unce_bwd(const float* x, const int64_t* y, const float* lse_all, const float* bkg_gap,
                             const float* g_px, const float* g_scalar, float g_mul, const float* stats,
                             int mean_over_valid, float* dx, int accumulate, int B, int C, int old_cl, int64_t HW,
@@ -845,6 +1177,31 @@
                           float* stats, float* lse3, float* scratch, int B, int C, int C_old, int64_t HW,
                           int variant, float stats_scale, void* stream) {
   return kd_fwd_impl(x, t, mask, alpha, out_px, stats, lse3, scratch, B, C, C_old, HW, variant, stats_scale, stream);
+}
+
+extern "C" int ucd_kd_fwd_lowres(const float* lr, const float* lo, const float* mask, float alpha, float* out_px,
+                                 float* stats, float* lse3, float* scratch, int B, int C, int C_old, int h, int w,
+                                 int H, int W, int variant, float stats_scale, void* stream) {
+  UCD_CHECK_ARG(lr && lo && stats && lse3 && scratch, "ucd_kd_fwd_lowres: null pointer");
+  UCD_CHECK_ARG(B > 0 && h > 0 && w > 0 && H > 0 && W > 0 && C_old >= 1 && C >= C_old,
+                "ucd_kd_fwd_lowres: bad shape C=%d C_old=%d", C, C_old);
+  UCD_CHECK_ARG(variant >= 0 && variant <= 2, "ucd_kd_fwd_lowres: bad variant %d", variant);
+  const int Cu = variant == 1 ? C_old : C, mz = variant == 2 ? 1 : 0;
+  LrLaunch L;
+  int rc = UCD_OK;
+  if (!lowres_shape("ucd_kd_fwd_lowres", (const void*)unkd_fwd_lowres_kernel, B, min(Cu, kLrWin) + min(C_old, kLrWin),
+                    h, w, H, W, L, rc))
+    return rc;
+  cudaStream_t st = (cudaStream_t)stream;
+  const int v4 = W % 4 == 0 && aligned16(lse3) && (out_px == nullptr || aligned16(out_px)) &&
+                 ((long long)B * H * W) % 4 == 0;
+  unkd_fwd_lowres_kernel<<<L.grid, kStreamThreads, L.dyn, st>>>(lr, lo, mask, alpha, out_px, lse3, scratch, B, Cu, C,
+                                                                 C_old, mz, h, w, H, W, (float)h / (float)H,
+                                                                 (float)w / (float)W, L.tw4, L.n_tiles, v4);
+  UCD_CHECK_LAUNCH("unkd_fwd_lowres_kernel");
+  reduce_partials_kernel<<<1, 256, 0, st>>>(scratch, L.grid, 1, stats, stats_scale);
+  UCD_CHECK_LAUNCH("reduce_partials_kernel");
+  return UCD_OK;
 }
 
 extern "C" int ucd_kd_bwd(const float* x, const float* t, const float* mask, float alpha, const float* lse3,
diff --git a/ucd_b200/csrc/common.cuh b/ucd_b200/csrc/common.cuh
--- a/ucd_b200/csrc/common.cuh
+++ b/ucd_b200/csrc/common.cuh
@@ -136,6 +136,34 @@
   return t;
 }
 
+constexpr int kIvMaxRows = 96;
+__device__ __forceinline__ int interval_rows(int k, int h, int H, float scale_h, float* s_h0, float* s_h1, int* s_lo,
+                                             int* s_hi, int& Ya, int& ia) {
+  const float inv = (float)H / (float)h;
+  int lo = (int)floorf(((float)k - 0.5f) * inv) - 2, hi = (int)ceilf(((float)k + 1.5f) * inv) + 2;
+  lo = max(lo, 0), hi = min(hi, H - 1);
+  if (threadIdx.x < kIvMaxRows) {
+    const int Y = lo + (int)threadIdx.x;
+    bool match = false;
+    if (Y <= hi) {
+      const Tap ty = bilinear_tap(Y, scale_h, h, H);
+      match = ty.i0 == k;
+      s_h0[threadIdx.x] = ty.w0, s_h1[threadIdx.x] = ty.w1;
+    }
+    const unsigned bal = __ballot_sync(0xffffffffu, match);
+    if ((threadIdx.x & 31) == 0) {
+      const int wq = threadIdx.x >> 5;
+      s_lo[wq] = bal ? wq * 32 + __ffs(bal) - 1 : 1 << 30;
+      s_hi[wq] = bal ? wq * 32 + 31 - __clz(bal) : -1;
+    }
+  }
+  __syncthreads();
+  ia = min(s_lo[0], min(s_lo[1], s_lo[2]));
+  const int ib = max(s_hi[0], max(s_hi[1], s_hi[2]));
+  Ya = lo + ia;
+  return ib - ia + 1;
+}
+
 __device__ __forceinline__ float bilinear_blend(bool small_out, float v00, float v01, float v10, float v11,
                                                 float h0, float h1, float w0, float w1) {
   if (small_out) {
diff --git a/ucd_b200/csrc/upsample.cu b/ucd_b200/csrc/upsample.cu
--- a/ucd_b200/csrc/upsample.cu
+++ b/ucd_b200/csrc/upsample.cu
@@ -87,12 +87,11 @@
   }
 }
 
-constexpr int kUpMaxIvRows = 96;
 template <int VEC>
 __global__ void __launch_bounds__(kUpThreads)
 upsample_fwd_interval_kernel(const float* __restrict__ in, float* __restrict__ out, int h, int w, int H, int W,
                              float scale_h, float scale_w, int tw, int n_col_tiles) {
-  __shared__ float s_h0[kUpMaxIvRows], s_h1[kUpMaxIvRows];
+  __shared__ float s_h0[kIvMaxRows], s_h1[kIvMaxRows];
   __shared__ int s_lo[3], s_hi[3];
   const int wv = (W + VEC - 1) / VEC;
   const int rp = kUpThreads / tw;
@@ -100,29 +99,9 @@
   const long long plane = blockIdx.x / per_plane;
   const int rem = (int)(blockIdx.x - plane * per_plane);
   const int k = rem / n_col_tiles, col_tile = rem - k * n_col_tiles;
-  const float inv = (float)H / (float)h;
-  int lo = (int)floorf(((float)k - 0.5f) * inv) - 2, hi = (int)ceilf(((float)k + 1.5f) * inv) + 2;
-  lo = max(lo, 0), hi = min(hi, H - 1);
-  if (threadIdx.x < kUpMaxIvRows) {
-    const int Y = lo + (int)threadIdx.x;
-    bool match = false;
-    if (Y <= hi) {
-      const Tap ty = bilinear_tap(Y, scale_h, h, H);
-      match = ty.i0 == k;
-      s_h0[threadIdx.x] = ty.w0, s_h1[threadIdx.x] = ty.w1;
-    }
-    const unsigned bal = __ballot_sync(0xffffffffu, match);
-    if ((threadIdx.x & 31) == 0) {
-      const int wq = threadIdx.x >> 5;
-      s_lo[wq] = bal ? wq * 32 + __ffs(bal) - 1 : 1 << 30;
-      s_hi[wq] = bal ? wq * 32 + 31 - __clz(bal) : -1;
-    }
-  }
-  __syncthreads();
-  const int ia = min(s_lo[0], min(s_lo[1], s_lo[2])), ib = max(s_hi[0], max(s_hi[1], s_hi[2]));
-  const int nrow = ib - ia + 1;
+  int Ya, ia;
+  const int nrow = interval_rows(k, h, H, scale_h, s_h0, s_h1, s_lo, s_hi, Ya, ia);
   if (nrow <= 0) return;
-  const int Ya = lo + ia;
   const int xg = col_tile * tw + (int)threadIdx.x % tw, rphase = (int)threadIdx.x / tw;
   if (xg >= wv || rphase >= rp) return;
   const int X = xg * VEC;
diff --git a/ucd_b200/losses.py b/ucd_b200/losses.py
--- a/ucd_b200/losses.py
+++ b/ucd_b200/losses.py
@@ -72,9 +72,32 @@
 
 def interpolate_bilinear(x, size):
     out = _UpsampleFn.apply(x, int(size[0]), int(size[1]))
-    if out.requires_grad:
-        out._ucd_upsample = (x, x._version, out._version)
+    out._ucd_upsample = (x, x._version, out._version)
     return out
+
+
+def _lowres_source(outputs):
+    src = _intact_source(outputs)
+    if src is None or not (src.is_cuda and src.dtype == torch.float32 and src.dim() == 4 and src.is_contiguous()
+                           and outputs.dim() == 4 and src.device == outputs.device
+                           and src.shape[:2] == outputs.shape[:2] and _lowres_shape_ok(src.shape, outputs.shape)):
+        return None
+    return src
+
+
+def _intact_source(outputs):
+    rec = getattr(outputs, "_ucd_upsample", None)
+    if rec is None:
+        return None
+    src, src_version, out_version = rec
+    if src._version != src_version or outputs._version != out_version:
+        return None
+    return src
+
+
+def _lowres_shape_ok(src_shape, out_shape):
+    (h, w), (H, W) = tuple(src_shape[2:]), tuple(out_shape[2:])
+    return H + W > 128 and H > h and W > w and H <= 40 * h
 
 
 class _Route:
@@ -205,8 +228,8 @@
 
 class _UnceFn(torch.autograd.Function):
     @staticmethod
-    def forward(ctx, inputs, targets, old_cl, ignore_index, reduction, chain=None, link=None, route=None, src=None,
-                probe=None):
+    def forward(ctx, inputs, targets, old_cl, ignore_index, reduction, lowres=None, chain=None, link=None, route=None,
+                src=None, probe=None):
         ctx.chain, ctx.is_head, ctx.seq = chain, link is None, (chain.calls if chain is not None else 0)
         ctx.route = route
         ctx.set_materialize_grads(False)
@@ -220,8 +243,16 @@
         stats = torch.empty(2, device=dev, dtype=torch.float32) if want_stats else None
         scratch = (torch.empty(_lib.lib().ucd_reduce_scratch_floats(), device=dev, dtype=torch.float32)
                    if want_stats else None)
-        check(_lib.lib().ucd_unce_fwd(ptr(x), ptr(targets), ptr(loss_px), ptr(lse), None, ptr(stats),
-                                      ptr(scratch), B, C, old_cl, HW, ignore_index, cur_stream()), "unce_fwd")
+        rc = _lib.UCD_ENOSUP
+        if lowres is not None:
+            lr = lowres[0]
+            rc = _lib.lib().ucd_unce_fwd_lowres(ptr(lr), ptr(targets), ptr(loss_px), ptr(lse), None, ptr(stats),
+                                                ptr(scratch), B, C, old_cl, lr.shape[2], lr.shape[3],
+                                                inputs.shape[2], inputs.shape[3], ignore_index, cur_stream())
+        if rc == _lib.UCD_ENOSUP:
+            rc = _lib.lib().ucd_unce_fwd(ptr(x), ptr(targets), ptr(loss_px), ptr(lse), None, ptr(stats),
+                                         ptr(scratch), B, C, old_cl, HW, ignore_index, cur_stream())
+        check(rc, "unce_fwd")
         ctx.save_for_backward(x, targets, lse, stats, loss_px)
         ctx.cfg = (B, C, HW, old_cl, ignore_index, reduction)
         out = loss_px if reduction == "none" else (stats[0].clone() if reduction == "sum" else stats[0] / stats[1])
@@ -235,9 +266,9 @@
         B, C, HW, old_cl, ignore_index, reduction = ctx.cfg
         if g is None:
             if ctx.chain is None:
-                return (None,) * 10
+                return (None,) * 11
             d_in, d_link, d_src = ctx.chain.submit(None, ctx.seq, ctx.is_head, ctx.route)
-            return d_in, None, None, None, None, None, d_link, None, d_src, None
+            return d_in, None, None, None, None, None, None, d_link, None, d_src, None
         g_px, g_sc = None, None
         if reduction == "none":
             g_sc = _scalar_grad(g)
@@ -253,9 +284,9 @@
         if ctx.chain is None:
             dx = torch.empty_like(x)
             _launch_term(term, dx, False)
-            return (dx,) + (None,) * 9
+            return (dx,) + (None,) * 10
         d_in, d_link, d_src = ctx.chain.submit(term, ctx.seq, ctx.is_head, ctx.route)
-        return d_in, None, None, None, None, None, d_link, None, d_src, None
+        return d_in, None, None, None, None, None, None, d_link, None, d_src, None
 
 
 def _chained(fn, inputs, args):
@@ -292,7 +323,9 @@
             raise ValueError("UnbiasedCrossEntropy: inputs [B,C,...] and targets [B,...] shapes disagree")
         old_cl = inputs.shape[1] if self.old_cl is None else int(self.old_cl)
         tgt = targets if targets.is_contiguous() else targets.contiguous()
-        out = _chained(_UnceFn, inputs, (tgt, old_cl, int(self.ignore_index), self.reduction))
+        src = _lowres_source(inputs)
+        out = _chained(_UnceFn, inputs, (tgt, old_cl, int(self.ignore_index), self.reduction,
+                                         None if src is None else (src,)))
         if tgt is not targets:
             targets.copy_(tgt)
         return out
@@ -300,8 +333,8 @@
 
 class _UnkdFn(torch.autograd.Function):
     @staticmethod
-    def forward(ctx, inputs, targets, mask, alpha, reduction, variant=0, chain=None, link=None, route=None, src=None,
-                probe=None):
+    def forward(ctx, inputs, targets, mask, alpha, reduction, variant=0, lowres=None, chain=None, link=None, route=None,
+                src=None, probe=None):
         ctx.chain, ctx.is_head, ctx.seq = chain, link is None, (chain.calls if chain is not None else 0)
         ctx.route = route
         ctx.set_materialize_grads(False)
@@ -316,8 +349,16 @@
         lse3 = torch.empty((3,) + px_shape, device=dev, dtype=torch.float32)
         scratch = torch.empty(_lib.lib().ucd_reduce_scratch_floats(), device=dev, dtype=torch.float32)
         scale = -1.0 / float(B * HW) if reduction == "mean" else -1.0
-        check(_lib.lib().ucd_kd_fwd(ptr(x), ptr(t), ptr(m), float(alpha), ptr(out_px), ptr(stats), ptr(lse3),
-                                    ptr(scratch), B, C, C_old, HW, variant, scale, cur_stream()), "kd_fwd")
+        rc = _lib.UCD_ENOSUP
+        if lowres is not None:
+            lr, lo = lowres
+            rc = _lib.lib().ucd_kd_fwd_lowres(ptr(lr), ptr(lo), ptr(m), float(alpha), ptr(out_px), ptr(stats),
+                                              ptr(lse3), ptr(scratch), B, C, C_old, lr.shape[2], lr.shape[3],
+                                              inputs.shape[2], inputs.shape[3], variant, scale, cur_stream())
+        if rc == _lib.UCD_ENOSUP:
+            rc = _lib.lib().ucd_kd_fwd(ptr(x), ptr(t), ptr(m), float(alpha), ptr(out_px), ptr(stats), ptr(lse3),
+                                       ptr(scratch), B, C, C_old, HW, variant, scale, cur_stream())
+        check(rc, "kd_fwd")
         ctx.save_for_backward(x, t, m, lse3)
         ctx.cfg = (B, C, C_old, HW, float(alpha), reduction, variant)
         out = out_px if reduction == "none" else stats[0]
@@ -331,9 +372,9 @@
         B, C, C_old, HW, alpha, reduction, variant = ctx.cfg
         if g is None:
             if ctx.chain is None:
-                return (None,) * 11
+                return (None,) * 12
             d_in, d_link, d_src = ctx.chain.submit(None, ctx.seq, ctx.is_head, ctx.route)
-            return d_in, None, None, None, None, None, None, d_link, None, d_src, None
+            return d_in, None, None, None, None, None, None, None, d_link, None, d_src, None
         g_px, g_sc, g_mul = None, None, 1.0
         if reduction == "none":
             g_sc = _scalar_grad(g)
@@ -350,9 +391,9 @@
         if ctx.chain is None:
             dx = torch.empty_like(x)
             _launch_term(term, dx, False)
-            return (dx,) + (None,) * 10
+            return (dx,) + (None,) * 11
         d_in, d_link, d_src = ctx.chain.submit(term, ctx.seq, ctx.is_head, ctx.route)
-        return d_in, None, None, None, None, None, None, d_link, None, d_src, None
+        return d_in, None, None, None, None, None, None, None, d_link, None, d_src, None
 
 
 class UnbiasedKnowledgeDistillationLoss(nn.Module):
@@ -369,7 +410,14 @@
         if mask is not None and tuple(mask.shape) != (inputs.shape[0],) + tuple(inputs.shape[2:]):
             raise ValueError("UnbiasedKnowledgeDistillationLoss: mask must be [B,...]")
         red = self.reduction if self.reduction in ("mean", "sum") else "none"
-        return _chained(_UnkdFn, inputs, (targets.detach(), mask, self.alpha, red, 0))
+        return _chained(_UnkdFn, inputs, (targets.detach(), mask, self.alpha, red, 0, _kd_lowres(inputs, targets)))
+
+
+def _kd_lowres(inputs, targets):
+    lr, lo = _lowres_source(inputs), _lowres_source(targets)
+    if lr is None or lo is None or lr.shape[2:] != lo.shape[2:]:
+        return None
+    return lr, lo
 
 
 def _kd_forward(name, variant, self, inputs, targets, mask):
@@ -379,7 +427,7 @@
     if mask is not None and tuple(mask.shape) != (inputs.shape[0],) + tuple(inputs.shape[2:]):
         raise ValueError("%s: mask must be [B,...]" % name)
     red = self.reduction if self.reduction in ("mean", "sum") else "none"
-    return _chained(_UnkdFn, inputs, (targets.detach(), mask, self.alpha, red, variant))
+    return _chained(_UnkdFn, inputs, (targets.detach(), mask, self.alpha, red, variant, _kd_lowres(inputs, targets)))
 
 
 class KnowledgeDistillationLoss(nn.Module):
```

Measured after the change: 563,800 (median of 6 runs). 0.976x the previous value.
